# NVIDIA/AMGX

Measured on AMD Instinct MI355X. Metric: amg_setup_solve_seconds_poisson256_fgmres_agg, lower is better.
Workload: dtype fp64; 1 GPU; global_batch=16777216, seq_len=256, parallelism=dd1, rows_per_gpu=16777216, converged=True

## Files before the change

amgx_amd/amg/coloring.py:

```python

from __future__ import annotations

from typing import Callable, Dict

import numpy as np
import torch

from .. import ops

COLORING_REGISTRY: Dict[str, Callable] = {}


def register_coloring(name: str):
    def deco(fn):
        COLORING_REGISTRY[name] = fn
        return fn
    return deco


def _host_adj(A, level: int = 1):
    import scipy.sparse as sp
    ro = A.row_offsets.cpu().numpy().astype(np.int64)
    ci = A.col_indices.cpu().numpy().astype(np.int64)
    n = A.n_rows
    keep = ci < n
    rows = np.repeat(np.arange(n), np.diff(ro))[keep]
    cols = ci[keep]
    g = sp.csr_matrix((np.ones(rows.size, dtype=np.int8), (rows, cols)),
                      shape=(n, n))
    g = g + g.T
    if level >= 2:
        g = g @ g
    g = g.tocsr()
    g.setdiag(0)
    g.eliminate_zeros()
    return g.indptr, g.indices


def _square_graph_matrix(A):
    from ..matrix import CSRMatrix
    n = A.n_rows
    dev = A.row_offsets.device
    ci = A.col_indices
    keep = ci < n
    if bool(keep.all()):
        ro, cols = A.row_offsets, A.col_indices
    else:
        deg = A.row_offsets.to(torch.int64)
        rows = torch.repeat_interleave(
            torch.arange(n, dtype=torch.int64, device=dev),
            deg[1:] - deg[:-1])
        kept = torch.bincount(rows[keep], minlength=n)
        ro = torch.zeros(n + 1, dtype=torch.int64, device=dev)
        torch.cumsum(kept, 0, out=ro[1:])
        ro = ro.to(torch.int32)
        cols = ci[keep].contiguous()
    P = CSRMatrix(ro, cols,
                  torch.ones(int(cols.numel()), dtype=torch.float64,
                             device=dev), n_cols=n)
    return ops.spgemm(P, P)


def _greedy(indptr, indices, order):
    n = indptr.size - 1
    colors = np.full(n, -1, dtype=np.int32)
    for i in order:
        nb = indices[indptr[i]:indptr[i + 1]]
        used = set(int(colors[j]) for j in nb if colors[j] >= 0)
        c = 0
        while c in used:
            c += 1
        colors[i] = c
    return colors, (int(colors.max()) + 1 if n else 0)


def _hash(i: np.ndarray, salt: int) -> np.ndarray:
    s = np.uint64((salt * 0x9E3779B97F4A7C15) % (1 << 64))
    x = (i.astype(np.uint64) + s) * np.uint64(0xBF58476D1CE4E5B9)
    return (x ^ (x >> np.uint64(31))).astype(np.uint64)


@register_coloring("MIN_MAX")
def _min_max(A, scope, level):
    frac = scope.get("max_uncolored_percentage") if scope is not None \
        else 0.0
    if level <= 1:
        return ops.color_matrix(A, max_uncolored_frac=float(frac or 0))
    return ops.color_matrix(_square_graph_matrix(A),
                            max_uncolored_frac=float(frac or 0))


@register_coloring("PARALLEL_GREEDY")
def _parallel_greedy(A, scope, level):
    if A.row_offsets.is_cuda:
        return ops.color_matrix(A if level <= 1 else _square_graph_matrix(A),
                                seed=7)
    indptr, indices = _host_adj(A, level)
    n = indptr.size - 1
    colors = np.full(n, -1, dtype=np.int32)
    w = _hash(np.arange(n), 7)
    guard = 0
    while (colors < 0).any():
        newly = []
        for i in np.nonzero(colors < 0)[0]:
            nb = indices[indptr[i]:indptr[i + 1]]
            un_nb = nb[colors[nb] < 0]
            un_nb = un_nb[un_nb != i]
            if un_nb.size and not (w[i] > w[un_nb]).all():
                continue
            used = set(int(colors[j]) for j in nb if colors[j] >= 0)
            c = 0
            while c in used:
                c += 1
            newly.append((i, c))
        for i, c in newly:
            colors[i] = c
        guard += 1
        if guard > n + 2:
            raise RuntimeError("PARALLEL_GREEDY coloring did not converge")
    return colors, int(colors.max()) + 1 if n else 0


@register_coloring("SERIAL_GREEDY_BFS")
def _serial_greedy_bfs(A, scope, level):
    import collections
    indptr, indices = _host_adj(A, level)
    n = indptr.size - 1
    order = []
    seen = np.zeros(n, dtype=bool)
    for s in range(n):
        if seen[s]:
            continue
        q = collections.deque([s])
        seen[s] = True
        while q:
            i = q.popleft()
            order.append(i)
            for j in indices[indptr[i]:indptr[i + 1]]:
                if not seen[j]:
                    seen[j] = True
                    q.append(j)
    return _greedy(indptr, indices, np.asarray(order, dtype=np.int64))


@register_coloring("GREEDY_RECOLOR")
def _greedy_recolor(A, scope, level):
    colors, num = COLORING_REGISTRY["MIN_MAX"](A, scope, level)
    if not torch.is_tensor(colors):
        colors = torch.from_numpy(np.ascontiguousarray(colors))
    colors = colors.to(A.row_offsets.device, torch.int64)
    n = A.n_rows
    if n == 0 or num <= 1:
        return colors.to(torch.int32), max(num, 1 if n else 0)
    dev = colors.device
    if level >= 2:
        if dev.type == "cuda":
            A2 = _square_graph_matrix(A)
            ro64 = A2.row_offsets.to(torch.int64)
            ci = A2.col_indices.to(torch.int64)
        else:
            indptr, indices = _host_adj(A, level)
            ro64 = torch.from_numpy(indptr.astype(np.int64))
            ci = torch.from_numpy(indices.astype(np.int64))
    else:
        ro64 = A.row_offsets.to(torch.int64)
        ci = A.col_indices.to(torch.int64)
    rows = torch.repeat_interleave(
        torch.arange(n, dtype=torch.int64, device=dev), ro64[1:] - ro64[:-1])
    keep = (ci < n) & (ci != rows)
    er, ec = rows[keep], ci[keep]
    for c in range(num - 1, 0, -1):
        in_class = colors == c
        if not bool(in_class.any()):
            continue
        sel = in_class[er]
        sr, sc = er[sel], ec[sel]
        local = torch.full((n,), -1, dtype=torch.int64, device=dev)
        cls_rows = torch.nonzero(in_class, as_tuple=True)[0]
        local[cls_rows] = torch.arange(cls_rows.numel(), dtype=torch.int64,
                                       device=dev)
        used = torch.zeros(cls_rows.numel(), c + 1, dtype=torch.bool,
                           device=dev)
        nb_col = torch.clamp(colors[sc], max=c)
        used[local[sr], nb_col] = True
        cand = torch.arange(c + 1, dtype=torch.int64, device=dev) \
            .expand(cls_rows.numel(), c + 1)
        new_c = torch.where(used, torch.full_like(cand, c), cand) \
            .min(dim=1).values
        colors[cls_rows] = torch.minimum(new_c, colors[cls_rows])
    return colors.to(torch.int32), int(colors.max()) + 1


@register_coloring("MULTI_HASH")
def _multi_hash(A, scope, level):
    if A.row_offsets.is_cuda:
        max_hash = int(scope.get("max_num_hash")) if scope is not None else 7
        return ops.color_matrix(A if level <= 1 else _square_graph_matrix(A),
                                seed=11, multihash_rounds=max_hash)
    indptr, indices = _host_adj(A, level)
    n = indptr.size - 1
    max_hash = int(scope.get("max_num_hash")) if scope is not None else 7
    colors = np.full(n, -1, dtype=np.int32)
    for salt in range(max_hash):
        w = _hash(np.arange(n), salt + 11)
        un = colors < 0
        un_rows = np.nonzero(un)[0]
        if un_rows.size == 0:
            break
        newc = []
        for i in un_rows:
            nb = indices[indptr[i]:indptr[i + 1]]
            nb = nb[un[nb]]
            nbw = w[nb[nb != i]]
            if nbw.size == 0 or w[i] > nbw.max():
                newc.append(i)
        colors[np.asarray(newc, dtype=np.int64)] = salt
    if (colors < 0).any():
        for i in np.nonzero(colors < 0)[0]:
            nb = indices[indptr[i]:indptr[i + 1]]
            used = set(int(colors[j]) for j in nb if colors[j] >= 0)
            c = 0
            while c in used:
                c += 1
            colors[i] = max(c, 0)
    return colors, int(colors.max()) + 1 if n else 0


@register_coloring("ROUND_ROBIN")
def _round_robin(A, scope, level):
    n = A.n_rows
    if A.row_offsets.is_cuda and n > 20000:
        num = int(scope.get("num_colors") or 0) if scope is not None else 0
        if num <= 0:
            ro = A.row_offsets.to(torch.int64)
            num = max(int((ro[1:] - ro[:-1]).max()) + 1, 1)
        colors = (torch.arange(n, dtype=torch.int64,
                               device=A.row_offsets.device)
                  % num).to(torch.int32)
        return colors, num
    indptr, indices = _host_adj(A, level)
    n = indptr.size - 1
    colors = np.full(n, -1, dtype=np.int32)
    k = 1
    for i in range(n):
        nb = indices[indptr[i]:indptr[i + 1]]
        used = set(int(colors[j]) for j in nb if colors[j] >= 0)
        start = i % max(k, 1)
        c = start
        while c in used:
            c += 1
        colors[i] = c
        k = max(k, c + 1)
    return colors, int(colors.max()) + 1 if n else 0


@register_coloring("UNIFORM")
def _uniform(A, scope, level):
    n = A.n_rows
    ro = A.row_offsets.to(torch.int64)
    k = int((ro[1:] - ro[:-1]).max()) + 1 if n else 1
    k = max(k, 1)
    colors = (torch.arange(n, dtype=torch.int64,
                           device=A.row_offsets.device) % k).to(torch.int32)
    return colors, k if n else 0


@register_coloring("MIN_MAX_2RING")
def _min_max_2ring(A, scope, level):
    return ops.color_matrix(_square_graph_matrix(A))


@register_coloring("GREEDY_MIN_MAX_2RING")
def _greedy_min_max_2ring(A, scope, level):
    if A.row_offsets.is_cuda:
        return ops.color_matrix(_square_graph_matrix(A), seed=3)
    indptr, indices = _host_adj(A, 2)
    return _greedy(indptr, indices, np.arange(indptr.size - 1))


@register_coloring("LOCALLY_DOWNWIND")
def _locally_downwind(A, scope, level):
    indptr, indices = _host_adj(A, level)
    ro = A.row_offsets.cpu().numpy().astype(np.int64)
    ci = A.col_indices.cpu().numpy().astype(np.int64)
    v = A.values.cpu().numpy().reshape(A.nnz, -1)[:, 0]
    n = A.n_rows
    rows = np.repeat(np.arange(n), np.diff(ro))
    off = (rows != ci) & (ci < n)
    outflow = np.zeros(n)
    np.add.at(outflow, rows[off], -v[off])
    order = np.argsort(-outflow, kind="stable")
    return _greedy(indptr, indices, order)


class MatrixColoring:
    def __init__(self, colors: torch.Tensor, num_colors: int):
        self.colors = colors
        self.num_colors = num_colors
        counts = torch.bincount(colors.to(torch.int64), minlength=num_colors)
        order = torch.argsort(colors.to(torch.int64), stable=True)
        self.rows_sorted = order.to(torch.int32).contiguous()
        b = [0]
        for c in counts.cpu().tolist():
            b.append(b[-1] + int(c))
        self.bounds = b
        self.bounds_dev = torch.tensor(b, dtype=torch.int32,
                                       device=colors.device)

    @classmethod
    def create(cls, A, scope=None) -> "MatrixColoring":
        scheme = (scope.get("matrix_coloring_scheme")
                  if scope is not None else "MIN_MAX") or "MIN_MAX"
        level = int(scope.get("coloring_level")) if scope is not None else 1
        fn = COLORING_REGISTRY.get(scheme)
        if fn is None:
            raise KeyError(f"unknown coloring scheme {scheme!r}; known: "
                           f"{sorted(COLORING_REGISTRY)}")
        colors, num = fn(A, scope, max(level, 1))
        if isinstance(colors, np.ndarray):
            colors = torch.from_numpy(colors)
        return cls(colors.to(A.row_offsets.device), num)

    def rows_of(self, c: int) -> torch.Tensor:
        return self.rows_sorted[self.bounds[c]:self.bounds[c + 1]]

    def validate(self, A, level: int = 1) -> bool:
        indptr, indices = _host_adj(A, level)
        col = self.colors.cpu().numpy()
        rows = np.repeat(np.arange(indptr.size - 1), np.diff(indptr))
        return not bool((col[rows] == col[indices]).any())
```

amgx_amd/amg/level.py:

```python

from __future__ import annotations

from typing import Optional

import numpy as np
import torch

from .. import ops
from ..matrix import CSRMatrix


class AMGLevel:

    def __init__(self, A: CSRMatrix, scope, index: int):
        self.A = A
        self.scope = scope
        self.index = index
        self.next: Optional[AMGLevel] = None
        self.smoother = None
        mgr = getattr(A, "manager", None)
        n = mgr.ext_size if mgr is not None else A.n_rows * A.block_dim
        self.r = torch.zeros(n, dtype=A.dtype, device=A.device)
        self.bc = None
        self.xc = None

    def create_coarse_vertices(self) -> int:
        raise NotImplementedError

    def create_coarse_matrix(self) -> CSRMatrix:
        raise NotImplementedError

    def restrict_residual(self, r, bc):
        raise NotImplementedError

    def prolongate_and_apply(self, xc, x):
        raise NotImplementedError

    def rebuild_coarse_values(self):
        return None

    def alloc_coarse_vectors(self, Ac: CSRMatrix):
        mgr = getattr(Ac, "manager", None)
        nc = mgr.ext_size if mgr is not None else Ac.n_rows * Ac.block_dim
        self.bc = torch.zeros(nc, dtype=Ac.dtype, device=Ac.device)
        self.xc = torch.zeros(nc, dtype=Ac.dtype, device=Ac.device)


class AggregationLevel(AMGLevel):

    def __init__(self, A, scope, index):
        super().__init__(A, scope, index)
        self.aggregates = None
        self.num_aggregates = 0
        self._scale = None
        self._scale_counter = 0

    def create_coarse_vertices(self) -> int:
        from .aggregation import AGG_SELECTOR_REGISTRY
        selector = self.scope.get("selector") or "SIZE_2"
        mgr = getattr(self.A, "manager", None)
        fn = AGG_SELECTOR_REGISTRY.get(selector)
        if fn is None:
            raise KeyError(f"unknown aggregation selector {selector!r}; "
                           f"known: {sorted(AGG_SELECTOR_REGISTRY)}")
        if mgr is not None:
            agg, num = fn(self._local_square_view(), self.scope)
        else:
            agg, num = fn(self.A, self.scope)
        self.aggregates = agg.to(self.A.row_offsets.device)
        self.num_aggregates = num
        self._build_r_structure()
        return num

    def _local_square_view(self) -> CSRMatrix:
        A = self.A
        n = A.n_rows
        ro = A.row_offsets.to(torch.int64)
        keep = A.col_indices.to(torch.int64) < n
        rows = torch.repeat_interleave(
            torch.arange(n, dtype=torch.int64, device=keep.device),
            ro[1:] - ro[:-1])
        counts = torch.bincount(rows[keep], minlength=n)
        ro2 = torch.zeros(n + 1, dtype=torch.int64, device=keep.device)
        torch.cumsum(counts, 0, out=ro2[1:])
        return CSRMatrix(ro2.to(torch.int32),
                         A.col_indices[keep].contiguous(),
                         A.values[keep].contiguous(),
                         n_cols=n, block_dim=A.block_dim)

    def _build_r_structure(self):
        agg = self.aggregates.to(torch.int64)
        order = torch.argsort(agg, stable=True).to(torch.int32)
        counts = torch.bincount(agg, minlength=self.num_aggregates)
        off = torch.zeros(self.num_aggregates + 1, dtype=torch.int64,
                          device=agg.device)
        torch.cumsum(counts, 0, out=off[1:])
        self.r_structure = (off.to(torch.int32).contiguous(),
                            order.contiguous())

    def create_coarse_matrix(self) -> CSRMatrix:
        mgr = getattr(self.A, "manager", None)
        gen = self.scope.get("coarseAgenerator")
        if mgr is None:
            Ac = ops.galerkin_aggregation(self.A, self.aggregates,
                                          self.num_aggregates, generator=gen)
            Ac = self._color_renumber(Ac)
            geom = self.A._cache.get("geometry")
            if geom is not None:
                g = np.asarray(geom, dtype=np.float64)
                agg = self.aggregates.cpu().numpy().astype(np.int64)
                sums = np.zeros((self.num_aggregates, g.shape[1]))
                cnts = np.zeros(self.num_aggregates)
                np.add.at(sums, agg, g)
                np.add.at(cnts, agg, 1.0)
                Ac._cache["geometry"] = sums / np.maximum(cnts, 1.0)[:, None]
            return Ac
        return self._create_coarse_matrix_distributed(mgr)

    def _create_coarse_matrix_distributed(self, mgr) -> CSRMatrix:
        import torch.distributed as tdist
        from ..distributed.manager import DistributedManager
        A = self.A
        nc_local = self.num_aggregates
        counts = [None] * mgr.world
        tdist.all_gather_object(counts, nc_local)
        coarse_start = int(sum(counts[:mgr.rank]))
        n_global_c = int(sum(counts))
        aggv = torch.zeros((A.n_cols,), dtype=torch.float64, device=A.device)
        aggv[:mgr.n_local] = self.aggregates.to(torch.float64) + coarse_start
        mgr.exchange_halo(aggv, block_override=1)
        agg_col = aggv.round().to(torch.int32)
        Ac_local = ops.galerkin_aggregation(
            A, self.aggregates, nc_local, agg_col, n_global_c,
            generator=self.scope.get("coarseAgenerator"))
        Ac = DistributedManager.upload_global_csr(
            Ac_local.row_offsets, Ac_local.col_indices, Ac_local.values,
            nc_local, coarse_start, n_global_c,
            device=A.device, block_dim=A.block_dim, dtype=A.dtype)
        iperm = Ac.manager.row_iperm.to(self.aggregates.device)
        self.aggregates = iperm[self.aggregates.long()].to(torch.int32)
        self._build_r_structure()
        return Ac

    def _color_renumber(self, Ac):
        import os

        import torch

        from .coloring import MatrixColoring
        if not os.environ.get("AMGX_AMD_COARSE_RENUMBER"):
            return Ac
        if (not Ac.values.is_cuda or Ac.block_dim != 1
                or getattr(self.A, "manager", None) is not None
                or Ac.n_rows < 512):
            return Ac
        col = MatrixColoring.create(Ac, self.scope)
        perm = col.rows_sorted.to(torch.int64)
        iperm = torch.empty_like(perm)
        iperm[perm] = torch.arange(Ac.n_rows, dtype=torch.int64,
                                   device=perm.device)
        self.aggregates = iperm[self.aggregates.to(torch.int64)] \
            .to(torch.int32)
        self._build_r_structure()
        Ac2 = ops.galerkin_aggregation(self.A, self.aggregates,
                                       self.num_aggregates,
                                       generator=self.scope.get(
                                           "coarseAgenerator"))
        self._coarse_coloring = MatrixColoring(
            col.colors[perm].contiguous(), col.num_colors)
        Ac2.coloring = self._coarse_coloring
        return Ac2

    def rebuild_coarse_values(self):
        if self.aggregates is None \
                or getattr(self.A, "manager", None) is not None:
            return None
        Ac = ops.galerkin_aggregation(self.A, self.aggregates,
                                      self.num_aggregates,
                                      generator=self.scope.get(
                                          "coarseAgenerator"))
        coloring = getattr(self, "_coarse_coloring", None)
        if coloring is not None and Ac.values.is_cuda:
            Ac.coloring = coloring
        return Ac

    def restrict_residual(self, r, bc):
        ops.restrict_agg(r, self.aggregates, self.num_aggregates,
                         self.A.block_dim,
                         structure=getattr(self, "r_structure", None), out=bc)

    def prolongate_and_apply(self, xc, x):
        es = int(self.scope.get("error_scaling") or 0)
        if es in (2, 3):
            self._prolongate_scaled(xc, x, es)
            return
        ops.prolongate_agg(x, xc, self.aggregates, self.A.block_dim)

    def _prolongate_scaled(self, xc, x, mode: int):
        import math

        if self.A.values.is_complex():
            raise NotImplementedError(
                "error_scaling 2 / 3 is not available in the complex modes")
        if self._scale_counter > 0 and self._scale is not None:
            ef = torch.zeros_like(x)
            ops.prolongate_agg(ef, xc, self.aggregates, self.A.block_dim)
            ops.axpy(x, ef, self._scale)
            self._scale_counter -= 1
            return
        ef = torch.zeros_like(x)
        ops.prolongate_agg(ef, xc, self.aggregates, self.A.block_dim)
        steps = int(self.scope.get("scaling_smoother_steps") or 2)
        if self.smoother is not None and steps > 0:
            self.smoother.sweep(self.r, ef, steps)
        Aef = torch.zeros_like(ef)
        ops.spmv(self.A, ef, Aef)
        mgr = getattr(self.A, "manager", None)

        def gdot(u, v):
            if mgr is not None:
                d = ops.dot(u.reshape(-1)[:mgr.owned_size],
                            v.reshape(-1)[:mgr.owned_size])
                return float(mgr.global_sum(d))
            return float(ops.dot(u, v))

        if mode == 2:
            num, den = gdot(self.r, Aef), gdot(Aef, Aef)
        else:
            num, den = gdot(self.r, ef), gdot(ef, Aef)
        if den == 0.0:
            alpha = 1.0
        else:
            alpha = num / den
            if abs(alpha) < 0.3:
                alpha = math.copysign(0.3, alpha)
            elif abs(alpha) > 10.0:
                alpha = math.copysign(10.0, alpha)
        ops.axpy(x, ef, alpha)
        self._scale = alpha
        self._scale_counter = int(self.scope.get("reuse_scale") or 0)


class ClassicalLevel(AMGLevel):

    default_selector = "PMIS"
    default_interp = "D1"

    def __init__(self, A, scope, index):
        if A.block_dim != 1:
            raise ValueError(
                "CLASSICAL AMG supports scalar (1x1) matrices only, got "
                f"block_dim={A.block_dim}; use algorithm=AGGREGATION for "
                "block systems")
        super().__init__(A, scope, index)
        self.P = None
        self.R = None
        self.cf_map = None
        self.num_coarse = 0

    def create_coarse_vertices(self) -> int:
        mgr = getattr(self.A, "manager", None)
        if mgr is not None:
            from .classical_dist import (aggressive_thin_dist, pmis_dist,
                                         strength_dist)
            theta = float(self.scope.get("strength_threshold"))
            mrs = float(self.scope.get("max_row_sum"))
            self._strong_out, strong_union = strength_dist(
                self.A, mgr, theta, mrs)
            cf, nc = pmis_dist(self.A, mgr, strong_union)
            self._aggressive = self.index < int(
                self.scope.get("aggressive_levels") or 0)
            if self._aggressive:
                cf, nc = aggressive_thin_dist(self.A, mgr, strong_union, cf)
            self.cf_map = cf
            self.num_coarse = nc
            self.A._cache["cf_map"] = self.cf_map
            return nc
        from .classical import SELECTOR_REGISTRY, STRENGTH_REGISTRY
        strength = self.scope.get("strength") or "AHAT"
        S = STRENGTH_REGISTRY[strength](self.A, self.scope)
        sel = self.scope.get("selector") if self.scope.has("selector") \
            else self.default_selector
        if sel in (None, "SIZE_2", "SIZE_4", "SIZE_8"):
            sel = self.default_selector
        if self.index < int(self.scope.get("aggressive_levels") or 0):
            agg_sel = self.scope.get("aggressive_selector")
            sel = ("AGGRESSIVE_" + sel) if agg_sel in (None, "DEFAULT") \
                else agg_sel
            self._aggressive = True
        else:
            self._aggressive = False
        cf, nc = SELECTOR_REGISTRY[sel](self.A, S, self.scope)
        dev = self.A.row_offsets.device
        S, cf = S.to(dev), cf.to(dev)
        self.S = S
        self.cf_map = cf
        self.num_coarse = nc
        self.A._cache["cf_map"] = cf
        return nc

    def create_coarse_matrix(self) -> CSRMatrix:
        mgr = getattr(self.A, "manager", None)
        if mgr is not None:
            return self._create_coarse_matrix_distributed(mgr)
        from .classical import INTERP_REGISTRY
        interp = self.scope.get("interpolator") \
            if self.scope.has("interpolator") else self.default_interp
        if getattr(self, "_aggressive", False):
            interp = self.scope.get("aggressive_interpolator") or "MULTIPASS"
        self.P = INTERP_REGISTRY[interp](self.A, self.S, self.cf_map,
                                         self.num_coarse, self.scope)
        if self.P.row_offsets.device != self.A.row_offsets.device:
            self.P = self.P.to(self.A.row_offsets.device)
        tf = float(self.scope.get("interp_truncation_factor"))
        me = int(self.scope.get("interp_max_elements"))
        if tf > 0.0 or me >= 0:
            self.P = ops.truncate_rows(self.P, tf, me)
        self.R = ops.transpose(self.P)
        Ac = ops.galerkin_rap(self.R, self.A, self.P)
        return Ac

    def rebuild_coarse_values(self):
        if self.cf_map is None \
                or getattr(self.A, "manager", None) is not None:
            return None
        from .classical import STRENGTH_REGISTRY
        strength = self.scope.get("strength") or "AHAT"
        self.S = STRENGTH_REGISTRY[strength](self.A, self.scope) \
            .to(self.A.row_offsets.device)
        self.A._cache["cf_map"] = self.cf_map
        return self.create_coarse_matrix()

    def _create_coarse_matrix_distributed(self, mgr) -> CSRMatrix:
        from .classical_dist import (ClassicalDistOperators,
                                     coarse_numbering, rap_dist)
        from ..distributed.manager import DistributedManager
        A = self.A
        cf_ext, coarse_offs = coarse_numbering(mgr, self.cf_map,
                                               self.num_coarse)
        interp = self.scope.get("interpolator") \
            if self.scope.has("interpolator") else self.default_interp
        if getattr(self, "_aggressive", False):
            interp = self.scope.get("aggressive_interpolator") or "MULTIPASS"
        if interp == "D2":
            from .classical_dist import interp_d2_dist
            P_m = interp_d2_dist(A, mgr, self._strong_out, cf_ext,
                                 coarse_offs,
                                 float(self.scope.get("strength_threshold")))
        elif interp in (None, "D1"):
            S_dev = self._strong_out
            if A.row_offsets.is_cuda:
                S_dev = S_dev.to(torch.uint8)
            P_m = ops._backend(A).interp_d1(A, S_dev, cf_ext,
                                            int(coarse_offs[-1]))
        elif interp == "MULTIPASS":
            from .classical_dist import interp_multipass_dist
            P_m = interp_multipass_dist(A, mgr, self._strong_out, cf_ext,
                                        coarse_offs)
        elif interp == "EM":
            from .classical_dist import interp_em_dist
            P_m = interp_em_dist(A, mgr, self._strong_out, cf_ext,
                                 coarse_offs)
        else:
            raise NotImplementedError(
                f"distributed interpolator {interp!r}: D1/D2/MULTIPASS/EM"
                " are wired")
        tf = float(self.scope.get("interp_truncation_factor"))
        me = int(self.scope.get("interp_max_elements"))
        if tf > 0.0 or me >= 0:
            P_m = ops.truncate_rows(P_m, tf, me)
        rap = rap_dist(A, mgr, P_m, coarse_offs)
        Ac = DistributedManager.upload_global_csr(
            rap.row_offsets, rap.col_indices, rap.values, self.num_coarse,
            int(coarse_offs[mgr.rank]), int(coarse_offs[-1]),
            device=A.row_offsets.device, block_dim=1, dtype=A.dtype)
        self._dist_ops = ClassicalDistOperators(A, mgr, P_m, Ac,
                                                coarse_offs)
        return Ac

    def restrict_residual(self, r, bc):
        if getattr(self, "_dist_ops", None) is not None:
            self._dist_ops.restrict(r, bc)
            return
        ops.spmv(self.R, r, bc)

    def prolongate_and_apply(self, xc, x):
        if getattr(self, "_dist_ops", None) is not None:
            self._dist_ops.prolongate_add(xc, x)
            return
        tmp = torch.zeros_like(x)
        ops.spmv(self.P, xc, tmp)
        ops.axpy(x, tmp, 1.0)


class EnergyminLevel(ClassicalLevel):

    @property
    def default_selector(self):
        return self.scope.get("energymin_selector") or "CR"

    @property
    def default_interp(self):
        return self.scope.get("energymin_interpolator") or "EM"


def create_level(algorithm: str, A, scope, index) -> AMGLevel:
    if A.values.is_complex() and algorithm != "AGGREGATION":
        raise NotImplementedError(
            f"algorithm={algorithm} (classical / energymin AMG) is not "
            "available in the complex modes")
    if algorithm == "AGGREGATION":
        return AggregationLevel(A, scope, index)
    if algorithm == "CLASSICAL":
        return ClassicalLevel(A, scope, index)
    if algorithm == "ENERGYMIN":
        return EnergyminLevel(A, scope, index)
    raise KeyError(f"unknown AMG algorithm {algorithm!r}")
```

amgx_amd/csrc/bindings.cpp:

```cpp

#include <torch/extension.h>
#include <ATen/cuda/CUDAContext.h>
#include <pybind11/complex.h>

#include <algorithm>
#include <array>
#include <climits>
#include <complex>
#include <vector>

#include "core_api.h"

namespace {

using torch::Tensor;

hipStream_t cur_stream() {
    return (hipStream_t)at::cuda::getCurrentCUDAStream().stream();
}

inline void check_dev(const Tensor& t) {
    TORCH_CHECK(t.is_cuda(), "amgx_amd._core requires device tensors");
}

// ... 330 lines not shown
    int n = (int)(ro.numel() - 1);
    check_scalar_if_complex(va, b, "gs_smooth_rows");
    DISPATCH(AMGX_VALUE_PAIRS, "gs_smooth_rows", (va, x), [&] {
        amgx_hip::gs_smooth_rows<scalar_a, scalar_v>(
            iptr(ro), iptr(ci), dptr<scalar_a>(va), dptr<scalar_a>(dinv),
            dptr<scalar_v>(bvec), dptr<scalar_v>(x), iptr(rows),
            (int)rows.numel(), (scalar_v)omega, n, (int)b, cur_stream());
    });
}

void gs_sweep(Tensor ro, Tensor ci, Tensor va, int64_t b, Tensor dinv,
              Tensor bvec, Tensor x, Tensor rows_sorted,
              std::vector<int64_t> bounds, double omega, bool symmetric) {
    check_block_dim(b, "gs_sweep");
    int n = (int)(ro.numel() - 1);
    check_scalar_if_complex(va, b, "gs_sweep");
    DISPATCH(AMGX_VALUE_PAIRS, "gs_sweep", (va, x), [&] {
        auto run = [&](int, int64_t s, int64_t e) {
            amgx_hip::gs_smooth_rows<scalar_a, scalar_v>(
                iptr(ro), iptr(ci), dptr<scalar_a>(va), dptr<scalar_a>(dinv),
                dptr<scalar_v>(bvec), dptr<scalar_v>(x), iptr(rows_sorted) + s,
                (int)(e - s), (scalar_v)omega, n, (int)b, cur_stream());
        };
        for_each_color(bounds, true, run);
        if (symmetric) for_each_color(bounds, false, run);
    });
}

void gs_sweep_sorted(Tensor ro_s, Tensor ci_s, Tensor va_s, Tensor dinv_s,
                     Tensor bvec, Tensor x, Tensor rows_sorted,
                     std::vector<int64_t> bounds, Tensor bounds_dev,
                     double omega, bool symmetric) {
    int nc = (int)bounds.size() - 1;
    int64_t n = (int64_t)ro_s.numel() - 1;
    if (n <= amgx_hip::SMALL_LEVEL_ROWS) {
        DISPATCH(AMGX_VALUE_PAIRS, "gs_sweep_small", (va_s, x), [&] {
            amgx_hip::gs_sweep_small<scalar_a, scalar_v>(
                iptr(ro_s), iptr(ci_s), dptr<scalar_a>(va_s),
                dptr<scalar_a>(dinv_s), dptr<scalar_v>(bvec),
                dptr<scalar_v>(x), iptr(rows_sorted), iptr(bounds_dev), nc,
                (scalar_v)omega, symmetric, cur_stream());
        });
        return;
    }
    DISPATCH(AMGX_VALUE_PAIRS, "gs_sweep_sorted", (va_s, x), [&] {
        auto run = [&](int, int64_t s, int64_t e) {
            amgx_hip::gs_rows_sorted<scalar_a, scalar_v>(
                iptr(ro_s) + s, iptr(ci_s), dptr<scalar_a>(va_s),
                dptr<scalar_a>(dinv_s) + s, dptr<scalar_v>(bvec),
                dptr<scalar_v>(x), iptr(rows_sorted) + s, (int)(e - s),
                (scalar_v)omega, cur_stream());
        };
        for_each_color(bounds, true, run);
        if (symmetric) for_each_color(bounds, false, run);
    });
}

Tensor dilu_setup(Tensor ro, Tensor ci, Tensor va, int64_t b, Tensor didx,
                  Tensor tidx, Tensor colors, Tensor rows_sorted,
                  std::vector<int64_t> bounds) {
    check_block_dim(b, "dilu_setup");
    int n = (int)(ro.numel() - 1);
    check_scalar_if_complex(va, b, "dilu_setup");
    auto einv = b == 1 ? torch::zeros({n}, va.options())
                       : torch::zeros({n, b, b}, va.options());
    DISPATCH(AMGX_VALUE_TYPES, "dilu_setup", (va), [&] {
        for_each_color(bounds, true, [&](int c, int64_t s, int64_t e) {
            amgx_hip::dilu_setup_color<scalar_t>(
                iptr(ro), iptr(ci), dptr<scalar_t>(va), iptr(didx), iptr(tidx),
                iptr(colors), iptr(rows_sorted) + s, (int)(e - s), c,
                dptr<scalar_t>(einv), (int)b, cur_stream());
        });
    });
    return einv;
}

std::vector<Tensor> slab_split(Tensor ro_s, Tensor ci_s, Tensor rows_sorted,
                               Tensor colors, bool upper) {
    check_dev(ro_s);
    int64_t n = (int64_t)ro_s.numel() - 1;
    TORCH_CHECK(rows_sorted.numel() == n && colors.numel() == n,
                "slab_split: rows_sorted / colors do not have n rows");
    hipStream_t st = cur_stream();
    auto ro_x = torch::empty({n + 1}, ro_s.options());
    long long nnz = amgx_hip::slab_split_count(
        iptr(ro_s), iptr(ci_s), iptr(rows_sorted), iptr(colors), (int)n,
        upper, iptr(ro_x), st);
    auto ci_x = torch::empty({(int64_t)nnz}, ro_s.options());
    auto map_x = torch::empty({(int64_t)nnz}, ro_s.options());
    amgx_hip::slab_split_fill(iptr(ro_s), iptr(ci_s), iptr(rows_sorted),
                              iptr(colors), (int)n, upper, iptr(ro_x),
                              iptr(ci_x), iptr(map_x), st);
    return {ro_x, ci_x, map_x};
}

void dilu_sorted(Tensor ro_s, Tensor ci_s, Tensor va_s, int64_t b,
                 Tensor einv_s, Tensor rows_sorted,
                 std::vector<int64_t> bounds, Tensor bounds_dev, Tensor rhs,
                 Tensor w, Tensor z, Tensor x, double relax, bool fused,
                 bool any_size) {
    check_block_dim(b, "dilu_sorted");
    TORCH_CHECK(!fused || b == 1 || b == 4,
                "dilu_sorted: no fused-residual kernel for block_dim ", b);
    check_scalar_if_complex(va_s, b, "dilu_sorted");
    int nc = (int)bounds.size() - 1;
    int bb = (int)(b * b);
    int64_t n = (int64_t)ro_s.numel() - 1;
    if (b == 1) {
        TORCH_CHECK(any_size || n <= amgx_hip::DILU_SMALL_ROWS,
                    "dilu_sorted: scalar levels of more than ",
                    amgx_hip::DILU_SMALL_ROWS, " rows run dilu_split");
        TORCH_CHECK(bounds_dev.numel() == nc + 1 && rows_sorted.numel() == n &&
                        w.numel() >= n && z.numel() >= w.numel() &&
                        x.numel() >= n && rhs.numel() >= n &&
                        (!fused || x.numel() >= w.numel()),
                    "dilu_sorted: vectors shorter than the matrix");
        DISPATCH(AMGX_VALUE_PAIRS, "dilu_small_full", (va_s, x), [&] {
            amgx_hip::dilu_small_full<scalar_a, scalar_v>(
                iptr(ro_s), iptr(ci_s), dptr<scalar_a>(va_s),
                dptr<scalar_a>(einv_s), iptr(rows_sorted), iptr(bounds_dev),
                nc, dptr<scalar_v>(rhs), dptr<scalar_v>(w), dptr<scalar_v>(z),
                dptr<scalar_v>(x), (scalar_v)relax, (long long)w.numel(),
                fused, cur_stream());
        });
        return;
    }
    w.zero_();
    z.zero_();
    DISPATCH(AMGX_VALUE_PAIRS, "dilu_sorted", (va_s, x), [&] {
        hipStream_t st = cur_stream();
        const scalar_v* xres = fused ? dptr<scalar_v>(x) : nullptr;
        for_each_color(bounds, true, [&](int, int64_t s, int64_t e) {
            amgx_hip::dilu_fwd_sorted<scalar_a, scalar_v>(
                iptr(ro_s) + s, iptr(ci_s), dptr<scalar_a>(va_s),
                dptr<scalar_a>(einv_s) + s * bb, iptr(rows_sorted) + s,
                (int)(e - s), dptr<scalar_v>(rhs), xres, dptr<scalar_v>(w),
                (int)b, st);
        });
        for_each_color(bounds, false, [&](int, int64_t s, int64_t e) {
            amgx_hip::dilu_bwd_sorted<scalar_a, scalar_v>(
                iptr(ro_s) + s, iptr(ci_s), dptr<scalar_a>(va_s),
                dptr<scalar_a>(einv_s) + s * bb, iptr(rows_sorted) + s,
                (int)(e - s), dptr<scalar_v>(w), dptr<scalar_v>(z), (int)b,
                st);
        });
        amgx_hip::axpy<scalar_v>(dptr<scalar_v>(x), dptr<scalar_v>(z),
                                 (scalar_v)relax, x.numel(), st);
    });
}

constexpr double DILU_LANES_THRESHOLD_FULL = 8.0;
constexpr double DILU_LANES_THRESHOLD_SPLIT = 4.0;
int64_t dilu_lanes(double entries_per_row, bool split) {
    double t = split ? DILU_LANES_THRESHOLD_SPLIT : DILU_LANES_THRESHOLD_FULL;
    return entries_per_row <= t ? 1 : 8;
}

constexpr int64_t DILU_STREAM_MIN_ROWS_FULL = 1 << 14;
constexpr int64_t DILU_STREAM_MIN_ROWS_SPLIT = 1 << 14;
bool dilu_stream(double entries_per_row, int64_t color_rows, bool split) {
    int64_t least = split ? DILU_STREAM_MIN_ROWS_SPLIT
                          : DILU_STREAM_MIN_ROWS_FULL;
    return entries_per_row > 0.0 && color_rows >= least;
}

void dilu_split(Tensor ro_f, Tensor ci_f, Tensor va_f, Tensor ro_u,
                Tensor ci_u, Tensor va_u, Tensor einv_s, Tensor rows_sorted,
                std::vector<int64_t> bounds, Tensor rhs, Tensor w, Tensor x,
                double relax, bool fused, int64_t lanes,
                c10::optional<Tensor> y_opt, int64_t form) {
    int64_t n = (int64_t)ro_u.numel() - 1;
    TORCH_CHECK(ro_f.numel() == n + 1 && rows_sorted.numel() == n &&
                    einv_s.numel() == n,
                "dilu_split: slabs, rows_sorted and Einv disagree on n");
    TORCH_CHECK(form == 0 || form == 1 || form == 2,
                "dilu_split: form must be 0 (routed), 1 (lane forms) or 2 "
                "(stream form)");
    TORCH_CHECK(form != 2 || lanes == 0,
                "dilu_split: the stream form takes no lanes");
    TORCH_CHECK(!bounds.empty() && bounds.front() == 0 && bounds.back() == n,
                "dilu_split: color bounds do not cover the n rows");
    TORCH_CHECK(va_f.numel() == ci_f.numel() && va_u.numel() == ci_u.numel(),
                "dilu_split: scalar slabs hold one value per column index");
    TORCH_CHECK(rhs.numel() >= n && x.numel() >= n && w.numel() >= n &&
                    (!fused || w.numel() >= x.numel()),
                "dilu_split: vectors shorter than the matrix");
    TORCH_CHECK(w.scalar_type() == x.scalar_type() &&
                    rhs.scalar_type() == x.scalar_type() &&
                    va_u.scalar_type() == va_f.scalar_type() &&
                    einv_s.scalar_type() == va_f.scalar_type(),
                "dilu_split: mixed value types");
    TORCH_CHECK(lanes == 0 || lanes == 1 || lanes == 8,
                "dilu_split: lanes must be 0 (routed), 1 or 8");
    Tensor y;
    if (fused) {
        y = y_opt.has_value() ? *y_opt : torch::empty_like(w);
        TORCH_CHECK(y.is_contiguous() && y.device() == x.device() &&
                        y.scalar_type() == x.scalar_type() &&
                        y.numel() >= x.numel(),
                    "dilu_split: y must be a vector like w");
    }
    double rows = (double)std::max<int64_t>(n, 1);
    int lanes_f = lanes ? (int)lanes
                        : (int)dilu_lanes((double)ci_f.numel() / rows, !fused);
    int lanes_u = lanes ? (int)lanes
                        : (int)dilu_lanes((double)ci_u.numel() / rows, true);
    const double epr_f = (double)ci_f.numel() / rows;
    const double epr_u = (double)ci_u.numel() / rows;
    auto pick = [&](int lane_form, double epr, int64_t count, bool split) {
        bool stream = form == 2 || (form == 0 && lanes == 0 &&
                                    dilu_stream(epr, count, split));
        return stream ? amgx_hip::DILU_STREAM : lane_form;
    };
    DISPATCH(AMGX_VALUE_PAIRS, "dilu_split", (va_f, x), [&] {
        hipStream_t st = cur_stream();
        if (fused)
            amgx_hip::dilu_y_init<scalar_v>(dptr<scalar_v>(x),
                                            dptr<scalar_v>(y),
                                            (long long)x.numel(), st);
        for_each_color(bounds, true, [&](int, int64_t s, int64_t e) {
            if (fused)
                amgx_hip::dilu_fwd_full<scalar_a, scalar_v>(
                    iptr(ro_f) + s, iptr(ci_f), dptr<scalar_a>(va_f),
                    dptr<scalar_a>(einv_s) + s, iptr(rows_sorted) + s,
                    (int)(e - s), dptr<scalar_v>(rhs), dptr<scalar_v>(x),
                    dptr<scalar_v>(w), dptr<scalar_v>(y),
                    pick(lanes_f, epr_f, e - s, false), st);
            else
                amgx_hip::dilu_fwd_lower<scalar_a, scalar_v>(
                    iptr(ro_f) + s, iptr(ci_f), dptr<scalar_a>(va_f),
                    dptr<scalar_a>(einv_s) + s, iptr(rows_sorted) + s,
                    (int)(e - s), dptr<scalar_v>(rhs), dptr<scalar_v>(w),
                    pick(lanes_f, epr_f, e - s, true), st);
        });
        for_each_color(bounds, false, [&](int, int64_t s, int64_t e) {
            amgx_hip::dilu_bwd_upper<scalar_a, scalar_v>(
                iptr(ro_u) + s, iptr(ci_u), dptr<scalar_a>(va_u),
                dptr<scalar_a>(einv_s) + s, iptr(rows_sorted) + s,
                (int)(e - s), dptr<scalar_v>(w), dptr<scalar_v>(x),
                (scalar_v)relax, pick(lanes_u, epr_u, e - s, true), st);
        });
    });
}

void dilu_small(Tensor ro_f, Tensor ci_f, Tensor va_f, Tensor ro_u,
                Tensor ci_u, Tensor va_u, Tensor einv_s, Tensor rows_sorted,
                std::vector<int64_t> bounds, Tensor bounds_dev, Tensor rhs,
                Tensor w, Tensor x, double relax, bool fused, int64_t lanes,
                c10::optional<Tensor> y_opt, int64_t sweeps, bool any_size) {
    int64_t n = (int64_t)ro_u.numel() - 1;
    int64_t nc = (int64_t)bounds.size() - 1;
    TORCH_CHECK(any_size || n <= amgx_hip::DILU_SMALL_ROWS,
                "dilu_small: scalar levels of more than ",
                amgx_hip::DILU_SMALL_ROWS, " rows run dilu_split");
    TORCH_CHECK(ro_f.numel() == n + 1 && rows_sorted.numel() == n &&
                    einv_s.numel() == n,
                "dilu_small: slabs, rows_sorted and Einv disagree on n");
    TORCH_CHECK(!bounds.empty() && bounds.front() == 0 && bounds.back() == n &&
                    bounds_dev.numel() == nc + 1 &&
                    bounds_dev.scalar_type() == torch::kInt32,
                "dilu_small: color bounds do not cover the n rows");
    TORCH_CHECK(va_f.numel() == ci_f.numel() && va_u.numel() == ci_u.numel(),
                "dilu_small: scalar slabs hold one value per column index");
    TORCH_CHECK(rhs.numel() >= n && x.numel() >= n && w.numel() >= n &&
                    (!fused || w.numel() >= x.numel()),
                "dilu_small: vectors shorter than the matrix");
    TORCH_CHECK(w.scalar_type() == x.scalar_type() &&
                    rhs.scalar_type() == x.scalar_type() &&
                    va_u.scalar_type() == va_f.scalar_type() &&
                    einv_s.scalar_type() == va_f.scalar_type(),
                "dilu_small: mixed value types");
    TORCH_CHECK(lanes == 0 || lanes == 1 || lanes == 8,
                "dilu_small: lanes must be 0 (routed), 1 or 8");
    TORCH_CHECK(sweeps >= 1 && sweeps <= (1 << 20),
                "dilu_small: sweeps must be at least 1");
    for (Tensor t : {ro_f, ci_f, va_f, ro_u, ci_u, va_u, einv_s, rows_sorted,
                     bounds_dev, rhs, w, x})
        check_dev(t);
    Tensor y;
    if (fused) {
        TORCH_CHECK(y_opt.has_value(), "dilu_small: a fused apply needs y");
        y = *y_opt;
        TORCH_CHECK(y.is_contiguous() && y.device() == x.device() &&
                        y.scalar_type() == x.scalar_type() &&
                        y.numel() >= x.numel(),
                    "dilu_small: y must be a vector like w");
    }
    double rows = (double)std::max<int64_t>(n, 1);
    int lanes_f = lanes ? (int)lanes
                        : (int)dilu_lanes((double)ci_f.numel() / rows, !fused);
    int lanes_u = lanes ? (int)lanes
                        : (int)dilu_lanes((double)ci_u.numel() / rows, true);
    DISPATCH(AMGX_VALUE_PAIRS, "dilu_small", (va_f, x), [&] {
        amgx_hip::dilu_small<scalar_a, scalar_v>(
            iptr(ro_f), iptr(ci_f), dptr<scalar_a>(va_f), iptr(ro_u),
            iptr(ci_u), dptr<scalar_a>(va_u), dptr<scalar_a>(einv_s),
            iptr(rows_sorted), iptr(bounds_dev), (int)nc, dptr<scalar_v>(rhs),
            dptr<scalar_v>(w), fused ? dptr<scalar_v>(y) : nullptr,
            dptr<scalar_v>(x), (scalar_v)relax, (long long)x.numel(), fused,
            lanes_f, lanes_u, (int)sweeps, cur_stream());
    });
}

std::tuple<Tensor, int64_t> color_minmax(Tensor ro, Tensor ci, int64_t n,
                                         int64_t max_rounds, int64_t seed,
                                         int64_t mode1_rounds) {
    auto colors = torch::full({n}, -1,
                              ro.options().dtype(torch::kInt32));
    auto colors_next = torch::empty_like(colors);
    auto counter = torch::zeros({1}, ro.options().dtype(torch::kInt32));
    hipStream_t st = cur_stream();
    int rounds = 0;
    for (; rounds < max_rounds; ++rounds) {
        counter.zero_();
        int mode = rounds < mode1_rounds ? 1 : 0;
        amgx_hip::color_minmax_round(
            iptr(ro), iptr(ci), (int)n, iptr(colors), iptr(colors_next),
            rounds, (int)(seed + rounds * 7919), mode, iptr(counter), st);
        std::swap(colors, colors_next);
        int left = counter.cpu().item<int>();
        if (left == 0) break;
    }
    TORCH_CHECK((colors.min().cpu().item<int>()) >= 0,
                "MIN_MAX coloring did not converge in ", max_rounds,
                " rounds");
    int64_t ncolors = (colors.max().cpu().item<int>()) + 1;
    return {colors, ncolors};
}

Tensor size2_match(Tensor ro, Tensor ci, Tensor va, Tensor tidx, Tensor diag,
                   int64_t n, int64_t max_iters, int64_t seed) {
    auto agg = torch::full({n}, -1, ro.options().dtype(torch::kInt32));
    auto prop = torch::empty({n}, ro.options().dtype(torch::kInt32));
    auto changed = torch::zeros({1}, ro.options().dtype(torch::kInt32));
    hipStream_t st = cur_stream();
    DISPATCH(AMGX_VALUE_TYPES, "size2_match", (va), [&] {
        for (int it = 0; it < max_iters; ++it) {
            amgx_hip::agg_propose<scalar_t>(
                iptr(ro), iptr(ci), dptr<scalar_t>(va), iptr(tidx),
                dptr<scalar_t>(diag), (int)n, iptr(agg), iptr(prop), (int)seed,
                st);
            changed.zero_();
            amgx_hip::agg_match(iptr(prop), (int)n, iptr(agg), iptr(changed),
                                st);
            if (changed.cpu().item<int>() == 0) break;
        }
        auto agg_out = torch::empty_like(agg);
        amgx_hip::agg_merge_singletons<scalar_t>(
            iptr(ro), iptr(ci), dptr<scalar_t>(va), iptr(tidx),
            dptr<scalar_t>(diag), (int)n, iptr(agg), iptr(agg_out), st);
        agg = agg_out;
    });
    return agg;
}

Tensor pairwise_weights(Tensor ro, Tensor ci, Tensor va, Tensor tidx,
                        Tensor diag, int64_t n, int64_t formula) {
    check_dev(va);
    TORCH_CHECK(formula == 0 || formula == 1,
                "pairwise_weights: weight_formula must be 0 or 1");
    TORCH_CHECK_NOT_IMPLEMENTED(formula == 0 || !va.is_complex(),
                                "pairwise_weights: weight_formula 1 is "
                                "signed and unavailable for complex values");
    TORCH_CHECK(tidx.numel() == ci.numel() && va.numel() == ci.numel() &&
                    diag.numel() == n && ro.numel() == n + 1,
                "pairwise_weights: array sizes do not match the structure");
    auto w = torch::empty({ci.numel()}, va.options().dtype(torch::kFloat64));
    DISPATCH(AMGX_VALUE_TYPES, "pairwise_weights", (va), [&] {
        amgx_hip::pairwise_weights<scalar_t>(
            iptr(ro), iptr(ci), dptr<scalar_t>(va), iptr(tidx),
            dptr<scalar_t>(diag), (int)n, (int)formula, dptr<double>(w),
            cur_stream());
    });
    return w;
}

int pairwise_lanes(int64_t nnz, int64_t n) {
    double avg = (double)nnz / (double)std::max<int64_t>(n, 1);
    return avg <= 8.0 ? 1 : 8;
}

Tensor pairwise_propose(Tensor ro, Tensor ci, Tensor w, int64_t n, Tensor agg,
                        Tensor sizes, int64_t cap, int64_t seed,
                        int64_t lanes) {
    check_dev(w);
    TORCH_CHECK(ro.numel() == n + 1 && w.numel() == ci.numel() &&
                    agg.numel() == n && sizes.numel() == n,
                "pairwise_propose: array sizes do not match the structure");
    auto prop = torch::empty({n}, ro.options().dtype(torch::kInt32));
    int icap = cap <= 0 ? INT_MAX : (int)std::min<int64_t>(cap, INT_MAX);
    if (lanes == 0) lanes = pairwise_lanes(ci.numel(), n);
    amgx_hip::pairwise_propose(iptr(ro), iptr(ci), dptr<double>(w), (int)n,
                               iptr(agg), iptr(sizes), icap, (int)seed,
                               (int)lanes, iptr(prop), cur_stream());
    return prop;
}

std::tuple<Tensor, int64_t, Tensor, int64_t> pairwise_match(
    Tensor ro, Tensor ci, Tensor w, int64_t n, Tensor sizes_in, int64_t cap,
    int64_t merge_singletons, int64_t max_iters, double max_unassigned,
    int64_t seed, int64_t lanes) {
    check_dev(w);
    TORCH_CHECK(ro.numel() == n + 1 && w.numel() == ci.numel() &&
                    sizes_in.numel() == n,
                "pairwise_match: array sizes do not match the structure");
    TORCH_CHECK(merge_singletons >= 0 && merge_singletons <= 2,
                "pairwise_match: merge_singletons must be 0, 1 or 2");
    auto iopt = ro.options().dtype(torch::kInt32);
    auto agg = torch::full({n}, -1, iopt);
    auto sizes = sizes_in.clone();
    if (n == 0) return {agg, 0, sizes, 0};
    auto prop = torch::empty({n}, iopt);
    auto counter = torch::zeros({1}, iopt);
    hipStream_t st = cur_stream();
    const int* rp = iptr(ro);
    const int* cp = iptr(ci);
    const double* wp = dptr<double>(w);
    int icap = cap <= 0 ? INT_MAX : (int)std::min<int64_t>(cap, INT_MAX);
    if (lanes == 0) lanes = pairwise_lanes(ci.numel(), n);
    auto unaggregated = [&] {
        counter.zero_();
        amgx_hip::pairwise_count_unaggregated(iptr(agg), (int)n,
                                              iptr(counter), st);
        return (int64_t)counter.cpu().item<int>();
    };

    int64_t un = n, rounds = 0;
    while (rounds < max_iters && un > 0 &&
           !((double)un < max_unassigned * (double)n)) {
        amgx_hip::pairwise_propose(rp, cp, wp, (int)n, iptr(agg), iptr(sizes),
                                   icap, (int)seed, (int)lanes, iptr(prop),
                                   st);
        amgx_hip::pairwise_match(iptr(prop), (int)n, iptr(agg), iptr(sizes),
                                 st);
        ++rounds;
        int64_t left = unaggregated();
        if (left == un) break;
        un = left;
    }

    if (merge_singletons == 1 && un > 0) {
        auto agg_next = torch::empty_like(agg);
        while (un > 0) {
            amgx_hip::pairwise_join_sweep(rp, cp, wp, (int)n, iptr(agg),
                                          (int)seed, iptr(agg_next), st);
            std::swap(agg, agg_next);
            int64_t left = unaggregated();
            if (left == un) break;
            un = left;
        }
    } else if (merge_singletons == 2 && un > 0) {
        auto bid_root = torch::empty({n}, iopt);
        auto bid_w = torch::zeros({n}, ro.options().dtype(torch::kInt64));
        auto bid_i = torch::full({n}, n, iopt);
        while (un > 0) {
            amgx_hip::pairwise_join_capped(
                rp, cp, wp, (int)n, iptr(agg), iptr(sizes), icap, (int)seed,
                iptr(bid_root),
                reinterpret_cast<unsigned long long*>(dptr<int64_t>(bid_w)),
                iptr(bid_i), st);
            int64_t left = unaggregated();
            if (left == un) break;
            un = left;
        }
    }

    auto ids = torch::empty({n + 1}, iopt);
    size_t tmp_bytes = amgx_hip::pairwise_renumber_tmp_bytes((int)n);
    auto tmp = torch::empty({(int64_t)std::max<size_t>(tmp_bytes, 16)},
                            ro.options().dtype(torch::kUInt8));
    auto agg_out = torch::empty({n}, iopt);
    auto sizes_out = torch::zeros({n}, iopt);
    amgx_hip::pairwise_renumber(iptr(agg), (int)n, iptr(sizes_in), iptr(ids),
                                tmp.data_ptr(), tmp_bytes, iptr(agg_out),
                                iptr(sizes_out), st);
    int64_t num = ids[n].cpu().item<int>();
    return {agg_out, num, sizes_out.narrow(0, 0, num).clone(), rounds};
}

void restrict_agg(Tensor r, Tensor agg, int64_t b, Tensor rc) {
    rc.zero_();
    DISPATCH(AMGX_VALUE_TYPES, "restrict_agg", (r), [&] {
        amgx_hip::restrict_agg<scalar_t>(dptr<scalar_t>(r), iptr(agg),
                                         (int)agg.numel(), (int)b,
                                         dptr<scalar_t>(rc), cur_stream());
    });
}

void restrict_csr(Tensor r, Tensor off, Tensor fids, int64_t b, Tensor rc) {
    DISPATCH(AMGX_VALUE_TYPES, "restrict_csr", (r), [&] {
        amgx_hip::restrict_csr<scalar_t>(
            iptr(off), iptr(fids), dptr<scalar_t>(r), (int)(off.numel() - 1),
            (int)b, dptr<scalar_t>(rc), cur_stream());
    });
}

void prolongate_agg(Tensor x, Tensor xc, Tensor agg, int64_t b) {
    DISPATCH(AMGX_VALUE_TYPES, "prolongate_agg", (x), [&] {
        amgx_hip::prolongate_agg<scalar_t>(
            dptr<scalar_t>(x), dptr<scalar_t>(xc), iptr(agg), (int)agg.numel(),
            (int)b, cur_stream());
    });
}

void dense_gemv(Tensor Ainv, Tensor b, Tensor x) {
    DISPATCH(AMGX_VALUE_PAIRS, "dense_gemv", (Ainv, b), [&] {
        amgx_hip::dense_gemv<scalar_a, scalar_v>(
            dptr<scalar_a>(Ainv), dptr<scalar_v>(b), dptr<scalar_v>(x),
            (int)b.numel(), cur_stream());
    });
}

void gather(Tensor src, Tensor idx, int64_t b, Tensor dst) {
    DISPATCH(AMGX_VALUE_TYPES, "gather", (src), [&] {
        amgx_hip::gather<scalar_t>(dptr<scalar_t>(src), iptr(idx),
                                   (int)idx.numel(), (int)b,
                                   dptr<scalar_t>(dst), cur_stream());
    });
}

std::tuple<Tensor, Tensor, Tensor> galerkin_agg(Tensor ro, Tensor ci,
                                                Tensor va, Tensor agg,
                                                Tensor agg_col, int64_t nc,
                                                int64_t ncmod,
                                                int64_t block_dim) {
    int n = (int)(ro.numel() - 1);
    long long nnz = ci.numel();
    int bb = (int)(block_dim * block_dim);
    check_scalar_if_complex(va, block_dim, "galerkin_agg");
    auto ro_c = torch::empty({nc + 1}, ro.options());
    auto ci_c = torch::empty({nnz}, ro.options());
    auto va_c = block_dim == 1
                    ? torch::empty({nnz}, va.options())
                    : torch::empty({nnz, block_dim, block_dim}, va.options());
    long long nnz_c = 0;
    DISPATCH(AMGX_VALUE_TYPES, "galerkin_agg", (va), [&] {
        nnz_c = amgx_hip::galerkin_agg<scalar_t>(
            iptr(ro), iptr(ci), dptr<scalar_t>(va), n, nnz, iptr(agg),
            iptr(agg_col), (int)nc, (long long)ncmod, iptr(ro_c), iptr(ci_c),
            dptr<scalar_t>(va_c), bb, cur_stream());
    });
    return {ro_c, ci_c.narrow(0, 0, nnz_c), va_c.narrow(0, 0, nnz_c)};
}

std::tuple<Tensor, Tensor, Tensor> spgemm(Tensor roA, Tensor ciA, Tensor vaA,
                                          Tensor roB, Tensor ciB, Tensor vaB,
                                          int64_t n_cols_B,
                                          int64_t capacity) {
    int m = (int)(roA.numel() - 1);
    int k = (int)(roB.numel() - 1);
    auto ro_c = torch::empty({m + 1}, roA.options());
    auto ci_c = torch::empty({capacity}, roA.options());
    auto va_c = torch::empty({capacity}, vaA.options());
    long long nnz_c = 0;
    DISPATCH(AMGX_VALUE_TYPES, "spgemm", (vaA), [&] {
        nnz_c = amgx_hip::spgemm_esc<scalar_t>(
            iptr(roA), iptr(ciA), dptr<scalar_t>(vaA), m, ciA.numel(),
            iptr(roB), iptr(ciB), dptr<scalar_t>(vaB), k, (int)n_cols_B,
            iptr(ro_c), iptr(ci_c), dptr<scalar_t>(va_c), cur_stream());
    });
    return {ro_c, ci_c.narrow(0, 0, nnz_c), va_c.narrow(0, 0, nnz_c)};
}

std::tuple<Tensor, Tensor, Tensor> transpose(Tensor ro, Tensor ci, Tensor va,
                                             int64_t n_cols) {
    int m = (int)(ro.numel() - 1);
    long long nnz = ci.numel();
    auto ro_t = torch::empty({n_cols + 1}, ro.options());
    auto ci_t = torch::empty({nnz}, ro.options());
    auto va_t = torch::empty({nnz}, va.options());
    DISPATCH(AMGX_REAL_TYPES, "transpose", (va), [&] {
        amgx_hip::transpose_csr<scalar_t>(
            iptr(ro), iptr(ci), dptr<scalar_t>(va), m, (int)n_cols, nnz,
            iptr(ro_t), iptr(ci_t), dptr<scalar_t>(va_t), cur_stream());
    });
    return {ro_t, ci_t, va_t};
}

Tensor strength_ahat(Tensor ro, Tensor ci, Tensor va, Tensor didx,
                     double theta, double max_row_sum) {
    int n = (int)(ro.numel() - 1);
    auto strong = torch::empty({ci.numel()}, ro.options().dtype(torch::kUInt8));
    DISPATCH(AMGX_REAL_TYPES, "strength_ahat", (va), [&] {
        amgx_hip::strength_ahat<scalar_t>(
            iptr(ro), iptr(ci), dptr<scalar_t>(va), iptr(didx), n, theta,
            max_row_sum, dptr<unsigned char>(strong), cur_stream());
    });
    return strong;
}

Tensor pmis_select(Tensor ro, Tensor ci, Tensor tidx, Tensor strong,
                   int64_t max_rounds) {
    int n = (int)(ro.numel() - 1);
    auto w = torch::empty({n}, ro.options().dtype(torch::kFloat32));
    auto state = torch::zeros({n}, ro.options().dtype(torch::kChar));
    auto state_mid = torch::zeros_like(state);
    auto state_out = torch::zeros_like(state);
    auto counter = torch::zeros({1}, ro.options().dtype(torch::kInt32));
    hipStream_t st = cur_stream();
    amgx_hip::pmis_lambda(iptr(ro), iptr(ci), iptr(tidx),
                          dptr<unsigned char>(strong), n, dptr<float>(w), st);
    amgx_hip::pmis_mark_isolated(iptr(ro), iptr(ci), iptr(tidx),
                                 dptr<unsigned char>(strong), n,
                                 dptr<signed char>(state), st);
    for (int64_t round = 0;; ++round) {
        if (round >= max_rounds) {
            TORCH_CHECK(!state.eq(0).any().item<bool>(),
                        "PMIS failed to converge in ", max_rounds, " rounds");
            break;
        }
        counter.zero_();
        amgx_hip::pmis_one_round(
            iptr(ro), iptr(ci), iptr(tidx), dptr<unsigned char>(strong), n,
            dptr<float>(w), dptr<signed char>(state),
            dptr<signed char>(state_mid), dptr<signed char>(state_out),
            iptr(counter), st);
        std::swap(state, state_out);
        if (counter.cpu().item<int>() == 0) break;
    }
    return state;
}

std::tuple<Tensor, Tensor, Tensor> interp_d1(Tensor ro, Tensor ci, Tensor va,
                                             Tensor strong, Tensor cf,
                                             Tensor didx, Tensor p_ro,
                                             int64_t p_nnz) {
    int n = (int)(ro.numel() - 1);
    auto p_ci = torch::empty({p_nnz}, ro.options());
    auto p_va = torch::empty({p_nnz}, va.options());
    DISPATCH(AMGX_REAL_TYPES, "interp_d1", (va), [&] {
        amgx_hip::interp_d1<scalar_t>(
            iptr(ro), iptr(ci), dptr<scalar_t>(va),
            dptr<unsigned char>(strong), iptr(cf), iptr(didx), iptr(p_ro), n,
            (int)cf.numel(), iptr(p_ci), dptr<scalar_t>(p_va), cur_stream());
    });
    return {p_ro, p_ci, p_va};
}

std::tuple<Tensor, Tensor, Tensor> truncate_rows(Tensor ro, Tensor ci,
                                                 Tensor va, double factor,
                                                 int64_t max_elem) {
    int n = (int)(ro.numel() - 1);
    auto counts = torch::empty({n}, ro.options());
    DISPATCH(AMGX_REAL_TYPES, "truncate_count", (va), [&] {
        amgx_hip::truncate_rows_gpu<scalar_t>(
            iptr(ro), iptr(ci), dptr<scalar_t>(va), n, factor, (int)max_elem,
            nullptr, nullptr, nullptr, iptr(counts), cur_stream());
    });
    auto ro_out = torch::zeros({n + 1}, ro.options());
    ro_out.slice(0, 1, n + 1).copy_(
        torch::cumsum(counts.to(torch::kLong), 0).to(torch::kInt));
    int64_t nnz_out = n > 0 ? ro_out[n].item<int64_t>() : 0;
    auto ci_out = torch::empty({nnz_out}, ro.options());
    auto va_out = torch::empty({nnz_out}, va.options());
    DISPATCH(AMGX_REAL_TYPES, "truncate_fill", (va), [&] {
        amgx_hip::truncate_fill_gpu<scalar_t>(
            iptr(ro), iptr(ci), dptr<scalar_t>(va), n, factor, (int)max_elem,
            iptr(ro_out), iptr(ci_out), dptr<scalar_t>(va_out), cur_stream());
    });
    return {ro_out, ci_out, va_out};
}

Tensor interp_d1_count(Tensor ro, Tensor ci, Tensor strong, Tensor cf) {
    int n = (int)(ro.numel() - 1);
    auto counts = torch::empty({n}, ro.options());
    amgx_hip::interp_d1_count(iptr(ro), iptr(ci), dptr<unsigned char>(strong),
                              iptr(cf), n, (int)cf.numel(), iptr(counts),
                              cur_stream());
    return counts;
}

Tensor ilu0_setup(Tensor ro, Tensor ci, Tensor va, Tensor didx, Tensor pos,
                  Tensor rows_sorted, std::vector<int64_t> bounds) {
    int n = (int)(ro.numel() - 1);
    auto lu = va.clone();
    DISPATCH(AMGX_REAL_TYPES, "ilu0_setup", (va), [&] {
        for_each_color(bounds, true, [&](int, int64_t s, int64_t e) {
            amgx_hip::ilu0_factor_color_launch<scalar_t>(
                iptr(ro), iptr(ci), iptr(pos), iptr(didx),
                iptr(rows_sorted) + s, (int)(e - s), dptr<scalar_t>(lu), n,
                cur_stream());
        });
    });
    return lu;
}

std::vector<Tensor> ilu0_setup_block(Tensor ro, Tensor ci, Tensor va,
                                     int64_t b, Tensor didx, Tensor pos,
                                     Tensor rows_sorted,
                                     std::vector<int64_t> bounds) {
    check_block_dim(b, "ilu0_setup_block");
    int n = (int)(ro.numel() - 1);
    auto lu = va.clone().reshape({-1});
    auto dinv = torch::zeros({(int64_t)n * b * b}, va.options());
    DISPATCH(AMGX_REAL_TYPES, "ilu0_setup_block", (va), [&] {
        hipStream_t st = cur_stream();
        for_each_color(bounds, true, [&](int, int64_t s, int64_t e) {
            amgx_hip::ilu0_factor_color_block_launch<scalar_t>(
                iptr(ro), iptr(ci), iptr(pos), iptr(didx),
                iptr(rows_sorted) + s, (int)(e - s), dptr<scalar_t>(lu),
                dptr<scalar_t>(dinv), n, (int)b, st);
            amgx_hip::ilu0_invert_diag_block_launch<scalar_t>(
                iptr(didx), iptr(rows_sorted) + s, (int)(e - s),
                dptr<scalar_t>(lu), dptr<scalar_t>(dinv), (int)b, st);
        });
    });
    return {lu, dinv};
}

void ilu0_apply_block(Tensor ro, Tensor ci, Tensor lu, Tensor dinv,
                      int64_t b, Tensor pos, Tensor rows_sorted,
                      std::vector<int64_t> bounds, Tensor r, Tensor y,
                      Tensor z, Tensor x, double relax) {
    check_block_dim(b, "ilu0_apply_block");
    int n = (int)(ro.numel() - 1);
    y.zero_();
    z.zero_();
    DISPATCH(AMGX_REAL_PAIRS, "ilu0_apply_block", (lu, x), [&] {
        hipStream_t st = cur_stream();
        for_each_color(bounds, true, [&](int, int64_t s, int64_t e) {
            amgx_hip::ilu0_fwd_block_launch<scalar_a, scalar_v>(
                iptr(ro), iptr(ci), iptr(pos), dptr<scalar_a>(lu),
                iptr(rows_sorted) + s, (int)(e - s), dptr<scalar_v>(r),
                dptr<scalar_v>(y), n, (int)b, st);
        });
        for_each_color(bounds, false, [&](int, int64_t s, int64_t e) {
            amgx_hip::ilu0_bwd_block_launch<scalar_a, scalar_v>(
                iptr(ro), iptr(ci), iptr(pos), dptr<scalar_a>(lu),
                dptr<scalar_a>(dinv), iptr(rows_sorted) + s, (int)(e - s),
                dptr<scalar_v>(y), dptr<scalar_v>(z), n, (int)b, st);
        });
        amgx_hip::axpy<scalar_v>(dptr<scalar_v>(x), dptr<scalar_v>(z),
                                 (scalar_v)relax, x.numel(), st);
    });
}

void ilu0_apply_sorted(Tensor ro_s, Tensor ci_s, Tensor lu_s, Tensor diag_s,
                       Tensor pos, Tensor rows_sorted,
                       std::vector<int64_t> bounds, Tensor r, Tensor y,
                       Tensor z, Tensor x, double relax) {
    int n = (int)(ro_s.numel() - 1);
    y.zero_();
    z.zero_();
    DISPATCH(AMGX_REAL_PAIRS, "ilu0_apply_sorted", (lu_s, x), [&] {
        hipStream_t st = cur_stream();
        for_each_color(bounds, true, [&](int, int64_t s, int64_t e) {
            amgx_hip::ilu0_fwd_sorted<scalar_a, scalar_v>(
                iptr(ro_s) + s, iptr(ci_s), dptr<scalar_a>(lu_s), iptr(pos),
                iptr(rows_sorted) + s, (int)(e - s), dptr<scalar_v>(r),
                dptr<scalar_v>(y), n, st);
        });
        for_each_color(bounds, false, [&](int, int64_t s, int64_t e) {
            amgx_hip::ilu0_bwd_sorted<scalar_a, scalar_v>(
                iptr(ro_s) + s, iptr(ci_s), dptr<scalar_a>(lu_s),
                dptr<scalar_a>(diag_s) + s, iptr(pos), iptr(rows_sorted) + s,
                (int)(e - s), dptr<scalar_v>(y), dptr<scalar_v>(z), n, st);
        });
        amgx_hip::axpy<scalar_v>(dptr<scalar_v>(x), dptr<scalar_v>(z),
                                 (scalar_v)relax, x.numel(), st);
    });
}

}

PYBIND11_MODULE(TORCH_EXTENSION_NAME, m) {
    m.attr("SMALL_LEVEL_ROWS") = amgx_hip::SMALL_LEVEL_ROWS;
    m.attr("SPGEMM_HASH_TOP_CAP") = pybind11::dict(
        pybind11::arg("float64") = amgx_hip::spgemm_hash_top_cap<double>(),
        pybind11::arg("float32") = amgx_hip::spgemm_hash_top_cap<float>(),
        pybind11::arg("complex128") =
            amgx_hip::spgemm_hash_top_cap<cplx<double>>(),
        pybind11::arg("complex64") =
            amgx_hip::spgemm_hash_top_cap<cplx<float>>());
    m.def("csrmv", &csrmv);
    m.def("reduce_op", &reduce_op);
    m.def("axpy", &axpy);
    m.def("axpy_dalpha", &axpy_dalpha);
    m.def("mfma4_probe", &mfma4_probe);
    m.def("spgemm_hash", &spgemm_hash);
    m.attr("ILU1_TOP_CAP") = amgx_hip::ILU1_TOP_CAP;
    m.def("ilu1_pattern", &ilu1_pattern);
    m.def("ilu1_embed", &ilu1_embed);
    m.def("bsrmv_generic", &bsrmv_generic);
    m.def("scal_drsqrt", &scal_drsqrt);
    m.def("axpby", &axpby);
    m.def("scal", &scal);
    m.def("diag_index", &diag_index);
    m.def("extract_diag", &extract_diag);
    m.def("trans_index", &trans_index);
    m.def("jacobi_dinv", &jacobi_dinv);
    m.def("jacobi_smooth", &jacobi_smooth);
    m.def("gs_smooth_rows", &gs_smooth_rows);
    m.def("gs_sweep", &gs_sweep);
    m.def("gs_sweep_sorted", &gs_sweep_sorted);
    m.def("dilu_setup", &dilu_setup);
    m.attr("DILU_SMALL_ROWS") = amgx_hip::DILU_SMALL_ROWS;
    {
        using pybind11::arg;
        m.def("dilu_sorted", &dilu_sorted, arg("ro_s"), arg("ci_s"),
              arg("va_s"), arg("b"), arg("einv_s"), arg("rows_sorted"),
              arg("bounds"), arg("bounds_dev"), arg("rhs"), arg("w"),
              arg("z"), arg("x"), arg("relax"), arg("fused"),
              arg("any_size") = false);
        m.def("dilu_small", &dilu_small, arg("ro_f"), arg("ci_f"),
              arg("va_f"), arg("ro_u"), arg("ci_u"), arg("va_u"),
              arg("einv_s"), arg("rows_sorted"), arg("bounds"),
              arg("bounds_dev"), arg("rhs"), arg("w"), arg("x"), arg("relax"),
              arg("fused"), arg("lanes") = 0, arg("y") = pybind11::none(),
              arg("sweeps") = 1, arg("any_size") = false);
    }
    {
        using pybind11::arg;
        m.def("dilu_split", &dilu_split, arg("ro_f"), arg("ci_f"),
              arg("va_f"), arg("ro_u"), arg("ci_u"), arg("va_u"),
              arg("einv_s"), arg("rows_sorted"), arg("bounds"), arg("rhs"),
              arg("w"), arg("x"), arg("relax"), arg("fused"),
              arg("lanes") = 0, arg("y") = pybind11::none(),
              arg("form") = 0);
    }
    m.def("dilu_lanes", &dilu_lanes, pybind11::arg("entries_per_row"),
          pybind11::arg("split") = false);
    m.def("dilu_stream", &dilu_stream, pybind11::arg("entries_per_row"),
          pybind11::arg("color_rows"), pybind11::arg("split") = false);
    m.def("dilu_stream_window", &amgx_hip::dilu_stream_window_of,
          pybind11::arg("pair_bytes") = 16);
    m.attr("DILU_STREAM_ROWS") = amgx_hip::DILU_STREAM_ROWS;
    m.attr("DILU_STREAM_WINDOW") = amgx_hip::DILU_STREAM_WINDOW;
    m.attr("DILU_STREAM_MIN_ROWS_FULL") = DILU_STREAM_MIN_ROWS_FULL;
    m.attr("DILU_STREAM_MIN_ROWS_SPLIT") = DILU_STREAM_MIN_ROWS_SPLIT;
    m.def("slab_split", &slab_split);
    m.def("color_minmax", &color_minmax);
    m.def("size2_match", &size2_match);
    m.def("pairwise_weights", &pairwise_weights);
    m.def("pairwise_propose", &pairwise_propose);
    m.def("pairwise_match", &pairwise_match);
    m.def("restrict_agg", &restrict_agg);
    m.def("restrict_csr", &restrict_csr);
    m.def("prolongate_agg", &prolongate_agg);
    m.def("dense_gemv", &dense_gemv);
    m.def("gather", &gather);
    m.def("galerkin_agg", &galerkin_agg);
    m.def("spgemm", &spgemm);
    m.def("transpose", &transpose);
    m.def("strength_ahat", &strength_ahat);
    m.def("pmis_select", &pmis_select);
    m.def("interp_d1", &interp_d1);
    m.def("interp_d1_count", &interp_d1_count);
    m.def("truncate_rows", &truncate_rows);
    m.def("ilu0_setup", &ilu0_setup);
    m.def("ilu0_setup_block", &ilu0_setup_block);
    m.def("ilu0_apply_sorted", &ilu0_apply_sorted);
    m.def("ilu0_apply_block", &ilu0_apply_block);
}
```

amgx_amd/csrc/core_api.h:

```cpp
#pragma once

#include <hip/hip_runtime.h>

#include <cstdint>

#include "cplx.h"

#define AMGX_REAL_TYPES(X) X(double) X(float)
#define AMGX_VALUE_TYPES(X) AMGX_REAL_TYPES(X) X(cplx<double>) X(cplx<float>)
#define AMGX_REAL_PAIRS(X) X(double, double) X(float, float) X(float, double)
#define AMGX_VALUE_PAIRS(X)                                                   \
    AMGX_REAL_PAIRS(X)                                                        \
    X(cplx<double>, cplx<double>)                                             \
    X(cplx<float>, cplx<float>)                                               \
    X(cplx<float>, cplx<double>)

#define AMGX_INSTANTIATE(F, ...) template decltype(F<__VA_ARGS__>) F<__VA_ARGS__>;

namespace amgx_hip {

constexpr int MAX_BLOCK_DIM = 16;


template <typename TA, typename TV>
void csrmv(const int* ro, const int* ci, const TA* va, const TV* x, TV* y,
           const TV* bvec, TV alpha, TV beta, TV gamma, int r0, int r1,
           double avg_deg, hipStream_t s);

template <typename TA, typename TV>
void bsrmv(const int* ro, const int* ci, const TA* va, int b, const TV* x,
           TV* y, const TV* bvec, TV alpha, TV beta, TV gamma, int r0, int r1,
           hipStream_t s);

template <typename TA, typename TV>
void bsrmv_generic(const int* ro, const int* ci, const TA* va, int b,
                   const TV* x, TV* y, const TV* bvec, TV alpha, TV beta,
                   TV gamma, int r0, int r1, hipStream_t s);

template <typename T>
void reduce(const T* x, const T* y, long long n, int op, void* ws, void* out,
            hipStream_t s);

template <typename T>
void axpy(T* y, const T* x, T a, long long n, hipStream_t s);
template <typename T>
void axpy_dalpha(T* y, const T* x, const T* alpha, T scale, long long n,
                 hipStream_t s);
template <typename T>
void scal_drsqrt(T* x, const T* s2, long long n, hipStream_t s);
template <typename T>
void axpby(T* y, const T* x, T a, T b, long long n, hipStream_t s);
template <typename T>
void scal(T* x, T a, long long n, hipStream_t s);

void diag_index(const int* ro, const int* ci, int n, int* out, hipStream_t s);
template <typename T>
void extract_diag(const T* va, const int* didx, int n, int b, T* out,
                  hipStream_t s);
void trans_index(const int* ro, const int* ci, int n, int* out, hipStream_t s);

template <typename T>
void jacobi_dinv(const int* ro, const T* va, const int* didx, int n, int b,
                 bool l1, T* dinv, hipStream_t s);
template <typename TA, typename TV>
void jacobi_smooth(const int* ro, const int* ci, const TA* va, const TA* dinv,
                   const TV* bvec, const TV* xi, TV* xo, TV omega, int n,
                   int b, hipStream_t s);
template <typename TA, typename TV>
void gs_smooth_rows(const int* ro, const int* ci, const TA* va,
                    const TA* dinv, const TV* bvec, TV* x, const int* rows,
                    int count, TV omega, int n, int b, hipStream_t s);

constexpr int SMALL_LEVEL_ROWS = 1 << 14;

template <typename TA, typename TV>
void gs_sweep_small(const int* ro_s, const int* ci_s, const TA* va_s,
                    const TA* dinv_s, const TV* bvec, TV* x, const int* rows,
                    const int* bounds, int ncolors, TV omega, bool symmetric,
                    hipStream_t s);
template <typename TA, typename TV>
void gs_rows_sorted(const int* ro_s, const int* ci_s, const TA* va_s,
                    const TA* dinv_s, const TV* bvec, TV* x, const int* rows,
                    int count, TV omega, hipStream_t s);

constexpr int DILU_SMALL_ROWS = 1 << 10;
template <typename TA, typename TV>
void dilu_small(const int* ro_f, const int* ci_f, const TA* va_f,
                const int* ro_u, const int* ci_u, const TA* va_u,
                const TA* einv_s, const int* rows, const int* bounds,
                int ncolors, const TV* rhs, TV* w, TV* y, TV* x, TV relax,
                long long vec_n, bool fused, int lanes_f, int lanes_u,
                int sweeps, hipStream_t s);
template <typename TA, typename TV>
void dilu_small_full(const int* ro_s, const int* ci_s, const TA* va_s,
                     const TA* einv_s, const int* rows, const int* bounds,
                     int ncolors, const TV* rhs, TV* w, TV* z, TV* x,
                     TV relax, long long vec_n, bool fused, hipStream_t s);
template <typename TA, typename TV>
void dilu_fwd_sorted(const int* ro_s, const int* ci_s, const TA* va_s,
                     const TA* einv_s, const int* rows, int count,
                     const TV* rhs, const TV* xres ,
                     TV* w, int b, hipStream_t s);
template <typename TA, typename TV>
void dilu_bwd_sorted(const int* ro_s, const int* ci_s, const TA* va_s,
                     const TA* einv_s, const int* rows, int count,
                     const TV* wv, TV* z, int b, hipStream_t s);
constexpr int DILU_STREAM = 64;
constexpr int DILU_STREAM_ROWS = 64;
constexpr int DILU_STREAM_WINDOW_BYTES = 8192;
constexpr int DILU_STREAM_WINDOW = 512;
constexpr int dilu_stream_window_of(int pair_bytes) {
    int w = DILU_STREAM_WINDOW_BYTES / pair_bytes;
    w -= w % 64;
    return w < DILU_STREAM_WINDOW ? w : DILU_STREAM_WINDOW;
}
template <typename TV>
void dilu_y_init(const TV* x, TV* y, long long n, hipStream_t s);
template <typename TA, typename TV>
void dilu_fwd_full(const int* ro_s, const int* ci_s, const TA* va_s,
                   const TA* einv_s, const int* rows, int count,
                   const TV* rhs, const TV* x, TV* w, TV* y, int lanes,
                   hipStream_t s);
template <typename TA, typename TV>
void dilu_fwd_lower(const int* ro_l, const int* ci_l, const TA* va_l,
                    const TA* einv_s, const int* rows, int count,
                    const TV* rhs, TV* w, int lanes, hipStream_t s);
template <typename TA, typename TV>
void dilu_bwd_upper(const int* ro_u, const int* ci_u, const TA* va_u,
                    const TA* einv_s, const int* rows, int count, TV* w,
                    TV* x, TV relax, int lanes, hipStream_t s);
template <typename T>
void dilu_setup_color(const int* ro, const int* ci, const T* va,
                      const int* didx, const int* tidx, const int* colors,
                      const int* rows, int count, int color, T* einv, int b,
                      hipStream_t s);

template <typename T>
void restrict_agg(const T* r, const int* agg, int n, int b, T* rc,
                  hipStream_t s);
template <typename T>
void restrict_csr(const int* off, const int* fids, const T* r, int nc, int b,
                  T* rc, hipStream_t s);
template <typename T>
void prolongate_agg(T* x, const T* xc, const int* agg, int n, int b,
                    hipStream_t s);

template <typename TA, typename TV>
void dense_gemv(const TA* Ainv, const TV* b, TV* x, int n, hipStream_t s);

template <typename T>
void gather(const T* src, const int* idx, int count, int b, T* dst,
            hipStream_t s);

void mfma4_probe(const double* a, const double* b, double* c, hipStream_t s);
template <typename TA, typename TV>
void bsrmv_b4(const int* ro, const int* ci, const TA* va, const TV* x, TV* y,
              const TV* bvec, double alpha, double beta, double gamma,
              int row_begin, int row_end, hipStream_t s);
template <typename TA, typename TV>
void bsrmv_bn(const int* ro, const int* ci, const TA* va, int b, const TV* x,
              TV* y, const TV* bvec, double alpha, double beta, double gamma,
              int row_begin, int row_end, hipStream_t s);
template <typename TA, typename TV>
void dilu_fwd_b4_sorted(const int* ro_s, const int* ci_s, const TA* va_s,
                        const TA* einv_s, const int* rows, int count,
                        const TV* r, const TV* xres ,
                        TV* w, hipStream_t s);
template <typename TA, typename TV>
void dilu_bwd_b4_sorted(const int* ro_s, const int* ci_s, const TA* va_s,
                        const TA* einv_s, const int* rows, int count,
                        const TV* w, TV* z, hipStream_t s);
template <typename TA>
void dilu_setup_b4(const int* ro, const int* ci, const TA* va,
                   const int* didx, const int* tidx, const int* colors,
                   const int* rows, int count, int color, TA* einv,
                   hipStream_t s);

void color_minmax_round(const int* ro, const int* ci, int n,
                        const int* colors_prev, int* colors_next, int iter,
                        int seed, int mode, int* n_uncolored, hipStream_t s);

template <typename T>
void agg_propose(const int* ro, const int* ci, const T* va, const int* tidx,
                 const T* diag, int n, const int* agg, int* prop, int seed,
                 hipStream_t s);
void agg_match(const int* prop, int n, int* agg, int* changed, hipStream_t s);
template <typename T>
void agg_merge_singletons(const int* ro, const int* ci, const T* va,
                          const int* tidx, const T* diag, int n,
                          const int* agg_in, int* agg_out, hipStream_t s);

template <typename T>
void pairwise_weights(const int* ro, const int* ci, const T* va,
                      const int* tidx, const T* diag, int n, int formula,
                      double* w, hipStream_t s);
void pairwise_propose(const int* ro, const int* ci, const double* w, int n,
                      const int* agg, const int* sizes, int cap, int seed,
                      int lanes, int* prop, hipStream_t s);
void pairwise_match(const int* prop, int n, int* agg, int* sizes,
                    hipStream_t s);
void pairwise_count_unaggregated(const int* agg, int n, int* count,
                                 hipStream_t s);
void pairwise_join_sweep(const int* ro, const int* ci, const double* w, int n,
                         const int* agg_in, int seed, int* agg_out,
                         hipStream_t s);
void pairwise_join_capped(const int* ro, const int* ci, const double* w, int n,
                          int* agg, int* sizes, int cap, int seed,
                          int* bid_root, unsigned long long* bid_w, int* bid_i,
                          hipStream_t s);
size_t pairwise_renumber_tmp_bytes(int n);
void pairwise_renumber(int* agg, int n, const int* sizes_in, int* ids,
                       void* tmp, size_t tmp_bytes, int* agg_out,
                       int* sizes_out, hipStream_t s);

long long slab_split_count(const int* ro_s, const int* ci_s, const int* rows,
                           const int* colors, int n, bool upper, int* ro_x,
                           hipStream_t s);
void slab_split_fill(const int* ro_s, const int* ci_s, const int* rows,
                     const int* colors, int n, bool upper, const int* ro_x,
                     int* ci_x, int* map_x, hipStream_t s);

template <typename T>
long long galerkin_agg(const int* ro, const int* ci, const T* va, int n,
                       long long nnz, const int* agg, const int* agg_col,
                       int nc, long long ncmod, int* ro_c, int* ci_c, T* va_c,
                       int bb, hipStream_t s);

template <typename T>
long long spgemm_esc(const int* roA, const int* ciA, const T* vaA, int m,
                     long long nnzA, const int* roB, const int* ciB,
                     const T* vaB, int k, int n, int* ro_c, int* ci_c, T* va_c,
                     hipStream_t s);

template <typename T>
void transpose_csr(const int* ro, const int* ci, const T* va, int m, int n,
                   long long nnz, int* ro_t, int* ci_t, T* va_t,
                   hipStream_t s);

template <typename T>
constexpr int spgemm_hash_top_cap() { return sizeof(T) > 8 ? 4096 : 8192; }
template <typename T>
long long spgemm_hash(const int* roA, const int* ciA, const T* vaA, int m,
                      const int* roB, const int* ciB, const T* vaB,
                      const int* aggcol, int mode, int cap0, int* roC_out,
                      int* ciC_cap_buf, T* vaC_cap_buf, long long cap_nnz,
                      int** big_rows_out, int* n_big_out, hipStream_t s);
void free_device_buf(void* p, hipStream_t s);

constexpr int ILU1_TOP_CAP = 8192;
struct Ilu1Tiers {
    int* mid_rows = nullptr;
    int n_mid = 0;
    int* big_rows = nullptr;
    int n_big = 0;
};
long long ilu1_pattern_count(const int* ro, const int* ci, const int* colors,
                             int n, int* roC_out, Ilu1Tiers* tiers,
                             hipStream_t s);
void ilu1_pattern_fill(const int* ro, const int* ci, const int* colors, int n,
                       const int* roC, int* ciC, const Ilu1Tiers& tiers,
                       hipStream_t s);
void ilu1_tiers_free(Ilu1Tiers* tiers, hipStream_t s);
template <typename T>
void ilu1_embed(const int* roA, const int* ciA, const T* vaA, int n,
                long long nnzA, int bb, const int* roL, const int* ciL,
                T* vaL, int* a_to_lu, hipStream_t s);

template <typename T>
void strength_ahat(const int* ro, const int* ci, const T* va, const int* didx,
                   int n, double theta, double max_row_sum,
                   unsigned char* strong, hipStream_t s);
void pmis_lambda(const int* ro, const int* ci, const int* tidx,
                 const unsigned char* strong, int n, float* w, hipStream_t s);
void pmis_mark_isolated(const int* ro, const int* ci, const int* tidx,
                        const unsigned char* strong, int n, signed char* state,
                        hipStream_t s);
void pmis_one_round(const int* ro, const int* ci, const int* tidx,
                    const unsigned char* strong, int n, const float* w,
                    const signed char* state, signed char* state_mid,
                    signed char* state_out, int* n_undecided, hipStream_t s);
void interp_d1_count(const int* ro, const int* ci, const unsigned char* strong,
                     const int* cf, int n, int ncols, int* counts,
                     hipStream_t s);
template <typename T>
void interp_d1(const int* ro, const int* ci, const T* va,
               const unsigned char* strong, const int* cf, const int* didx,
               const int* p_ro, int n, int ncols, int* p_ci, T* p_va,
               hipStream_t s);

template <typename T>
void ilu0_factor_color_launch(const int* ro, const int* ci, const int* pos,
                              const int* didx, const int* rows, int count,
                              T* lu, int n, hipStream_t s);
template <typename TA, typename TV>
void ilu0_fwd_sorted(const int* ro_s, const int* ci_s, const TA* lu_s,
                     const int* pos, const int* rows, int count, const TV* r,
                     TV* y, int n, hipStream_t s);
template <typename TA, typename TV>
void ilu0_bwd_sorted(const int* ro_s, const int* ci_s, const TA* lu_s,
                     const TA* diag_s, const int* pos, const int* rows,
                     int count, const TV* y, TV* z, int n, hipStream_t s);
template <typename T>
void ilu0_factor_color_block_launch(const int* ro, const int* ci,
                                    const int* pos, const int* didx,
                                    const int* rows, int count, T* lu,
                                    const T* dinv, int n, int b,
                                    hipStream_t s);
template <typename T>
void ilu0_invert_diag_block_launch(const int* didx, const int* rows,
                                   int count, const T* lu, T* dinv, int b,
                                   hipStream_t s);
template <typename TA, typename TV>
void ilu0_fwd_block_launch(const int* ro, const int* ci, const int* pos,
                           const TA* lu, const int* rows, int count,
                           const TV* r, TV* y, int n, int b, hipStream_t s);
template <typename TA, typename TV>
void ilu0_bwd_block_launch(const int* ro, const int* ci, const int* pos,
                           const TA* lu, const TA* dinv, const int* rows,
                           int count, const TV* y, TV* z, int n, int b,
                           hipStream_t s);

template <typename T>
void truncate_rows_gpu(const int* ro, const int* ci, const T* va, int n,
                       double factor, int max_elem, const int* ro_out,
                       int* ci_out, T* va_out, int* counts, hipStream_t s);
template <typename T>
void truncate_fill_gpu(const int* ro, const int* ci, const T* va, int n,
                       double factor, int max_elem, const int* ro_out,
                       int* ci_out, T* va_out, hipStream_t s);
}
```

amgx_amd/csrc/kernels_setup.hip:

```cpp

#include <cstring>

#include <rocprim/rocprim.hpp>

#include <stdexcept>
#include <string>

#include "common.h"
#include "core_api.h"

namespace amgx_hip {

__device__ __forceinline__ unsigned int hash_u32(unsigned int a,
                                                 unsigned int seed) {
    a ^= seed;
    a = (a ^ 61u) ^ (a >> 16);
    a *= 9u;
    a ^= a >> 4;
    a *= 0x27d4eb2du;
    a ^= a >> 15;
    return a;
}

__global__ __launch_bounds__(AMGX_BLOCK) void color_round_kernel(const int* __restrict__ ro,
                                   const int* __restrict__ ci, int n,
                                   const int* __restrict__ colors_prev,
                                   int* __restrict__ colors_next, int iter,
                                   int seed, int mode,
                                   int* __restrict__ n_uncolored) {
    int i = blockIdx.x * blockDim.x + threadIdx.x;
    if (i >= n) return;
    if (colors_prev[i] >= 0) { colors_next[i] = colors_prev[i]; return; }
    unsigned long long mine =
        ((unsigned long long)hash_u32((unsigned)i, (unsigned)seed) << 32) |
        (unsigned)i;
    bool is_max = true;
    unsigned long long used = 0ull;
    int big_used_max = -1;
    for (int k = ro[i]; k < ro[i + 1]; ++k) {
        int j = ci[k];
        if (j == i || j >= n) continue;
        int cj = colors_prev[j];
        if (cj >= 0) {
            if (cj < 64) used |= (1ull << cj);
            else big_used_max = max(big_used_max, cj);
            continue;
        }
        unsigned long long h =
            ((unsigned long long)hash_u32((unsigned)j, (unsigned)seed) << 32) |
            (unsigned)j;
        if (h > mine) { is_max = false; break; }
    }
    int out = -1;
    if (is_max) {
        if (mode == 1) {
            out = iter;
        } else {
            int c = (int)(__builtin_ffsll((long long)~used) - 1);
            if (c < 0 || c >= 64) c = big_used_max + 1;
            out = c;
        }
    } else {
        atomicAdd(n_uncolored, 1);
    }
    colors_next[i] = out;
}

void color_minmax_round(const int* ro, const int* ci, int n,
                        const int* colors_prev, int* colors_next, int iter,
                        int seed, int mode, int* n_uncolored, hipStream_t s) {
    hipLaunchKernelGGL(color_round_kernel, dim3(grid_1d(n)), dim3(AMGX_BLOCK),
                       0, s, ro, ci, n, colors_prev, colors_next, iter, seed,
                       mode, n_uncolored);
}

template <typename T>
__device__ __forceinline__ double edge_weight(const T* va, const int* tidx,
                                              const T* diag, int k, int i,
                                              int j) {
    double aij = absd(va[k]);
    double aji = tidx[k] >= 0 ? absd(va[tidx[k]]) : 0.0;
    double di = absd(diag[i]);
    double dj = absd(diag[j]);
    double scale = rsqrt((di > 0 ? di : 1.0) * (dj > 0 ? dj : 1.0));
    return (aij + aji) * scale;
}

template <typename T>
__global__ __launch_bounds__(AMGX_BLOCK) void agg_propose_kernel(const int* __restrict__ ro,
                                   const int* __restrict__ ci,
                                   const T* __restrict__ va,
                                   const int* __restrict__ tidx,
                                   const T* __restrict__ diag, int n,
                                   const int* __restrict__ agg,
                                   int* __restrict__ prop, int seed) {
    int i = blockIdx.x * blockDim.x + threadIdx.x;
    if (i >= n) return;
    if (agg[i] >= 0) { prop[i] = -1; return; }
    int best = -1;
    double bw = 0.0;
    unsigned int bt = 0;
    for (int k = ro[i]; k < ro[i + 1]; ++k) {
        int j = ci[k];
        if (j == i || j >= n || agg[j] >= 0) continue;
        double w = edge_weight(va, tidx, diag, k, i, j);
        unsigned int tj = hash_u32((unsigned)j, (unsigned)seed);
        if (w > bw ||
            (w == bw && best >= 0 &&
             (tj > bt || (tj == bt && j > best)))) {
            bw = w; best = j; bt = tj;
        }
    }
    prop[i] = best;
}

__global__ __launch_bounds__(AMGX_BLOCK) void agg_match_kernel(const int* __restrict__ prop, int n,
                                 int* __restrict__ agg,
                                 int* __restrict__ changed) {
    int i = blockIdx.x * blockDim.x + threadIdx.x;
    if (i >= n) return;
    int j = prop[i];
    if (j >= 0 && prop[j] == i && i < j) {
        agg[i] = i;
        agg[j] = i;
        atomicAdd(changed, 1);
    }
}

template <typename T>
__global__ __launch_bounds__(AMGX_BLOCK) void agg_singleton_kernel(const int* __restrict__ ro,
                                     const int* __restrict__ ci,
                                     const T* __restrict__ va,
                                     const int* __restrict__ tidx,
                                     const T* __restrict__ diag, int n,
                                     const int* __restrict__ agg_in,
                                     int* __restrict__ agg_out) {
    int i = blockIdx.x * blockDim.x + threadIdx.x;
    if (i >= n) return;
    if (agg_in[i] >= 0) { agg_out[i] = agg_in[i]; return; }
    int best = -1;
    double bw = -1.0;
    for (int k = ro[i]; k < ro[i + 1]; ++k) {
        int j = ci[k];
        if (j == i || j >= n || agg_in[j] < 0) continue;
        double w = edge_weight(va, tidx, diag, k, i, j);
        if (w > bw || (w == bw && best >= 0 && agg_in[j] > agg_in[best])) {
            bw = w;
            best = j;
        }
    }
    agg_out[i] = best >= 0 ? agg_in[best] : i;
}

template <typename T>
void agg_propose(const int* ro, const int* ci, const T* va, const int* tidx,
                 const T* diag, int n, const int* agg, int* prop, int seed,
                 hipStream_t s) {
    hipLaunchKernelGGL((agg_propose_kernel<T>), dim3(grid_1d(n)),
                       dim3(AMGX_BLOCK), 0, s, ro, ci, va, tidx, diag, n, agg,
                       prop, seed);
}

void agg_match(const int* prop, int n, int* agg, int* changed, hipStream_t s) {
    hipLaunchKernelGGL(agg_match_kernel, dim3(grid_1d(n)), dim3(AMGX_BLOCK),
                       0, s, prop, n, agg, changed);
}

template <typename T>
void agg_merge_singletons(const int* ro, const int* ci, const T* va,
                          const int* tidx, const T* diag, int n,
                          const int* agg_in, int* agg_out, hipStream_t s) {
    hipLaunchKernelGGL((agg_singleton_kernel<T>), dim3(grid_1d(n)),
                       dim3(AMGX_BLOCK), 0, s, ro, ci, va, tidx, diag, n,
                       agg_in, agg_out);
}


template <typename T>
__device__ __forceinline__ double pairwise_weight(const T* __restrict__ va,
                                                  const int* __restrict__ tidx,
                                                  const T* __restrict__ diag,
                                                  int k, int i, int j, int n,
                                                  int formula) {
#pragma clang fp contract(off)
    if (j == i || j >= n) return 0.0;
    int t = tidx[k];
    if (t < 0) return 0.0;
    if (formula == 0) {
        double di = absd(diag[i]), dj = absd(diag[j]);
        double m = di > dj ? di : dj;
        if (!(m > 0.0)) return 0.0;
        return 0.5 * (absd(va[k]) + absd(va[t])) / m;
    }
    if constexpr (is_cplx<T>::value) {
        return 0.0;
    } else {
        double di = (double)diag[i], dj = (double)diag[j];
        if (di == 0.0 || dj == 0.0) return 0.0;
        return -0.5 * ((double)va[k] / di + (double)va[t] / dj);
    }
}

template <typename T>
__global__ __launch_bounds__(AMGX_BLOCK) void pairwise_weights_kernel(
    const int* __restrict__ ro, const int* __restrict__ ci,
    const T* __restrict__ va, const int* __restrict__ tidx,
    const T* __restrict__ diag, int n, int formula, double* __restrict__ w) {
    int i = blockIdx.x * blockDim.x + threadIdx.x;
    if (i >= n) return;
    for (int k = ro[i]; k < ro[i + 1]; ++k)
        w[k] = pairwise_weight(va, tidx, diag, k, i, ci[k], n, formula);
}

__device__ __forceinline__ unsigned int pair_hash(int i, int j,
                                                  unsigned int seed) {
    unsigned int lo = (unsigned)min(i, j), hi = (unsigned)max(i, j);
    return hash_u32(hash_u32(lo, seed) ^ hi, seed);
}

struct PairCand {
    double w;
    unsigned int h;
    int j;
};

__device__ __forceinline__ bool cand_better(int i, const PairCand& a,
                                            const PairCand& b) {
    if (a.j < 0) return false;
    if (b.j < 0) return true;
    if (a.w != b.w) return a.w > b.w;
    if (a.h != b.h) return a.h > b.h;
    int alo = min(i, a.j), blo = min(i, b.j);
    if (alo != blo) return alo > blo;
    return max(i, a.j) > max(i, b.j);
}

__device__ __forceinline__ PairCand match_cand(
    const int* __restrict__ ci, const double* __restrict__ w,
    const int* __restrict__ agg, const int* __restrict__ sizes, int k, int i,
    int n, int si, int cap, unsigned int seed) {
    PairCand c{0.0, 0u, -1};
    int j = ci[k];
    if (j == i || j >= n) return c;
    double wk = w[k];
    if (!(wk > 0.0) || agg[j] >= 0) return c;
    if ((long long)si + sizes[j] > (long long)cap) return c;
    c.w = wk;
    c.h = pair_hash(i, j, seed);
    c.j = j;
    return c;
}

__global__ __launch_bounds__(AMGX_BLOCK) void pairwise_propose_kernel(
    const int* __restrict__ ro, const int* __restrict__ ci,
    const double* __restrict__ w, int n, const int* __restrict__ agg,
    const int* __restrict__ sizes, int cap, unsigned int seed,
    int* __restrict__ prop) {
    int i = blockIdx.x * blockDim.x + threadIdx.x;
    if (i >= n) return;
    if (agg[i] >= 0) { prop[i] = -1; return; }
    int si = sizes[i];
    PairCand best{0.0, 0u, -1};
    for (int k = ro[i]; k < ro[i + 1]; ++k) {
        PairCand c = match_cand(ci, w, agg, sizes, k, i, n, si, cap, seed);
        if (cand_better(i, c, best)) best = c;
    }
    prop[i] = best.j >= 0 ? best.j : i;
}

template <int L>
__global__ __launch_bounds__(AMGX_BLOCK) void pairwise_propose_vec_kernel(
    const int* __restrict__ ro, const int* __restrict__ ci,
    const double* __restrict__ w, int n, const int* __restrict__ agg,
    const int* __restrict__ sizes, int cap, unsigned int seed,
    int* __restrict__ prop) {
    const int lane = threadIdx.x & (L - 1);
    long long t = (long long)blockIdx.x * blockDim.x + threadIdx.x;
    if (t / L >= n) return;
    int i = (int)(t / L);
    if (agg[i] >= 0) {
        if (lane == 0) prop[i] = -1;
        return;
    }
    int si = sizes[i];
    PairCand best{0.0, 0u, -1};
    for (int k = ro[i] + lane; k < ro[i + 1]; k += L) {
        PairCand c = match_cand(ci, w, agg, sizes, k, i, n, si, cap, seed);
        if (cand_better(i, c, best)) best = c;
    }
#pragma unroll
    for (int off = L / 2; off > 0; off >>= 1) {
        PairCand o;
        o.w = __shfl_down(best.w, off, L);
        o.h = __shfl_down(best.h, off, L);
        o.j = __shfl_down(best.j, off, L);
        if (cand_better(i, o, best)) best = o;
    }
    if (lane == 0) prop[i] = best.j >= 0 ? best.j : i;
}

__global__ __launch_bounds__(AMGX_BLOCK) void pairwise_match_kernel(
    const int* __restrict__ prop, int n, int* __restrict__ agg,
    int* __restrict__ sizes) {
    int i = blockIdx.x * blockDim.x + threadIdx.x;
    if (i >= n) return;
    int j = prop[i];
    if (j > i && prop[j] == i) {
        agg[i] = i;
        agg[j] = i;
        sizes[i] += sizes[j];
    }
}

__global__ __launch_bounds__(AMGX_BLOCK) void pairwise_count_kernel(
    const int* __restrict__ agg, int n, int* __restrict__ count) {
    int i = blockIdx.x * blockDim.x + threadIdx.x;
    int c = block_reduce_sum<int>((i < n && agg[i] < 0) ? 1 : 0);
    if (threadIdx.x == 0 && c > 0) atomicAdd(count, c);
}

__device__ __forceinline__ PairCand join_cand(
    const int* __restrict__ ci, const double* __restrict__ w,
    const int* __restrict__ agg, const int* __restrict__ sizes, int k, int i,
    int n, int si, int cap, unsigned int seed) {
    PairCand c{0.0, 0u, -1};
    int j = ci[k];
    if (j == i || j >= n) return c;
    double wk = w[k];
    if (!(wk > 0.0)) return c;
    int r = agg[j];
    if (r < 0) return c;
    if (sizes && (long long)si + sizes[r] > (long long)cap) return c;
    c.w = wk;
    c.h = pair_hash(i, j, seed);
    c.j = j;
    return c;
}

__global__ __launch_bounds__(AMGX_BLOCK) void pairwise_join_sweep_kernel(
    const int* __restrict__ ro, const int* __restrict__ ci,
    const double* __restrict__ w, int n, const int* __restrict__ agg_in,
    unsigned int seed, int* __restrict__ agg_out) {
    int i = blockIdx.x * blockDim.x + threadIdx.x;
    if (i >= n) return;
    int a = agg_in[i];
    if (a < 0) {
        PairCand best{0.0, 0u, -1};
        for (int k = ro[i]; k < ro[i + 1]; ++k) {
            PairCand c = join_cand(ci, w, agg_in, nullptr, k, i, n, 0, 0, seed);
            if (cand_better(i, c, best)) best = c;
        }
        if (best.j >= 0) a = agg_in[best.j];
    }
    agg_out[i] = a;
}

__global__ __launch_bounds__(AMGX_BLOCK) void pairwise_bid_kernel(
    const int* __restrict__ ro, const int* __restrict__ ci,
    const double* __restrict__ w, int n, const int* __restrict__ agg,
    const int* __restrict__ sizes, int cap, unsigned int seed,
    int* __restrict__ bid_root, unsigned long long* __restrict__ bid_w) {
    int i = blockIdx.x * blockDim.x + threadIdx.x;
    if (i >= n) return;
    int r = -1;
    if (agg[i] < 0) {
        PairCand best{0.0, 0u, -1};
        int si = sizes[i];
        for (int k = ro[i]; k < ro[i + 1]; ++k) {
            PairCand c = join_cand(ci, w, agg, sizes, k, i, n, si, cap, seed);
            if (cand_better(i, c, best)) best = c;
        }
        if (best.j >= 0) {
            r = agg[best.j];
            unsigned long long bits =
                (unsigned long long)__double_as_longlong(best.w);
            bid_w[i] = bits;
            atomicMax(&bid_w[r], bits);
        }
    }
    bid_root[i] = r;
}

__global__ __launch_bounds__(AMGX_BLOCK) void pairwise_bid_tie_kernel(
    int n, const int* __restrict__ bid_root,
    const unsigned long long* __restrict__ bid_w, int* __restrict__ bid_i) {
    int i = blockIdx.x * blockDim.x + threadIdx.x;
    if (i >= n) return;
    int r = bid_root[i];
    if (r >= 0 && bid_w[i] == bid_w[r]) atomicMin(&bid_i[r], i);
}

__global__ __launch_bounds__(AMGX_BLOCK) void pairwise_accept_kernel(
    int n, int* __restrict__ agg, int* __restrict__ sizes,
    unsigned long long* __restrict__ bid_w, int* __restrict__ bid_i) {
    int r = blockIdx.x * blockDim.x + threadIdx.x;
    if (r >= n) return;
    if (agg[r] != r) return;
    int i = bid_i[r];
    if (i < n) {
        agg[i] = r;
        sizes[r] += sizes[i];
        bid_i[r] = n;
    }
    bid_w[r] = 0ull;
}

__global__ __launch_bounds__(AMGX_BLOCK) void pairwise_root_flag_kernel(
    int* __restrict__ agg, int n, int* __restrict__ ids) {
    int i = blockIdx.x * blockDim.x + threadIdx.x;
    if (i > n) return;
    int f = 0;
    if (i < n) {
        if (agg[i] < 0) agg[i] = i;
        f = agg[i] == i ? 1 : 0;
    }
    ids[i] = f;
}

__global__ __launch_bounds__(AMGX_BLOCK) void pairwise_renumber_kernel(
    const int* __restrict__ agg, int n, const int* __restrict__ ids,
    const int* __restrict__ sizes_in, int* __restrict__ agg_out,
    int* __restrict__ sizes_out) {
    int i = blockIdx.x * blockDim.x + threadIdx.x;
    if (i >= n) return;
    int id = ids[agg[i]];
    agg_out[i] = id;
    atomicAdd(&sizes_out[id], sizes_in[i]);
}

template <typename T>
void pairwise_weights(const int* ro, const int* ci, const T* va,
                      const int* tidx, const T* diag, int n, int formula,
                      double* w, hipStream_t s) {
    if (n <= 0) return;
    hipLaunchKernelGGL((pairwise_weights_kernel<T>), dim3(grid_1d(n)),
                       dim3(AMGX_BLOCK), 0, s, ro, ci, va, tidx, diag, n,
                       formula, w);
}

void pairwise_propose(const int* ro, const int* ci, const double* w, int n,
                      const int* agg, const int* sizes, int cap, int seed,
                      int lanes, int* prop, hipStream_t s) {
    if (n <= 0) return;
    if (lanes == 8) {
        hipLaunchKernelGGL((pairwise_propose_vec_kernel<8>),
                           dim3(grid_1d((long long)n * 8)), dim3(AMGX_BLOCK),
                           0, s, ro, ci, w, n, agg, sizes, cap,
                           (unsigned)seed, prop);
    } else if (lanes == 1) {
        hipLaunchKernelGGL(pairwise_propose_kernel, dim3(grid_1d(n)),
                           dim3(AMGX_BLOCK), 0, s, ro, ci, w, n, agg, sizes,
                           cap, (unsigned)seed, prop);
    } else {
        throw std::runtime_error("pairwise_propose: lanes must be 1 or 8");
    }
}

void pairwise_match(const int* prop, int n, int* agg, int* sizes,
                    hipStream_t s) {
    if (n <= 0) return;
    hipLaunchKernelGGL(pairwise_match_kernel, dim3(grid_1d(n)),
                       dim3(AMGX_BLOCK), 0, s, prop, n, agg, sizes);
}
// ... 199 lines not shown
            HIP_CHECK(hipMemsetAsync(ro_c, 0, (nc + 1) * sizeof(int), s));
        hipLaunchKernelGGL(keys_to_csr, dim3(grid_1d(h_runs, AMGX_BLOCK, 4096)),
                           dim3(AMGX_BLOCK), 0, s, ukeys, (long long)h_runs,
                           nc_ll, (long long)nc, ro_c, ci_c);
        dev_free(tmp, s); dev_free(tmpb, s); dev_free(vals, s);
        dev_free(nruns, s); dev_free(keys, s); dev_free(rows, s);
        return (long long)h_runs;
    }
    int* perm = (int*)dev_alloc(nnz * sizeof(int) * 2, s);
    int* perm_alt = perm + nnz;
    hipLaunchKernelGGL(make_agg_keys_perm, dim3(grid_1d(nnz, AMGX_BLOCK, 4096)),
                       dim3(AMGX_BLOCK), 0, s, rows, ci, agg, agg_col, nnz,
                       nc_ll, keys, perm);
    size_t tmp_bytes = 0;
    rocprim::radix_sort_pairs(nullptr, tmp_bytes, keys, keys_alt, perm,
                              perm_alt, nnz, 0, 64, s);
    void* tmp = dev_alloc(tmp_bytes, s);
    rocprim::radix_sort_pairs(tmp, tmp_bytes, keys, keys_alt, perm, perm_alt,
                              nnz, 0, 64, s);
    int* run_starts = (int*)dev_alloc((nnz + 1) * sizeof(int), s);
    unsigned int* nruns = (unsigned int*)dev_alloc(sizeof(unsigned int), s);
    HIP_CHECK(hipMemsetAsync(nruns, 0, sizeof(unsigned int), s));
    hipLaunchKernelGGL(find_run_starts, dim3(grid_1d(nnz, AMGX_BLOCK, 4096)),
                       dim3(AMGX_BLOCK), 0, s, keys_alt, nnz, run_starts,
                       nruns);
    unsigned int h_runs = 0;
    HIP_CHECK(hipMemcpyAsync(&h_runs, nruns, sizeof(unsigned int),
                             hipMemcpyDeviceToHost, s));
    HIP_CHECK(hipStreamSynchronize(s));
    if (h_runs == 0) {
        HIP_CHECK(hipMemsetAsync(ro_c, 0, (nc + 1) * sizeof(int), s));
        dev_free(run_starts, s); dev_free(nruns, s); dev_free(perm, s);
        dev_free(tmp, s); dev_free(keys, s); dev_free(rows, s);
        return 0;
    }
    size_t tmp3 = 0;
    int* rs_alt = (int*)dev_alloc(h_runs * sizeof(int), s);
    rocprim::radix_sort_keys(nullptr, tmp3, run_starts, rs_alt, h_runs, 0, 32, s);
    void* tmpc = dev_alloc(tmp3, s);
    rocprim::radix_sort_keys(tmpc, tmp3, run_starts, rs_alt, h_runs, 0, 32, s);
    K* ukeys = keys;
    hipLaunchKernelGGL(gather_keys, dim3(grid_1d(h_runs, AMGX_BLOCK, 4096)),
                       dim3(AMGX_BLOCK), 0, s, keys_alt, rs_alt,
                       (long long)h_runs, ukeys);
    hipLaunchKernelGGL(keys_to_csr, dim3(grid_1d(h_runs, AMGX_BLOCK, 4096)),
                       dim3(AMGX_BLOCK), 0, s, ukeys, (long long)h_runs, nc_ll,
                       (long long)nc, ro_c, ci_c);
    hipLaunchKernelGGL((sum_blocks_by_run<T>),
                       dim3(grid_1d((long long)h_runs * bb, AMGX_BLOCK, 4096)),
                       dim3(AMGX_BLOCK), 0, s, rs_alt, perm_alt, va, h_runs,
                       nnz, bb, va_c);
    dev_free(tmp, s); dev_free(tmpc, s); dev_free(rs_alt, s);
    dev_free(run_starts, s); dev_free(nruns, s); dev_free(perm, s);
    dev_free(keys, s); dev_free(rows, s);
    return (long long)h_runs;
}

__global__ __launch_bounds__(AMGX_BLOCK) void expand_degree(const int* __restrict__ ciA,
                              const int* __restrict__ roB, long long nnzA,
                              unsigned long long* __restrict__ deg) {
    long long stride = (long long)gridDim.x * blockDim.x;
    for (long long k = (long long)blockIdx.x * blockDim.x + threadIdx.x;
         k < nnzA; k += stride) {
        int c = ciA[k];
        deg[k] = (unsigned long long)(roB[c + 1] - roB[c]);
    }
}

template <typename T>
__global__ __launch_bounds__(AMGX_BLOCK) void expand_fill(const int* __restrict__ rowsA,
                            const int* __restrict__ ciA,
                            const T* __restrict__ vaA,
                            const int* __restrict__ roB,
                            const int* __restrict__ ciB,
                            const T* __restrict__ vaB, long long nnzA,
                            const unsigned long long* __restrict__ off,
                            long long ncolsB,
                            unsigned long long* __restrict__ keys,
                            T* __restrict__ vals) {
    long long stride = (long long)gridDim.x * blockDim.x;
    for (long long k = (long long)blockIdx.x * blockDim.x + threadIdx.x;
         k < nnzA; k += stride) {
        int i = rowsA[k];
        int c = ciA[k];
        T av = vaA[k];
        unsigned long long o = off[k];
        for (int t = roB[c]; t < roB[c + 1]; ++t) {
            keys[o] = (unsigned long long)i * ncolsB + ciB[t];
            vals[o] = av * vaB[t];
            ++o;
        }
    }
}

template <typename T>
long long spgemm_esc(const int* roA, const int* ciA, const T* vaA, int m,
                     long long nnzA, const int* roB, const int* ciB,
                     const T* vaB, int k, int n, int* ro_c, int* ci_c, T* va_c,
                     hipStream_t s) {
    using K = unsigned long long;
    K* deg = (K*)dev_alloc((nnzA + 1) * sizeof(K), s);
    hipLaunchKernelGGL(expand_degree, dim3(grid_1d(nnzA, AMGX_BLOCK, 4096)),
                       dim3(AMGX_BLOCK), 0, s, ciA, roB, nnzA, deg);
    size_t tmp_bytes = 0;
    rocprim::exclusive_scan(nullptr, tmp_bytes, deg, deg, (K)0, nnzA + 1,
                            rocprim::plus<K>(), s);
    void* tmp = dev_alloc(tmp_bytes, s);
    rocprim::exclusive_scan(tmp, tmp_bytes, deg, deg, (K)0, nnzA + 1,
                            rocprim::plus<K>(), s);
    K total = 0;
    HIP_CHECK(hipMemcpyAsync(&total, deg + nnzA, sizeof(K),
                             hipMemcpyDeviceToHost, s));
    HIP_CHECK(hipStreamSynchronize(s));
    dev_free(tmp, s);
    if (total == 0) {
        HIP_CHECK(hipMemsetAsync(ro_c, 0, (m + 1) * sizeof(int), s));
        dev_free(deg, s);
        return 0;
    }
    int* rowsA = (int*)dev_alloc(nnzA * sizeof(int), s);
    hipLaunchKernelGGL(fill_row_ids, dim3(grid_1d(m)), dim3(AMGX_BLOCK), 0, s,
                       roA, m, rowsA);
    K* keys = (K*)dev_alloc(total * sizeof(K) * 2, s);
    K* keys_alt = keys + total;
    T* vals = (T*)dev_alloc(total * sizeof(T) * 2, s);
    T* vals_alt = vals + total;
    hipLaunchKernelGGL((expand_fill<T>), dim3(grid_1d(nnzA, AMGX_BLOCK, 4096)),
                       dim3(AMGX_BLOCK), 0, s, rowsA, ciA, vaA, roB, ciB, vaB,
                       nnzA, deg, (long long)n, keys, vals);
    size_t tmp2 = 0;
    rocprim::radix_sort_pairs(nullptr, tmp2, keys, keys_alt, vals, vals_alt,
                              total, 0, 64, s);
    void* tmpb = dev_alloc(tmp2, s);
    rocprim::radix_sort_pairs(tmpb, tmp2, keys, keys_alt, vals, vals_alt,
                              total, 0, 64, s);
    unsigned int* nruns = (unsigned int*)dev_alloc(sizeof(unsigned int), s);
    size_t tmp3 = 0;
    rocprim::reduce_by_key(nullptr, tmp3, keys_alt, vals_alt, total, keys,
                           va_c, nruns, rocprim::plus<T>(),
                           rocprim::equal_to<K>(), s);
    void* tmpc = dev_alloc(tmp3, s);
    rocprim::reduce_by_key(tmpc, tmp3, keys_alt, vals_alt, total, keys, va_c,
                           nruns, rocprim::plus<T>(), rocprim::equal_to<K>(),
                           s);
    unsigned int h_runs = 0;
    HIP_CHECK(hipMemcpyAsync(&h_runs, nruns, sizeof(unsigned int),
                             hipMemcpyDeviceToHost, s));
    HIP_CHECK(hipStreamSynchronize(s));
    if (h_runs == 0)
        HIP_CHECK(hipMemsetAsync(ro_c, 0, (m + 1) * sizeof(int), s));
    hipLaunchKernelGGL(keys_to_csr, dim3(grid_1d(h_runs, AMGX_BLOCK, 4096)),
                       dim3(AMGX_BLOCK), 0, s, keys, (long long)h_runs,
                       (long long)n, (long long)m, ro_c, ci_c);
    dev_free(tmpb, s); dev_free(tmpc, s); dev_free(nruns, s);
    dev_free(vals, s); dev_free(keys, s); dev_free(rowsA, s); dev_free(deg, s);
    return (long long)h_runs;
}

template <typename T>
__global__ __launch_bounds__(AMGX_BLOCK) void gather_vals_rows(const int* __restrict__ perm,
                                 const T* __restrict__ va,
                                 const int* __restrict__ rows, long long nnz,
                                 T* __restrict__ va_t, int* __restrict__ ci_t) {
    long long stride = (long long)gridDim.x * blockDim.x;
    for (long long t = (long long)blockIdx.x * blockDim.x + threadIdx.x;
         t < nnz; t += stride) {
        int p = perm[t];
        va_t[t] = va[p];
        ci_t[t] = rows[p];
    }
}

__global__ __launch_bounds__(AMGX_BLOCK) void cols_to_ro(const int* __restrict__ cols_sorted, long long nnz,
                           int n, int* __restrict__ ro_t) {
    long long stride = (long long)gridDim.x * blockDim.x;
    for (long long t = (long long)blockIdx.x * blockDim.x + threadIdx.x;
         t < nnz; t += stride) {
        int c = cols_sorted[t];
        int cprev = (t == 0) ? -1 : cols_sorted[t - 1];
        if (c != cprev)
            for (int q = cprev + 1; q <= c; ++q) ro_t[q] = (int)t;
        if (t == nnz - 1)
            for (int q = c + 1; q <= n; ++q) ro_t[q] = (int)nnz;
    }
}

__global__ __launch_bounds__(AMGX_BLOCK) void iota_kernel(int* p, long long n) {
    long long stride = (long long)gridDim.x * blockDim.x;
    for (long long t = (long long)blockIdx.x * blockDim.x + threadIdx.x; t < n;
         t += stride)
        p[t] = (int)t;
}

template <typename T>
void transpose_csr(const int* ro, const int* ci, const T* va, int m, int n,
                   long long nnz, int* ro_t, int* ci_t, T* va_t,
                   hipStream_t s) {
    if (nnz == 0) {
        HIP_CHECK(hipMemsetAsync(ro_t, 0, (n + 1) * sizeof(int), s));
        return;
    }
    int* rows = (int*)dev_alloc(nnz * sizeof(int), s);
    hipLaunchKernelGGL(fill_row_ids, dim3(grid_1d(m)), dim3(AMGX_BLOCK), 0, s,
                       ro, m, rows);
    int* cols = (int*)dev_alloc(nnz * sizeof(int) * 2, s);
    int* cols_alt = cols + nnz;
    int* perm = (int*)dev_alloc(nnz * sizeof(int) * 2, s);
    int* perm_alt = perm + nnz;
    HIP_CHECK(hipMemcpyAsync(cols, ci, nnz * sizeof(int),
                             hipMemcpyDeviceToDevice, s));
    hipLaunchKernelGGL(iota_kernel, dim3(grid_1d(nnz, AMGX_BLOCK, 4096)),
                       dim3(AMGX_BLOCK), 0, s, perm, nnz);
    size_t tmp_bytes = 0;
    rocprim::radix_sort_pairs(nullptr, tmp_bytes, cols, cols_alt, perm,
                              perm_alt, nnz, 0, 32, s);
    void* tmp = dev_alloc(tmp_bytes, s);
    rocprim::radix_sort_pairs(tmp, tmp_bytes, cols, cols_alt, perm, perm_alt,
                              nnz, 0, 32, s);
    hipLaunchKernelGGL((gather_vals_rows<T>),
                       dim3(grid_1d(nnz, AMGX_BLOCK, 4096)), dim3(AMGX_BLOCK),
                       0, s, perm_alt, va, rows, nnz, va_t, ci_t);
    hipLaunchKernelGGL(cols_to_ro, dim3(grid_1d(nnz, AMGX_BLOCK, 4096)),
                       dim3(AMGX_BLOCK), 0, s, cols_alt, nnz, n, ro_t);
    dev_free(tmp, s); dev_free(perm, s); dev_free(cols, s); dev_free(rows, s);
}

template <bool UPPER>
__device__ __forceinline__ bool slab_split_keep(int j, int n, int c,
                                                const int* __restrict__ colors) {
    if (j >= n) return false;
    return UPPER ? colors[j] > c : colors[j] < c;
}

template <bool UPPER>
__global__ __launch_bounds__(AMGX_BLOCK) void slab_split_count_kernel(
    const int* __restrict__ ro_s, const int* __restrict__ ci_s,
    const int* __restrict__ rows, const int* __restrict__ colors, int n,
    int* __restrict__ counts) {
    int t = blockIdx.x * blockDim.x + threadIdx.x;
    if (t > n) return;
    int cnt = 0;
    if (t < n) {
        int c = colors[rows[t]];
        for (int k = ro_s[t]; k < ro_s[t + 1]; ++k)
            cnt += slab_split_keep<UPPER>(ci_s[k], n, c, colors) ? 1 : 0;
    }
    counts[t] = cnt;
}

template <bool UPPER>
__global__ __launch_bounds__(AMGX_BLOCK) void slab_split_fill_kernel(
    const int* __restrict__ ro_s, const int* __restrict__ ci_s,
    const int* __restrict__ rows, const int* __restrict__ colors, int n,
    const int* __restrict__ ro_x, int* __restrict__ ci_x,
    int* __restrict__ map_x) {
    int t = blockIdx.x * blockDim.x + threadIdx.x;
    if (t >= n) return;
    int c = colors[rows[t]];
    int o = ro_x[t];
    for (int k = ro_s[t]; k < ro_s[t + 1]; ++k) {
        int j = ci_s[k];
        if (slab_split_keep<UPPER>(j, n, c, colors)) {
            ci_x[o] = j;
            map_x[o] = k;
            ++o;
        }
    }
}

long long slab_split_count(const int* ro_s, const int* ci_s, const int* rows,
                           const int* colors, int n, bool upper, int* ro_x,
                           hipStream_t s) {
    auto kern = upper ? slab_split_count_kernel<true>
                      : slab_split_count_kernel<false>;
    hipLaunchKernelGGL(kern, dim3(grid_1d((long long)n + 1)),
                       dim3(AMGX_BLOCK), 0, s, ro_s, ci_s, rows, colors, n,
                       ro_x);
    size_t tmp_bytes = 0;
    rocprim::exclusive_scan(nullptr, tmp_bytes, ro_x, ro_x, 0, (size_t)n + 1,
                            rocprim::plus<int>(), s);
    void* tmp = dev_alloc(tmp_bytes, s);
    rocprim::exclusive_scan(tmp, tmp_bytes, ro_x, ro_x, 0, (size_t)n + 1,
                            rocprim::plus<int>(), s);
    int total = 0;
    HIP_CHECK(hipMemcpyAsync(&total, ro_x + n, sizeof(int),
                             hipMemcpyDeviceToHost, s));
    HIP_CHECK(hipStreamSynchronize(s));
    dev_free(tmp, s);
    return (long long)total;
}

void slab_split_fill(const int* ro_s, const int* ci_s, const int* rows,
                     const int* colors, int n, bool upper, const int* ro_x,
                     int* ci_x, int* map_x, hipStream_t s) {
    if (n <= 0) return;
    auto kern = upper ? slab_split_fill_kernel<true>
                      : slab_split_fill_kernel<false>;
    hipLaunchKernelGGL(kern, dim3(grid_1d(n)), dim3(AMGX_BLOCK), 0, s, ro_s,
                       ci_s, rows, colors, n, ro_x, ci_x, map_x);
}

#define INSTANTIATE_SETUP(T)                                                   \
    AMGX_INSTANTIATE(agg_propose, T)                                           \
    AMGX_INSTANTIATE(agg_merge_singletons, T)                                  \
    AMGX_INSTANTIATE(pairwise_weights, T)                                      \
    AMGX_INSTANTIATE(galerkin_agg, T)                                         \
    AMGX_INSTANTIATE(spgemm_esc, T)
#define INSTANTIATE_SETUP_REAL(T) AMGX_INSTANTIATE(transpose_csr, T)

AMGX_VALUE_TYPES(INSTANTIATE_SETUP)
AMGX_REAL_TYPES(INSTANTIATE_SETUP_REAL)

}
```

amgx_amd/ops/__init__.py:

```python

from __future__ import annotations

import torch


def _backend(obj):
    is_cuda = obj.is_cuda if isinstance(obj, torch.Tensor) else obj.is_cuda
    if is_cuda:
        from . import gpu
        return gpu
    from . import cpu
    return cpu


def compute_diag_index(A):
    return _backend(A).compute_diag_index(A)


def extract_diagonal(A):
    return _backend(A).extract_diagonal(A)


def _mgr(A):
    m = getattr(A, "manager", None)
    return m if (m is not None and m.neighbors) else None


def spmv(A, x, y=None, alpha=1.0, beta=0.0, row_begin=0, row_end=-1):
    B = _backend(A)
    mgr = _mgr(A)
    if mgr is None:
        return B.spmv(A, x, y, alpha, beta, row_begin, row_end)
    assert row_begin == 0 and row_end < 0, "windowed distributed spmv: internal"
    if y is None:
        y = _new_dist_vec(A, x)
    reqs = mgr.exchange_halo(x, async_start=True) or []
    B.spmv(A, x, y, alpha, beta, 0, mgr.boundary_start)
    for rq in reqs:
        rq.wait()
    B.spmv(A, x, y, alpha, beta, mgr.boundary_start, A.n_rows)
    return y


def _new_dist_vec(A, like):
    import torch
    return torch.zeros(A.manager.ext_size, dtype=like.dtype,
                       device=like.device)


def residual(A, x, b, r=None):
    B = _backend(A)
    mgr = _mgr(A)
    if mgr is None:
        return B.residual(A, x, b, r)
    if r is None:
        r = _new_dist_vec(A, b)
    reqs = mgr.exchange_halo(x, async_start=True) or []
    B.residual(A, x, b, r, 0, mgr.boundary_start)
    for rq in reqs:
        rq.wait()
    B.residual(A, x, b, r, mgr.boundary_start, A.n_rows)
    return r


def dot(x, y):
    return _backend(x).dot(x, y)


def nrm2(x):
    return _backend(x).nrm2(x)


def nrm1(x):
    return _backend(x).nrm1(x)


def nrmmax(x):
    return _backend(x).nrmmax(x)


def axpy(y, x, alpha):
    return _backend(x).axpy(y, x, alpha)


def axpby(y, x, alpha, beta):
    return _backend(x).axpby(y, x, alpha, beta)


def scal(x, alpha):
    return _backend(x).scal(x, alpha)


def jacobi_dinv(A, l1: bool = False):
    return _backend(A).jacobi_dinv(A, l1)


def jacobi_smooth(A, dinv, b, x_in, x_out, omega: float):
    mgr = _mgr(A)
    if mgr is not None:
        mgr.exchange_halo(x_in)
    return _backend(A).jacobi_smooth(A, dinv, b, x_in, x_out, omega)


def gs_smooth_color(A, dinv, b, x, color_rows, omega: float):
    return _backend(A).gs_smooth_color(A, dinv, b, x, color_rows, omega)


def gs_sweep(A, dinv, b, x, coloring, omega: float, symmetric: bool = False):
    mgr = _mgr(A)
    if mgr is not None:
        mgr.exchange_halo(x)
    return _backend(A).gs_sweep(A, dinv, b, x, coloring, omega, symmetric)


def color_matrix(A, max_uncolored_frac: float = 0.0, seed: int = 0,
                 multihash_rounds: int = 0):
    B = _backend(A)
    if multihash_rounds:
        return B.color_matrix(A, max_uncolored_frac, seed,
                              multihash_rounds=multihash_rounds)
    return B.color_matrix(A, max_uncolored_frac, seed)


def size2_matching(A, max_iterations: int = 15, deterministic: bool = True,
                   seed: int = 0):
    return _backend(A).size2_matching(A, max_iterations, deterministic, seed)


def pairwise_weights(A, formula: int = 0):
    return _backend(A).pairwise_weights(A, formula)


def pairwise_matching(row_offsets, col_indices, w, n, sizes, cap,
                      merge_singletons, max_iterations, max_unassigned, seed):
    return _backend(w).pairwise_matching(
        row_offsets, col_indices, w, n, sizes, cap, merge_singletons,
        max_iterations, max_unassigned, seed)


def galerkin_aggregation(A, aggregates, num_aggregates, agg_col=None,
                         ncols_mod=None, generator=None):
    return _backend(A).galerkin_aggregation(A, aggregates, num_aggregates,
                                            agg_col, ncols_mod, generator)


def restrict_agg(r, aggregates, num_aggregates, block_dim: int = 1,
                 structure=None, out=None):
    return _backend(r).restrict_agg(r, aggregates, num_aggregates, block_dim,
                                    structure, out)


def prolongate_agg(x, xc, aggregates, block_dim: int = 1):
    return _backend(x).prolongate_agg(x, xc, aggregates, block_dim)


def spgemm(A, B):
    return _backend(A).spgemm(A, B)


def transpose(A):
    return _backend(A).transpose(A)


def galerkin_rap(R, A, P):
    return _backend(A).galerkin_rap(R, A, P)


def truncate_rows(P, trunc_factor: float = 0.0, max_elements: int = -1):
    return _backend(P).truncate_rows(P, trunc_factor, max_elements)


def dilu_setup(A, coloring):
    return _backend(A).dilu_setup(A, coloring)


def dilu_solve(A, Einv, coloring, r, relaxation, x):
    return _backend(A).dilu_solve(A, Einv, coloring, r, relaxation, x)


def ilu1_pattern(A, coloring):
    return _backend(A).ilu1_pattern(A, coloring)


def dense_solve(Ainv, b, x):
    return _backend(b).dense_solve(Ainv, b, x)
```

amgx_amd/ops/cpu.py:

```python

from __future__ import annotations

import numpy as np
import scipy.sparse as sp
import torch


def _np(x: torch.Tensor) -> np.ndarray:
    return x.detach().numpy()


def _real_only(A, feature: str):
    if A.values.is_complex():
        raise NotImplementedError(
            f"{feature} is not available in the complex modes")


def _work_dtype(A):
    return np.complex128 if A.values.is_complex() else np.float64


def _csr(A) -> sp.csr_matrix:
    m = A.to_scipy()
    if not sp.issparse(m):
# ... 166 lines not shown
        rb = r.reshape(-1)[:n_owned].reshape(-1, bd, 1).to(dinv.dtype)
        upd = torch.bmm(dinv, rb).reshape(-1).to(x_in.dtype)
    xo = x_out.reshape(-1)
    xo[:n_owned] = x_in.reshape(-1)[:n_owned] + omega * upd
    xo[n_owned:] = x_in.reshape(-1)[n_owned:]
    return x_out


def gs_sweep(A, dinv, b, x, coloring, omega, symmetric=False):
    for c in range(coloring.num_colors):
        gs_smooth_color(A, dinv, b, x, coloring.rows_of(c), omega)
    if symmetric:
        for c in range(coloring.num_colors - 1, -1, -1):
            gs_smooth_color(A, dinv, b, x, coloring.rows_of(c), omega)
    return x


def gs_smooth_color(A, dinv, b, x, color_rows, omega: float):
    m = _csr(A) if A.block_dim == 1 else A.to_scipy()
    rows = _np(color_rows).astype(np.int64)
    bd = A.block_dim
    if bd == 1:
        sub = m[rows, :] @ _np(x).reshape(-1)
        upd = omega * _np(dinv)[rows] * (_np(b).reshape(-1)[rows] - sub)
        _np(x).reshape(-1)[rows] += upd
    else:
        xv = _np(x).reshape(-1)
        rowsb = (rows[:, None] * bd + np.arange(bd)[None, :]).reshape(-1)
        sub = (m @ xv)[rowsb]
        res = (_np(b).reshape(-1)[rowsb] - sub).reshape(-1, bd, 1)
        upd = np.matmul(_np(dinv)[rows].astype(res.dtype), res).reshape(-1)
        xv[rowsb] += omega * upd
    return x


def color_matrix(A, max_uncolored_frac: float = 0.0, seed: int = 0):
    ro = _np(A.row_offsets).astype(np.int64)
    ci = _np(A.col_indices).astype(np.int64)
    n = A.n_rows
    rows = np.repeat(np.arange(n), np.diff(ro))
    keep = (rows != ci) & (ci < n)
    er, ec = rows[keep], ci[keep]
    x = (np.arange(n, dtype=np.uint64)
         + np.uint64((seed * 0x9E3779B97F4A7C15) % (1 << 64)))
    x = x * np.uint64(0xBF58476D1CE4E5B9)
    w = x ^ (x >> np.uint64(31))
    colors = np.full(n, -1, dtype=np.int32)
    isolated = np.ones(n, dtype=bool)
    isolated[er] = False
    colors[isolated] = 0
    guard = 0
    while (colors < 0).any():
        guard += 1
        if guard > n + 2:
            raise RuntimeError("coloring did not converge")
        un = colors < 0
        act = un[er] & un[ec]
        beaten = np.zeros(n, dtype=bool)
        np.logical_or.at(beaten, er[act], w[ec[act]] > w[er[act]])
        cand = un & ~beaten
        nb_colored = colors[ec] >= 0
        used = np.zeros(n, dtype=np.uint64)
        sel = nb_colored & cand[er]
        np.bitwise_or.at(used, er[sel],
                         np.uint64(1) << colors[ec[sel]].astype(np.uint64))
        free = (~used).astype(np.uint64)
        low = (free & (~free + np.uint64(1)))
        c_new = np.zeros(n, dtype=np.int32)
        nz = low > 0
        c_new[nz] = (np.log2(low[nz].astype(np.float64))).astype(np.int32)
        big = cand & ~nz
        if big.any():
            mx = np.zeros(n, dtype=np.int32)
            np.maximum.at(mx, er[sel], colors[ec[sel]])
            c_new[big] = mx[big] + 1
        colors[cand] = c_new[cand]
    num = int(colors.max()) + 1 if n else 0
    return torch.from_numpy(colors), num


def _strength_weights(A):
    m = _csr(A) if A.block_dim == 1 else _block_norm_csr(A)
    if m.shape[1] != m.shape[0]:
        m = m[:, :m.shape[0]]
    ad = np.abs(m.diagonal())
    ad = np.where(ad > 0, ad, 1.0)
    absm = abs(m.tocsr())
    w = 0.5 * (absm + absm.T).tocsr()
    dinv = 1.0 / np.sqrt(ad)
    w = sp.diags(dinv) @ w @ sp.diags(dinv)
    w = w.tocsr()
    w.setdiag(0.0)
    w.eliminate_zeros()
    return w


def _block_norm_csr(A) -> sp.csr_matrix:
    _real_only(A, "a block matrix (Frobenius block norms)")
    vals = _np(A.values)
    norms = np.sqrt((vals.astype(np.float64) ** 2).sum(axis=(1, 2)))
    return sp.csr_matrix((norms, _np(A.col_indices).astype(np.int64),
                          _np(A.row_offsets).astype(np.int64)),
                         shape=(A.n_rows, A.n_cols))


def size2_matching(A, max_iterations: int = 15, deterministic: bool = True,
                   seed: int = 0):
    w = _strength_weights(A).tocoo()
    n = A.n_rows
    er = w.row.astype(np.int64)
    ec = w.col.astype(np.int64)
    ew = w.data.astype(np.float64)
    keep = er != ec
    er, ec, ew = er[keep], ec[keep], ew[keep]
    agg = np.full(n, -1, dtype=np.int64)
    rng = np.random.RandomState(seed)
    tie = rng.rand(n)
    next_id = 0
    for _ in range(max_iterations):
        if not (agg < 0).any():
            break
        un = agg < 0
        act = un[er] & un[ec]
        if not act.any():
            break
        ar, ac, aw = er[act], ec[act], ew[act]
        order = np.lexsort((tie[ac], aw, ar))
        prop = np.full(n, -1, dtype=np.int64)
        prop[ar[order]] = ac[order]
        cand = np.nonzero(prop >= 0)[0]
        mutual = cand[(prop[prop[cand]] == cand) & (cand < prop[cand])]
        if mutual.size == 0:
            break
        ids = next_id + np.arange(mutual.size)
        agg[mutual] = ids
        agg[prop[mutual]] = ids
        next_id += int(mutual.size)
    left = agg < 0
    if left.any():
        sel = left[er] & (agg[ec] >= 0)
        if sel.any():
            sr, sc, sw = er[sel], ec[sel], ew[sel]
            order = np.lexsort((np.arange(sr.size), sw, sr))
            join = np.full(n, -1, dtype=np.int64)
            join[sr[order]] = sc[order]
            can_join = left & (join >= 0)
            agg[can_join] = agg[join[can_join]]
        singles = np.nonzero(agg < 0)[0]
        agg[singles] = next_id + np.arange(singles.size)
        next_id += int(singles.size)
    return torch.from_numpy(agg.astype(np.int32)), int(next_id)


_U32 = 0xFFFFFFFF


def _hash_u32(a: int, seed: int) -> int:
    a = (a ^ seed) & _U32
    a = ((a ^ 61) ^ (a >> 16)) & _U32
    a = (a * 9) & _U32
    a ^= a >> 4
    a = (a * 0x27D4EB2D) & _U32
    a ^= a >> 15
    return a


def _pair_hash(i: int, j: int, seed: int) -> int:
    lo, hi = min(i, j), max(i, j)
    return _hash_u32(_hash_u32(lo, seed) ^ hi, seed)


def _absd(v) -> float:
    if isinstance(v, complex):
        return float(np.sqrt(np.float64(v.real) * np.float64(v.real)
                             + np.float64(v.imag) * np.float64(v.imag)))
    return abs(v)


def pairwise_weights(A, formula: int = 0) -> torch.Tensor:
    if formula not in (0, 1):
        raise ValueError("weight_formula must be 0 or 1")
    if A.values.is_complex() and A.block_dim > 1:
        raise NotImplementedError(
            "aggregation of a block matrix is not available in the complex "
            "modes")
    if formula == 1 and (A.values.is_complex() or A.block_dim > 1):
        raise NotImplementedError(
            "weight_formula 1 is signed: scalar real matrices only")
    n = A.n_rows
    ro = _np(A.row_offsets).astype(np.int64)
    ci = _np(A.col_indices).astype(np.int64)
    vals = _np(A.values)
    if A.block_dim > 1:
        vals = np.sqrt((vals.astype(np.float64) ** 2).sum(axis=(1, 2)))
    va = [complex(v) if np.iscomplexobj(vals) else float(v) for v in vals]
    pos = [{int(ci[k]): k for k in range(ro[i], ro[i + 1])} for i in range(n)]
    diag = [va[pos[i][i]] if i in pos[i] else 0.0 for i in range(n)]
    w = np.zeros(ci.size, dtype=np.float64)
    for i in range(n):
        for k in range(ro[i], ro[i + 1]):
            j = int(ci[k])
            if j == i or j >= n or i not in pos[j]:
                continue
            t = pos[j][i]
            if formula == 0:
                m = max(_absd(diag[i]), _absd(diag[j]))
                if m > 0.0:
                    w[k] = 0.5 * (_absd(va[k]) + _absd(va[t])) / m
            elif diag[i] != 0.0 and diag[j] != 0.0:
                w[k] = -0.5 * (va[k] / diag[i] + va[t] / diag[j])
    return torch.from_numpy(w)


def pairwise_matching(row_offsets, col_indices, w, n, sizes, cap,
                      merge_singletons, max_iterations, max_unassigned, seed):
    if merge_singletons not in (0, 1, 2):
        raise ValueError("merge_singletons must be 0, 1 or 2")
    ro = [int(v) for v in _np(row_offsets)]
    ci = [int(v) for v in _np(col_indices)]
    w = [float(v) for v in _np(w)]
    cur = [int(v) for v in _np(sizes)]
    seed = int(seed) & 0x7FFFFFFF
    cap =int(cap) if cap and cap > 0 else None
    agg = [-1] * n

    def edges(i):
        for k in range(ro[i], ro[i + 1]):
            if ci[k] != i and ci[k] < n and w[k] > 0.0:
                yield k, ci[k]

    def key(i, k):
        j = ci[k]
        return (w[k], _pair_hash(i, j, seed), min(i, j), max(i, j))

    def largest(i, ok):
        best = None
        for k, j in edges(i):
            if ok(j) and (best is None or key(i, k) > key(i, best)):
                best = k
        return best

    def fits(i, r):
        return cap is None or cur[i] + cur[r] <= cap

    un, rounds = n, 0
    while (rounds < max_iterations and un > 0
           and not un < max_unassigned * n):
        prop = [-1] * n
        for i in range(n):
            if agg[i] < 0:
                k = largest(i, lambda j: agg[j] < 0 and fits(i, j))
                prop[i] = ci[k] if k is not None else i
        pairs = 0
        for i in range(n):
            j = prop[i]
            if j > i and prop[j] == i:
                agg[i] = agg[j] = i
                cur[i] += cur[j]
                pairs += 1
        rounds += 1
        if pairs == 0:
            break
        un -= 2 * pairs

    if merge_singletons == 1:
        while True:
            new = list(agg)
            for i in range(n):
                if agg[i] < 0:
                    k = largest(i, lambda j: agg[j] >= 0)
                    if k is not None:
                        new[i] = agg[ci[k]]
                        cur[new[i]] += cur[i]
            if new == agg:
                break
            agg = new
    elif merge_singletons == 2:
        while True:
            bids = {}
            for i in range(n):
                if agg[i] < 0:
                    k = largest(i, lambda j: agg[j] >= 0 and fits(i, agg[j]))
                    if k is not None:
                        bids.setdefault(agg[ci[k]], []).append((w[k], i))
            if not bids:
                break
            for r, lst in bids.items():
                wmax = max(wk for wk, _ in lst)
                i = min(i for wk, i in lst if wk == wmax)
                agg[i] = r
                cur[r] += cur[i]
    for i in range(n):
        if agg[i] < 0:
            agg[i] = i

    roots = [i for i in range(n) if agg[i] == i]
    ids = {r: t for t, r in enumerate(roots)}
    out = np.array([ids[a] for a in agg], dtype=np.int32).reshape(n)
    szs = np.array([cur[r] for r in roots], dtype=np.int32).reshape(len(roots))
    return (torch.from_numpy(out), len(roots), torch.from_numpy(szs), rounds)


def galerkin_aggregation(A, aggregates, num_aggregates, agg_col=None,
                         ncols_mod=None, generator=None):
    from ..matrix import CSRMatrix
    agg = _np(aggregates).astype(np.int64)
    n = A.n_rows
    bd = A.block_dim
    if agg_col is not None:
        aggc = _np(agg_col).astype(np.int64)
        ro = _np(A.row_offsets).astype(np.int64)
        ci = _np(A.col_indices).astype(np.int64)
        vals = _np(A.values)
        rows = np.repeat(np.arange(n), np.diff(ro))
        I, J = agg[rows], aggc[ci]
        key = I * int(ncols_mod) + J
        order = np.argsort(key, kind="stable")
        key_s = key[order]
        uniq, start = np.unique(key_s, return_index=True)
        if bd == 1:
            sums = np.add.reduceat(vals[order], start)
        else:
            sums = np.add.reduceat(vals[order], start, axis=0)
        ro_c = np.zeros(num_aggregates + 1, dtype=np.int64)
        np.add.at(ro_c, (uniq // int(ncols_mod)) + 1, 1)
        ro_c = np.cumsum(ro_c)
        ci_c = (uniq % int(ncols_mod)).astype(np.int32)
        if bd == 1:
            out = CSRMatrix(torch.from_numpy(ro_c.astype(np.int32)),
                            torch.from_numpy(ci_c),
                            torch.from_numpy(sums).to(A.dtype),
                            n_cols=int(ncols_mod))
        else:
            out = CSRMatrix(torch.from_numpy(ro_c.astype(np.int32)),
                            torch.from_numpy(ci_c),
                            torch.from_numpy(sums).to(A.dtype),
                            n_cols=int(ncols_mod), block_dim=bd)
        return out
    if bd == 1:
        m = _csr(A)
        P = sp.csr_matrix((np.ones(n), (np.arange(n), agg)),
                          shape=(n, num_aggregates))
        Ac = (P.T @ m @ P).tocsr()
        Ac.sort_indices()
        return CSRMatrix.from_scipy(Ac, dtype=A.dtype)
    ro = _np(A.row_offsets).astype(np.int64)
    ci = _np(A.col_indices).astype(np.int64)
    vals = _np(A.values)
    rows = np.repeat(np.arange(n), np.diff(ro))
    I, J = agg[rows], agg[ci]
    key = I * num_aggregates + J
    order = np.argsort(key, kind="stable")
    key_s = key[order]
    uniq, start = np.unique(key_s, return_index=True)
    out = np.add.reduceat(vals[order], start, axis=0)
    ro_c = np.zeros(num_aggregates + 1, dtype=np.int32)
    np.add.at(ro_c, (uniq // num_aggregates) + 1, 1)
    ro_c = np.cumsum(ro_c).astype(np.int32)
    return type(A).from_bsr(ro_c, (uniq % num_aggregates).astype(np.int32), out,
                            n_cols=num_aggregates, dtype=A.dtype)


def restrict_agg(r, aggregates, num_aggregates, block_dim: int = 1,
                 structure=None, out=None):
    agg = aggregates.to(torch.int64)
    r = r.reshape(-1)[:agg.numel() * block_dim]
    if out is not None and out.dtype == r.dtype:
        rc = out.reshape(-1)[:num_aggregates * block_dim].zero_()
    else:
        rc = torch.zeros(num_aggregates * block_dim, dtype=r.dtype)
    if block_dim == 1:
        rc.index_add_(0, agg, r.reshape(-1))
    else:
        idx = (agg[:, None] * block_dim +
               torch.arange(block_dim, dtype=torch.int64)[None, :]).reshape(-1)
        rc.index_add_(0, idx, r.reshape(-1))
    if out is not None and out.dtype != r.dtype:
        out.reshape(-1)[:rc.numel()].copy_(rc)
    return rc


def prolongate_agg(x, xc, aggregates, block_dim: int = 1):
    agg = aggregates.to(torch.int64)
    xo = x.reshape(-1)[:agg.numel() * block_dim]
    if block_dim == 1:
        xo.add_(xc.reshape(-1)[agg])
    else:
        idx = (agg[:, None] * block_dim +
               torch.arange(block_dim, dtype=torch.int64)[None, :]).reshape(-1)
        xo.add_(xc.reshape(-1)[idx])
    return x


def spgemm(A, B):
    from ..matrix import CSRMatrix
    C = (_csr(A) @ _csr(B)).tocsr()
    C.sum_duplicates()
    C.sort_indices()
    return CSRMatrix.from_scipy(C, dtype=A.dtype)


def transpose(A):
    from ..matrix import CSRMatrix
    return CSRMatrix.from_scipy(_csr(A).T.tocsr(), dtype=A.dtype)


def galerkin_rap(R, A, P):
    from ..matrix import CSRMatrix
    C = (_csr(R) @ _csr(A) @ _csr(P)).tocsr()
    C.sum_duplicates()
    C.sort_indices()
    return CSRMatrix.from_scipy(C, dtype=A.dtype)


def truncate_rows(P, trunc_factor: float = 0.0, max_elements: int = -1):
    from ..matrix import CSRMatrix
    if not (0.0 < trunc_factor < 1.0):
        trunc_factor = 0.0
    if trunc_factor <= 0.0 and max_elements < 0:
        return P
    _real_only(P, "interpolation truncation")
    m = _csr(P).copy()
    n = m.shape[0]
    data, indices, indptr = m.data, m.indices, m.indptr
    new_data, new_idx, new_ptr = [], [], [0]
    for i in range(n):
        s, e = indptr[i], indptr[i + 1]
        d, c = data[s:e], indices[s:e]
        if d.size:
            rs_old = d.sum()
            keep = np.abs(d) >= trunc_factor * np.abs(d).max()
            d2, c2 = d[keep], c[keep]
            if max_elements >= 0 and d2.size > max_elements:
                top = np.argsort(-np.abs(d2), kind="stable")[:max_elements]
                top.sort()
                d2, c2 = d2[top], c2[top]
            rs_new = d2.sum()
            if rs_new != 0 and rs_old != 0:
                d2 = d2 * (rs_old / rs_new)
            new_data.append(d2)
            new_idx.append(c2)
        new_ptr.append(new_ptr[-1] + (len(new_data[-1]) if d.size else 0))
    out = sp.csr_matrix((np.concatenate(new_data) if new_data else np.zeros(0),
                         np.concatenate(new_idx) if new_idx else np.zeros(0, dtype=int),
                         np.asarray(new_ptr)), shape=m.shape)
    return CSRMatrix.from_scipy(out, dtype=P.dtype)


def dilu_setup(A, coloring):
    bd = A.block_dim
    colors = _np(coloring.colors).astype(np.int64)
    if bd == 1:
        m = _csr(A)
        if m.shape[1] != m.shape[0]:
            m = m[:, :m.shape[0]].tocsr()
        wd = _work_dtype(A)
        if A.values.is_complex():
            coo = m.tocoo()
            clash = (coo.row != coo.col) & (colors[coo.row] == colors[coo.col])
            if clash.any():
                raise RuntimeError(
                    "dilu_setup: the coloring is not a valid distance-1 "
                    f"coloring of the matrix ({int(clash.sum())} couplings "
                    "join rows of one color)")
        d = m.diagonal().astype(wd)
        B = m.multiply(m.T).tocsr()
        einv = np.zeros(A.n_rows, dtype=wd)
        done = np.zeros(A.n_rows, dtype=np.float64)
        for c in range(coloring.num_colors):
            rows = np.nonzero(colors == c)[0]
            e = d[rows] - (B[rows, :] @ (einv * done))
            dref = np.where(d[rows] != 0.0, d[rows], 1.0)
            bad = np.abs(e) < 1e-10 * np.abs(dref)
            e = np.where(bad, dref, e)
            einv[rows] = 1.0 / e
            done[rows] = 1.0
        return torch.from_numpy(einv).to(A.dtype)
    _real_only(A, "a block matrix (block DILU)")
    ro = _np(A.row_offsets).astype(np.int64)
    ci = _np(A.col_indices).astype(np.int64)
    vals = _np(A.values).astype(np.float64)
    D = _np(extract_diagonal(A)).astype(np.float64).copy()
    has_diag = _np(A.diag_index()) >= 0
    tau = dilu_pivot_floor(A.dtype)
    AT = transpose_block_index(A)
    einv = np.zeros_like(D)
    with np.errstate(all="ignore"):
        for c in range(coloring.num_colors):
            rows = np.nonzero(colors == c)[0]
            for i in rows:
                E = D[i].copy()
                for k in range(ro[i], ro[i + 1]):
                    j = ci[k]
                    if j != i and j < A.n_rows and colors[j] < c \
                            and AT[k] >= 0:
                        E -= vals[k] @ einv[j] @ vals[AT[k]]
                einv[i] = _dilu_block_inverse(
                    E, D[i] if has_diag[i] else None, tau)
    return torch.from_numpy(einv).to(A.dtype)


def dilu_pivot_floor(dtype) -> float:
    return 1e-5 if dtype in (torch.float32, np.float32) else 1e-10


def _dilu_block_inverse(E, D, tau):
    dmax = float(np.abs(D).max()) if D is not None else 0.0
    emax = float(np.fmax.reduce(np.abs(E).ravel(), initial=0.0))
    inv, pmin = _gauss_jordan_inv(E[None])
    if emax <= 1e10 * (dmax + 1.0) \
            and pmin[0] >= tau * (dmax if dmax > 0.0 else 1.0):
        return inv[0]
    if D is None:
        return np.eye(E.shape[0])
    return _gauss_jordan_inv(D[None])[0][0]


def transpose_block_index(A) -> np.ndarray:
    ro = _np(A.row_offsets).astype(np.int64)
    ci = _np(A.col_indices).astype(np.int64)
    n = A.n_rows
    rows = np.repeat(np.arange(n), np.diff(ro))
    ncols = max(int(A.n_cols), n)
    keys = rows * ncols + ci
    order = np.argsort(keys, kind="stable")
    skeys = keys[order]
    valid = ci < n
    want = np.where(valid, ci * ncols + rows, -1)
    pos = np.searchsorted(skeys, want)
    pos = np.minimum(pos, skeys.size - 1)
    found = valid & (skeys[pos] == want)
    out = np.where(found, order[pos], -1).astype(np.int64)
    return out


def dilu_solve(A, Einv, coloring, r, relaxation, x):
    bd = A.block_dim
    colors = _np(coloring.colors).astype(np.int64)
    m = A.to_scipy()
    if bd != 1:
        _real_only(A, "a block matrix (block DILU)")
    wd = np.complex128 if (A.values.is_complex() or r.is_complex()) \
        else np.float64
    rv = _np(r).reshape(-1).astype(wd)
    w = np.zeros_like(rv)
    ei = _np(Einv).astype(wd)
    nc = coloring.num_colors
    def rowsb(rows):
        return (rows[:, None] * bd + np.arange(bd)[None, :]).reshape(-1)
    mc = m.tocsr()
    for c in range(nc):
        rows = np.nonzero(colors == c)[0]
        rb = rowsb(rows)
        tmp = rv[rb] - (mc[rb, :] @ w)
        if bd == 1:
            w[rb] = ei[rows] * tmp
        else:
            w[rb] = np.matmul(ei[rows], tmp.reshape(-1, bd, 1)).reshape(-1)
    z = w.copy()
    later = np.zeros_like(w)
    for c in range(nc - 1, -1, -1):
        rows = np.nonzero(colors == c)[0]
        rb = rowsb(rows)
        s = mc[rb, :] @ later
        if bd == 1:
            z[rb] = w[rb] - ei[rows] * s
        else:
            z[rb] = w[rb] - np.matmul(ei[rows], s.reshape(-1, bd, 1)).reshape(-1)
        later[rb] = z[rb]
    _np(x).reshape(-1)[:z.size] += relaxation * z
    return x


def dense_solve(Ainv, b, x):
    wd = torch.complex128 if (Ainv.is_complex() or b.is_complex()) \
        else torch.float64
    x.reshape(-1).copy_((Ainv.to(wd) @ b.reshape(-1).to(wd)).to(x.dtype))
    return x


def ilu0_setup(A, coloring):
    _real_only(A, "MULTICOLOR_ILU")
    if A.block_dim != 1:
        return _ilu0_setup_block(A, coloring)
    ro = _np(A.row_offsets).astype(np.int64)
    ci = _np(A.col_indices).astype(np.int64)
    vals = _np(A.values).astype(np.float64).copy()
    colors = _np(coloring.colors).astype(np.int64)
    n = A.n_rows
    order = np.lexsort((np.arange(n), colors))
    pos = np.full(A.n_cols, np.iinfo(np.int64).max, dtype=np.int64)
    pos[order] = np.arange(n)
    lut = {}
    for i in range(n):
        for k in range(ro[i], ro[i + 1]):
            lut[(i, ci[k])] = k
    for i in order:
        row_ks = sorted((pos[ci[k]], k) for k in range(ro[i], ro[i + 1]))
        for pk, kidx in row_ks:
            k = ci[kidx]
            if pk >= pos[i]:
                continue
            ukk = vals[lut[(k, k)]]
            if ukk == 0.0:
                ukk = 1.0
            vals[kidx] /= ukk
            lik = vals[kidx]
# ... 260 lines not shown
```

amgx_amd/ops/gpu.py:

```python

from __future__ import annotations

import math

import torch

try:
    from .. import _core
except ImportError as e:
    raise ImportError(
        "amgx_amd._core (gfx950 HIP extension) is not built. Run "
        "`PYTORCH_ROCM_ARCH=gfx950 python setup.py build_ext --inplace` "
        f"at the repo root. Underlying error: {e}") from e


def _didx(A):
    if A._diag_idx is None:
        A._diag_idx = _core.diag_index(A.row_offsets, A.col_indices, A.n_rows)
    return A._diag_idx


def _tidx(A):
    t = A._cache.get("tidx")
    if t is None:
        t = _core.trans_index(A.row_offsets, A.col_indices, A.n_rows)
        A._cache["tidx"] = t
    return t


def _scratch(A, name, numel, dtype=None):
    dtype = dtype if dtype is not None else A.dtype
    key = ("scratch", name, numel, dtype)
    t = A._cache.get(key)
    if t is None:
        t = torch.empty(numel, dtype=dtype, device=A.device)
        A._cache[key] = t
    return t


MAX_BLOCK_DIM = 16


def _check_block_dim(A, name):
    if not 1 <= A.block_dim <= MAX_BLOCK_DIM:
        raise ValueError(
            f"{name}: block_dim {A.block_dim} is outside the supported range "
            f"1..{MAX_BLOCK_DIM} of the block smoother kernels")


def compute_diag_index(A):
    return _didx(A)


def extract_diagonal(A):
    if A.diag is not None:
        return A.diag
    return _core.extract_diag(A.row_offsets, A.col_indices, A.values,
                              _didx(A), A.n_rows, A.block_dim)


def spmv(A, x, y=None, alpha=1.0, beta=0.0, row_begin=0, row_end=-1):
    assert A.diag is None, \
        "external DIAG matrices must be folded at upload (capi does this)"
    if row_end < 0:
        row_end = A.n_rows
    if y is None:
        y = torch.zeros(A.n_rows * A.block_dim, dtype=x.dtype, device=x.device)
        beta = 0.0
    _core.csrmv(A.row_offsets, A.col_indices, A.values, A.block_dim,
                x.reshape(-1), y.reshape(-1), None, alpha, beta, 0.0,
                row_begin, row_end)
    return y


def residual(A, x, b, r=None, row_begin=0, row_end=-1):
    if r is None:
        r = torch.empty_like(b)
    if row_end < 0:
        row_end = A.n_rows
    _core.csrmv(A.row_offsets, A.col_indices, A.values, A.block_dim,
                x.reshape(-1), r.reshape(-1), b.reshape(-1), -1.0, 0.0, 1.0,
                row_begin, row_end)
    return r


def _coef(v, alpha):
    return complex(alpha) if v.is_complex() else float(alpha)


_RED_DOT, _RED_L1, _RED_LMAX, _RED_ABS2 = range(4)


def dot(x, y):
    r = _core.reduce_op(x.reshape(-1), y.reshape(-1), _RED_DOT).item()
    return complex(r) if x.is_complex() else float(r)


def nrm2(x):
    if x.is_complex():
        return math.sqrt(float(_core.reduce_op(x.reshape(-1), None,
                                               _RED_ABS2).item()))
    return math.sqrt(max(float(_core.reduce_op(x.reshape(-1), x.reshape(-1),
                                               _RED_DOT).item()), 0.0))


def nrm1(x):
    return float(_core.reduce_op(x.reshape(-1), None, _RED_L1).item())


def nrmmax(x):
    return float(_core.reduce_op(x.reshape(-1), None, _RED_LMAX).item())


def dot_async(x, y):
    if x.is_complex():
        raise TypeError("dot_async is real-only (complex modes use dot)")
    return _core.reduce_op(x.reshape(-1), y.reshape(-1), _RED_DOT)


def axpy_dalpha(y, x, alpha, scale=1.0):
    _core.axpy_dalpha(y.reshape(-1), x.reshape(-1), alpha.reshape(-1),
                      float(scale))
    return y


def scal_drsqrt(x, s2):
    _core.scal_drsqrt(x.reshape(-1), s2.reshape(-1))
    return x


def axpy(y, x, alpha):
    _core.axpy(y.reshape(-1), x.reshape(-1), _coef(x, alpha))
    return y


def axpby(y, x, alpha, beta):
    _core.axpby(y.reshape(-1), x.reshape(-1), _coef(x, alpha),
                _coef(x, beta))
    return y


def scal(x, alpha):
    _core.scal(x.reshape(-1), _coef(x, alpha))
    return x


def jacobi_dinv(A, l1: bool = False):
    _check_block_dim(A, "jacobi_dinv")
    if l1 and A.values.is_complex():
        raise NotImplementedError(
            "JACOBI_L1 is not available in the complex modes (dZZI / dCCI / "
            "dZCI): the device l1 diagonal is real-only")
    return _core.jacobi_dinv(A.row_offsets, A.col_indices, A.values, _didx(A),
                             A.n_rows, A.block_dim, bool(l1))


def jacobi_smooth(A, dinv, b, x_in, x_out, omega: float):
    _core.jacobi_smooth(A.row_offsets, A.col_indices, A.values, A.block_dim,
                        dinv, b.reshape(-1), x_in.reshape(-1),
                        x_out.reshape(-1), float(omega))
    return x_out


def gs_smooth_color(A, dinv, b, x, color_rows, omega: float):
    _check_block_dim(A, "gs_smooth_color")
    _core.gs_smooth_rows(A.row_offsets, A.col_indices, A.values, A.block_dim,
                         dinv, b.reshape(-1), x.reshape(-1), color_rows,
                         float(omega))
    return x


def gs_sweep(A, dinv, b, x, coloring, omega: float, symmetric: bool = False):
    _check_block_dim(A, "gs_sweep")
    if A.block_dim == 1:
        st = _slabs(A, coloring)
        va_s = _slab_copy(st, "gs_va", A.values, lambda v: v[st.nzmap])
        dinv_s = _slab_copy(st, "gs_dinv", dinv,
                            lambda d: d.reshape(-1)[st.perm])
        _core.gs_sweep_sorted(st.ro_s, st.ci_s, va_s, dinv_s, b.reshape(-1),
                              x.reshape(-1), coloring.rows_sorted,
                              coloring.bounds, coloring.bounds_dev,
                              float(omega), bool(symmetric))
        return x
    _core.gs_sweep(A.row_offsets, A.col_indices, A.values, A.block_dim, dinv,
                   b.reshape(-1), x.reshape(-1), coloring.rows_sorted,
                   coloring.bounds, float(omega), bool(symmetric))
    return x


def color_matrix(A, max_uncolored_frac: float = 0.0, seed: int = 0,
                 multihash_rounds: int = 0):
    colors, nc = _core.color_minmax(A.row_offsets, A.col_indices, A.n_rows,
                                    4096, int(seed), int(multihash_rounds))
    return colors, int(nc)


class _Slabs:
    __slots__ = ("coloring", "ro_s", "ci_s", "nzmap", "perm", "slot_of_row",
                 "copies", "upper", "lower")


def _slabs(A, coloring):
    st = A._cache.get("slabs")
    if st is None or st.coloring is not coloring:
        st = _Slabs()
        st.coloring = coloring
        st.copies = {}
        st.upper = st.lower = None
        n = A.n_rows
        perm = coloring.rows_sorted.to(torch.int64)
        ro64 = A.row_offsets.to(torch.int64)
        deg = ro64[1:] - ro64[:-1]
        counts = deg[perm]
        total = int(A.nnz)
        st.ro_s = torch.zeros(n + 1, dtype=torch.int32, device=A.device)
        csum = torch.cumsum(counts, 0)
        st.ro_s[1:] = csum.to(torch.int32)
        st.nzmap = (torch.repeat_interleave(ro64[perm], counts)
                    + torch.arange(total, device=A.device, dtype=torch.int64)
                    - torch.repeat_interleave(csum - counts, counts))
        st.ci_s = A.col_indices[st.nzmap].contiguous()
        st.perm = perm
        st.slot_of_row = torch.empty(n, dtype=torch.int32, device=A.device)
        st.slot_of_row[perm] = torch.arange(n, dtype=torch.int32,
                                            device=A.device)
        A._cache["slabs"] = st
    return st


def _slab_copy(st, name, src, gather):
    key = (src.data_ptr(), src._version)
    hit = st.copies.get(name)
    if hit is None or hit[0] != key:
        hit = (key, gather(src))
        st.copies[name] = hit
    return hit[1]


def _slab_part(st, upper):
    part = st.upper if upper else st.lower
    if part is None:
        part = tuple(_core.slab_split(st.ro_s, st.ci_s,
                                      st.coloring.rows_sorted,
                                      st.coloring.colors, bool(upper)))
        if upper:
            st.upper = part
        else:
            st.lower = part
    return part


def _split_path(A):
    return A.block_dim == 1 and A.n_rows > _core.DILU_SMALL_ROWS


class DiluState:
    __slots__ = ("einv", "va_s", "einv_s", "va_u", "va_l")

    def __init__(self, einv, va_s, einv_s, va_u=None):
        self.einv = einv
        self.va_s = va_s
        self.einv_s = einv_s
        self.va_u = va_u
        self.va_l = None

    def cpu(self):
        return self.einv.cpu()


def _check_dilu_coloring(A, coloring):
    n = A.n_rows
    ro = A.row_offsets.to(torch.int64)
    rows = torch.repeat_interleave(
        torch.arange(n, dtype=torch.int64, device=A.device), ro[1:] - ro[:-1])
    cols = A.col_indices.to(torch.int64)
    off = (cols != rows) & (cols < n)
    colors = coloring.colors.to(torch.int64)
    clash = off & (colors[rows] == colors[cols.clamp(max=n - 1)])
    if bool(clash.any()):
        raise RuntimeError(
            "dilu_setup: the coloring is not a valid distance-1 coloring of "
            f"the matrix ({int(clash.sum())} couplings join rows of one "
            "color)")


def dilu_setup(A, coloring):
    _check_block_dim(A, "dilu_setup")
    if A.values.is_complex():
        _check_dilu_coloring(A, coloring)
    einv = _core.dilu_setup(A.row_offsets, A.col_indices, A.values,
                            A.block_dim, _didx(A), _tidx(A), coloring.colors,
                            coloring.rows_sorted, coloring.bounds)
    st = _slabs(A, coloring)
    bb = A.block_dim * A.block_dim
    va_s = A.values.reshape(A.nnz, -1)[st.nzmap].reshape(-1).contiguous()
    einv_s = einv.reshape(A.n_rows, bb)[st.perm].reshape(-1).contiguous() \
        if A.block_dim > 1 else einv[st.perm].contiguous()
    va_u = _gather_part(va_s, _slab_part(st, True)) if A.block_dim == 1 \
        else None
    return DiluState(einv, va_s, einv_s, va_u)


def _gather_part(va_s, part):
    out = torch.empty(part[2].numel(), dtype=va_s.dtype, device=va_s.device)
    _core.gather(va_s, part[2], 1, out)
    return out


DILU_FORMS = ("split", "small", "small_full", "stream")


def _dilu_sorted(A, Einv, coloring, rhs, x, relaxation, fused, lanes=0,
                 sweeps=1, form=None):
    _check_block_dim(A, "dilu_solve / dilu_smooth")
    n = A.n_cols * A.block_dim
    w = _scratch(A, "dilu_w", n, x.dtype)
    st = _slabs(A, coloring)
    forced = form is not None
    if A.block_dim != 1:
        if lanes or forced:
            raise ValueError("lanes and form select among the scalar DILU "
                             "sweeps; a block level does not run them")
        form = "block"
    elif form is None:
        form = "split" if _split_path(A) else "small"
    elif form not in DILU_FORMS:
        raise ValueError(f"form must be one of {DILU_FORMS}")
    if form in ("split", "small", "stream"):
        ro_u, ci_u, _ = _slab_part(st, True)
        y = None
        if fused:
            fwd = (st.ro_s, st.ci_s, Einv.va_s)
            y = _scratch(A, "dilu_y", n, x.dtype)
        else:
            ro_l, ci_l, _ = part = _slab_part(st, False)
            if Einv.va_l is None:
                Einv.va_l = _gather_part(Einv.va_s, part)
            fwd = (ro_l, ci_l, Einv.va_l)
        if form == "small":
            _core.dilu_small(*fwd, ro_u, ci_u, Einv.va_u, Einv.einv_s,
                             coloring.rows_sorted, coloring.bounds,
                             coloring.bounds_dev, rhs.reshape(-1), w,
                             x.reshape(-1), float(relaxation), fused,
                             int(lanes), y, int(sweeps), forced)
            return
        for _ in range(sweeps):
            _core.dilu_split(*fwd, ro_u, ci_u, Einv.va_u, Einv.einv_s,
                             coloring.rows_sorted, coloring.bounds,
                             rhs.reshape(-1), w, x.reshape(-1),
                             float(relaxation), fused, int(lanes), y,
                             2 if form == "stream" else 0)
        return
    if lanes:
        raise ValueError("lanes selects the form of the split-slab sweeps; "
                         "the full-slab apply has one")
    z = _scratch(A, "dilu_z", n, x.dtype)
    for _ in range(sweeps):
        _core.dilu_sorted(st.ro_s, st.ci_s, Einv.va_s, A.block_dim,
                          Einv.einv_s, coloring.rows_sorted, coloring.bounds,
                          coloring.bounds_dev, rhs.reshape(-1), w, z,
                          x.reshape(-1), float(relaxation), fused, forced)


def dilu_smooth(A, Einv, coloring, b, x, relaxation, lanes=0, sweeps=1,
                form=None):
    if A.block_dim not in (1, 4):
        return False
    if getattr(A, "manager", None) is not None:
        return False
    _dilu_sorted(A, Einv, coloring, b, x, relaxation, True, lanes, sweeps,
                 form)
    return True


def dilu_solve(A, Einv, coloring, r, relaxation, x, lanes=0, sweeps=1,
               form=None):
    _dilu_sorted(A, Einv, coloring, r, x, relaxation, False, lanes, sweeps,
                 form)
    return x


def size2_matching(A, max_iterations: int = 15, deterministic: bool = True,
                   seed: int = 0):
    if A.block_dim > 1 and A.values.is_complex():
        raise NotImplementedError(
            "aggregation of a block matrix is not available in the complex "
            "modes (dZZI / dCCI / dZCI)")
    diag = extract_diagonal(A)
    if A.block_dim > 1:
        diag = torch.linalg.vector_norm(diag.reshape(A.n_rows, -1), dim=1)
        va = torch.linalg.vector_norm(
            A.values.reshape(A.nnz, -1).to(torch.float64), dim=1).to(A.dtype)
        roots = _core.size2_match(A.row_offsets, A.col_indices, va, _tidx(A),
                                  diag.to(A.dtype), A.n_rows, max_iterations,
                                  int(seed) + 0x9E3779B1)
    else:
        roots = _core.size2_match(A.row_offsets, A.col_indices, A.values,
                                  _tidx(A), diag, A.n_rows, max_iterations,
                                  int(seed) + 0x9E3779B1)
    uniq, agg = torch.unique(roots, sorted=True, return_inverse=True)
    return agg.to(torch.int32), int(uniq.numel())


def pairwise_weights(A, formula: int = 0):
    if A.block_dim > 1 and A.values.is_complex():
        raise NotImplementedError(
            "aggregation of a block matrix is not available in the complex "
            "modes (dZZI / dCCI / dZCI)")
    if formula == 1 and (A.values.is_complex() or A.block_dim > 1):
        raise NotImplementedError(
            "weight_formula 1 is signed: scalar real matrices only")
    if A.block_dim > 1:
        va = torch.linalg.vector_norm(
            A.values.reshape(A.nnz, -1).to(torch.float64), dim=1)
        didx = _didx(A).long()
        diag = torch.where(didx >= 0, va[didx.clamp(min=0)],
                           torch.zeros((), dtype=va.dtype, device=va.device))
    else:
        va, diag = A.values, extract_diagonal(A)
    return _core.pairwise_weights(A.row_offsets, A.col_indices, va, _tidx(A),
                                  diag.contiguous(), A.n_rows, int(formula))


def pairwise_matching(row_offsets, col_indices, w, n, sizes, cap,
                      merge_singletons, max_iterations, max_unassigned, seed,
                      lanes: int = 0):
    agg, num, szs, rounds = _core.pairwise_match(
        row_offsets, col_indices, w, int(n), sizes, int(cap or 0),
        int(merge_singletons), int(max_iterations), float(max_unassigned),
        int(seed) & 0x7FFFFFFF, int(lanes))
    return agg, int(num), szs, int(rounds)


def galerkin_aggregation(A, aggregates, num_aggregates, agg_col=None,
                         ncols_mod=None, generator=None):
    from ..matrix import CSRMatrix
    if agg_col is None:
        agg_col = aggregates
    if ncols_mod is None:
        ncols_mod = num_aggregates
    if A.block_dim > 1 and A.values.is_complex():
        raise NotImplementedError(
            "the Galerkin product of a block matrix is not available in the "
            "complex modes (dZZI / dCCI / dZCI)")
    if A.block_dim == 1 and generator != "THRUST":
        agg64 = aggregates.to(torch.int64)
        counts = torch.bincount(agg64, minlength=num_aggregates)
        m_ro = torch.zeros(num_aggregates + 1, dtype=torch.int64,
                           device=A.device)
        m_ro[1:] = torch.cumsum(counts, 0)
        fids = torch.argsort(agg64, stable=True).to(torch.int32)
        ro, ci, va, big = _core.spgemm_hash(
            m_ro.to(torch.int32), fids, A.values,
            A.row_offsets, A.col_indices, A.values,
            agg_col, 1, max(A.nnz, 1),
            64 if A.nnz <= 48 * max(num_aggregates, 1) else 512)
        if int(ro[0].item()) != -1:
            if big.numel():
                _sort_unsorted_rows(ro, ci, va, big)
            return CSRMatrix(ro, ci.contiguous(), va.contiguous(),
                             n_cols=int(ncols_mod), block_dim=1)
    ro_c, ci_c, va_c = _core.galerkin_agg(A.row_offsets, A.col_indices,
                                          A.values, aggregates, agg_col,
                                          num_aggregates, int(ncols_mod),
                                          A.block_dim)
    out = CSRMatrix(ro_c, ci_c.contiguous(), va_c.contiguous(),
                    n_cols=int(ncols_mod), block_dim=A.block_dim)
    return out


def restrict_agg(r, aggregates, num_aggregates, block_dim: int = 1,
                 structure=None, out=None):
    nc = num_aggregates * block_dim
    if out is None or out.dtype != r.dtype:
        rc = torch.empty(nc, dtype=r.dtype, device=r.device)
    else:
        rc = out.reshape(-1)[:nc]
    if structure is not None:
        off, fids = structure
        _core.restrict_csr(r.reshape(-1), off, fids, block_dim, rc)
    else:
        _core.restrict_agg(r.reshape(-1), aggregates, block_dim, rc)
    if out is not None and out.dtype != r.dtype:
        out.reshape(-1)[:nc].copy_(rc)
    return rc


def prolongate_agg(x, xc, aggregates, block_dim: int = 1):
    _core.prolongate_agg(x.reshape(-1), xc.reshape(-1), aggregates, block_dim)
    return x


def _expansion_bound(A, B):
    degB = (B.row_offsets[1:] - B.row_offsets[:-1]).to(torch.int64)
    return int(degB[A.col_indices.to(torch.int64)].sum().item())


def _sort_unsorted_rows(ro, ci, va, big_rows):
    ro64 = ro.to(torch.int64)
    for r in big_rows.tolist():
        s, e = int(ro64[r]), int(ro64[r + 1])
        order = torch.argsort(ci[s:e])
        ci[s:e] = ci[s:e][order]
        if va is not None:
            va[s:e] = va[s:e][order]


def spgemm(A, B):
    from ..matrix import CSRMatrix
    cap = max(_expansion_bound(A, B), 1)
    cap0 = 64 if cap <= 48 * max(A.n_rows, 1) else 512
    ro, ci, va, big = _core.spgemm_hash(A.row_offsets, A.col_indices,
                                        A.values, B.row_offsets,
                                        B.col_indices, B.values, None, 0,
                                        cap, cap0)
    if int(ro[0].item()) == -1:
        ro, ci, va = _core.spgemm(A.row_offsets, A.col_indices, A.values,
                                  B.row_offsets, B.col_indices, B.values,
                                  B.n_cols, cap)
        return CSRMatrix(ro, ci.contiguous(), va.contiguous(),
                         n_cols=B.n_cols)
    if big.numel():
        _sort_unsorted_rows(ro, ci, va, big)
    return CSRMatrix(ro, ci.contiguous(), va.contiguous(), n_cols=B.n_cols)


def transpose(A):
    from ..matrix import CSRMatrix
    ro, ci, va = _core.transpose(A.row_offsets, A.col_indices, A.values,
                                 A.n_cols)
    return CSRMatrix(ro, ci, va, n_cols=A.n_rows)


def galerkin_rap(R, A, P):
    AP = spgemm(A, P)
    return spgemm(R, AP)


def truncate_rows(P, trunc_factor: float = 0.0, max_elements: int = -1):
    if not (0.0 < trunc_factor < 1.0):
        trunc_factor = 0.0
    if trunc_factor <= 0.0 and max_elements < 0:
        return P
    from ..matrix import CSRMatrix
    ro, ci, va = _core.truncate_rows(P.row_offsets, P.col_indices,
                                     P.values, float(trunc_factor),
                                     int(max_elements))
    return CSRMatrix(ro, ci.contiguous(), va.contiguous(), n_cols=P.n_cols)


def dense_solve(Ainv, b, x):
    _core.dense_gemv(Ainv, b.reshape(-1), x.reshape(-1))
    return x


def strength_ahat(A, theta=0.25, max_row_sum=1.1):
    return _core.strength_ahat(A.row_offsets, A.col_indices, A.values,
                               _didx(A), float(theta), float(max_row_sum))


def _pmis_graph(A, S):
    n = A.n_rows
    ci, tidx = A.col_indices, _tidx(A)
    sym = A._cache.get("tidx_complete")
    if sym is None:
        sym = not bool(((tidx < 0) & (ci < n)).any().item())
        A._cache["tidx_complete"] = sym
    if sym:
        return A.row_offsets, ci, tidx, S
    one_way = (S != 0) & (tidx < 0) & (ci < n)
    if not bool(one_way.any().item()):
        return A.row_offsets, ci, tidx, S
    dev = A.device
    ro64 = A.row_offsets.to(torch.int64)
    rows = torch.repeat_interleave(
        torch.arange(n, dtype=torch.int64, device=dev), ro64[1:] - ro64[:-1])
    ci64 = ci.to(torch.int64)
    sel = (S != 0) & (ci64 != rows) & (ci64 < n)
    r, c = rows[sel], ci64[sel]
    uk, inv = torch.unique(torch.cat([r * n + c, c * n + r]),
                           return_inverse=True)
    flag = torch.zeros(uk.numel(), dtype=torch.uint8, device=dev)
    flag[inv[:r.numel()]] = 1
    g_ro = torch.zeros(n + 1, dtype=torch.int32, device=dev)
    g_ro[1:] = torch.cumsum(torch.bincount(uk // n, minlength=n),
                            0).to(torch.int32)
    g_ci = (uk % n).to(torch.int32).contiguous()
    return g_ro, g_ci, _core.trans_index(g_ro, g_ci, n), flag


def pmis_select(A, S):
    n = A.n_rows
    guard = 8 * (int(math.log2(n + 2)) + 8)
    state = _core.pmis_select(*_pmis_graph(A, S), guard)
    cmask = state == 1
    cf = torch.full((n,), -1, dtype=torch.int32, device=A.device)
    csum = torch.cumsum(cmask.to(torch.int64), 0)
    cf[cmask] = (csum[cmask] - 1).to(torch.int32)
    return cf, int(cmask.sum().item())


def interp_d1(A, S, cf_map, num_coarse):
    from ..matrix import CSRMatrix
    counts = _core.interp_d1_count(A.row_offsets, A.col_indices, S, cf_map)
    p_ro = torch.zeros(A.n_rows + 1, dtype=torch.int32, device=A.device)
    p_ro[1:] = torch.cumsum(counts.to(torch.int64), 0).to(torch.int32)
    p_nnz = int(p_ro[-1].item())
    p_ro, p_ci, p_va = _core.interp_d1(A.row_offsets, A.col_indices, A.values,
                                       S, cf_map, _didx(A), p_ro, p_nnz)
    return CSRMatrix(p_ro, p_ci, p_va, n_cols=num_coarse)


def ilu0_setup(A, coloring):
    _check_block_dim(A, "ilu0_setup")
    pos = _slabs(A, coloring).slot_of_row
    if A.block_dim != 1:
        lu, dinv = _core.ilu0_setup_block(
            A.row_offsets, A.col_indices, A.values.reshape(-1), A.block_dim,
            _didx(A), pos, coloring.rows_sorted, coloring.bounds)
        return (lu, dinv)
    lu = _core.ilu0_setup(A.row_offsets, A.col_indices, A.values, _didx(A),
                          pos, coloring.rows_sorted, coloring.bounds)
    return lu


def ilu1_pattern(A, coloring):
    from ..matrix import CSRMatrix
    colors = coloring.colors.to(torch.int32).contiguous()
    ro, ci, big = _core.ilu1_pattern(A.row_offsets, A.col_indices, colors,
                                     A.n_rows)
    if int(ro[0].item()) == -1:
        from . import cpu
        return cpu.ilu1_pattern(A.to("cpu"), coloring).to(A.device)
    if big.numel():
        _sort_unsorted_rows(ro, ci, None, big)
    bb = A.block_dim * A.block_dim
    va, _ = _core.ilu1_embed(A.row_offsets, A.col_indices,
                             A.values.reshape(-1), bb, ro, ci)
    if A.block_dim != 1:
        va = va.reshape(-1, A.block_dim, A.block_dim)
    return CSRMatrix(ro, ci, va, n_cols=A.n_cols, block_dim=A.block_dim)


def ilu0_solve(A, factors, coloring, r, x, relaxation=1.0):
    _check_block_dim(A, "ilu0_solve")
    n = A.n_cols * A.block_dim
    y = _scratch(A, "ilu_y", n, r.dtype)
    z = _scratch(A, "ilu_z", n, r.dtype)
    st = _slabs(A, coloring)
    if A.block_dim != 1:
        lu, dinv = factors
        _core.ilu0_apply_block(A.row_offsets, A.col_indices, lu, dinv,
                               A.block_dim, st.slot_of_row,
                               coloring.rows_sorted, coloring.bounds,
                               r.reshape(-1), y, z, x.reshape(-1),
                               float(relaxation))
        return x
    lu_s, diag_s = _slab_copy(
        st, "ilu", factors, lambda f: (
            f.reshape(-1)[st.nzmap],
            f.reshape(-1)[_didx(A).to(torch.int64)][st.perm]))
    _core.ilu0_apply_sorted(st.ro_s, st.ci_s, lu_s, diag_s, st.slot_of_row,
                            coloring.rows_sorted, coloring.bounds,
                            r.reshape(-1), y, z, x.reshape(-1),
                            float(relaxation))
    return x
```

setup.py:

```python

import os

from setuptools import setup

os.environ.setdefault("PYTORCH_ROCM_ARCH", "gfx950")

from torch.utils.cpp_extension import BuildExtension, CUDAExtension

here = os.path.dirname(os.path.abspath(__file__))
csrc = os.path.join(here, "amgx_amd", "csrc")

ext = CUDAExtension(
    name="amgx_amd._core",
    sources=[
        os.path.join(csrc, "bindings.cpp"),
        os.path.join(csrc, "kernels_solve.hip"),
        os.path.join(csrc, "kernels_setup.hip"),
        os.path.join(csrc, "kernels_classical.hip"),
        os.path.join(csrc, "kernels_mfma.hip"),
        os.path.join(csrc, "kernels_spgemm.hip"),
    ],
    extra_compile_args={
        "cxx": ["-O3", "-std=c++17"],
        "nvcc": ["-O3", "-std=c++17"],
    },
)

setup(
    name="amgx_amd",
    version="0.1.0",
    packages=["amgx_amd"],
    ext_modules=[ext],
    cmdclass={"build_ext": BuildExtension.with_options(use_ninja=True)},
)
```

Baseline: 1.216 s.

## Move setup orderings to native rocPRIM kernels and batch convergence checks

Replaces torch argsort/bincount/cumsum chains for color ordering, aggregate CSR structure and slab layout with native rocPRIM radix-sort and offset kernels. Coloring and matching loops now launch several rounds before reading the convergence flag back to the host, which cuts device-to-host syncs. Aggregate renumbering replaces torch.unique, the R structure is reused in the Galerkin product, and value gathers use a native kernel. Batched rounds can run extra idle iterations past convergence on small levels.

Measured after the change: 1.121 s (median of 6 runs). 7.9% less time.

```diff
diff --git a/amgx_amd/amg/coloring.py b/amgx_amd/amg/coloring.py
--- a/amgx_amd/amg/coloring.py
+++ b/amgx_amd/amg/coloring.py
@@ -297,6 +297,12 @@
     def __init__(self, colors: torch.Tensor, num_colors: int):
         self.colors = colors
         self.num_colors = num_colors
+        if colors.is_cuda:
+            from ..ops import gpu
+            self.rows_sorted, self.bounds_dev = gpu.color_order(colors,
+                                                                num_colors)
+            self.bounds = self.bounds_dev.cpu().tolist()
+            return
         counts = torch.bincount(colors.to(torch.int64), minlength=num_colors)
         order = torch.argsort(colors.to(torch.int64), stable=True)
         self.rows_sorted = order.to(torch.int32).contiguous()
diff --git a/amgx_amd/amg/level.py b/amgx_amd/amg/level.py
--- a/amgx_amd/amg/level.py
+++ b/amgx_amd/amg/level.py
@@ -89,6 +89,11 @@
                          n_cols=n, block_dim=A.block_dim)
 
     def _build_r_structure(self):
+        if self.aggregates.is_cuda:
+            from ..ops import gpu
+            self.r_structure = gpu.aggregate_csr(self.aggregates,
+                                                 self.num_aggregates)
+            return
         agg = self.aggregates.to(torch.int64)
         order = torch.argsort(agg, stable=True).to(torch.int32)
         counts = torch.bincount(agg, minlength=self.num_aggregates)
@@ -103,7 +108,9 @@
         gen = self.scope.get("coarseAgenerator")
         if mgr is None:
             Ac = ops.galerkin_aggregation(self.A, self.aggregates,
-                                          self.num_aggregates, generator=gen)
+                                          self.num_aggregates, generator=gen,
+                                          structure=getattr(
+                                              self, "r_structure", None))
             Ac = self._color_renumber(Ac)
             geom = self.A._cache.get("geometry")
             if geom is not None:
@@ -165,7 +172,8 @@
         Ac2 = ops.galerkin_aggregation(self.A, self.aggregates,
                                        self.num_aggregates,
                                        generator=self.scope.get(
-                                           "coarseAgenerator"))
+                                           "coarseAgenerator"),
+                                       structure=self.r_structure)
         self._coarse_coloring = MatrixColoring(
             col.colors[perm].contiguous(), col.num_colors)
         Ac2.coloring = self._coarse_coloring
@@ -178,7 +186,9 @@
         Ac = ops.galerkin_aggregation(self.A, self.aggregates,
                                       self.num_aggregates,
                                       generator=self.scope.get(
-                                          "coarseAgenerator"))
+                                          "coarseAgenerator"),
+                                      structure=getattr(self, "r_structure",
+                                                        None))
         coloring = getattr(self, "_coarse_coloring", None)
         if coloring is not None and Ac.values.is_cuda:
             Ac.coloring = coloring
diff --git a/amgx_amd/csrc/bindings.cpp b/amgx_amd/csrc/bindings.cpp
--- a/amgx_amd/csrc/bindings.cpp
+++ b/amgx_amd/csrc/bindings.cpp
@@ -656,49 +656,91 @@
     });
 }
 
+constexpr int64_t ROUND_SLOTS = 512;
+int64_t round_batch(int64_t n, int64_t batch) {
+    TORCH_CHECK(batch >= 0, "batch must be 0 (by level size) or positive");
+    if (batch > 0) return std::min(batch, ROUND_SLOTS);
+    if (n >= (int64_t(1) << 22)) return 1;
+    if (n >= (int64_t(1) << 20)) return 2;
+    if (n >= (int64_t(1) << 18)) return 4;
+    return 8;
+}
+
+template <typename Round>
+bool run_rounds(int64_t max_rounds, int64_t k, const Tensor& like,
+                Round round) {
+    auto slots = torch::zeros({ROUND_SLOTS},
+                              like.options().dtype(torch::kInt32));
+    int64_t rounds = 0, used = 0;
+    while (rounds < max_rounds) {
+        int64_t kk = std::min(k, max_rounds - rounds);
+        if (used + kk > ROUND_SLOTS) {
+            slots.zero_();
+            used = 0;
+        }
+        for (int64_t r = 0; r < kk; ++r, ++rounds)
+            round(rounds, iptr(slots) + used + r);
+        auto host = slots.narrow(0, used, kk).cpu();
+        const int* h = host.data_ptr<int>();
+        for (int64_t r = 0; r < kk; ++r)
+            if (h[r] == 0) return true;
+        used += kk;
+    }
+    return false;
+}
+
 std::tuple<Tensor, int64_t> color_minmax(Tensor ro, Tensor ci, int64_t n,
                                          int64_t max_rounds, int64_t seed,
-                                         int64_t mode1_rounds) {
+                                         int64_t mode1_rounds, int64_t batch) {
+    check_dev(ro);
+    TORCH_CHECK(ro.numel() == n + 1, "color_minmax: ro does not have n rows");
     auto colors = torch::full({n}, -1,
                               ro.options().dtype(torch::kInt32));
+    if (n == 0) return {colors, 0};
     auto colors_next = torch::empty_like(colors);
-    auto counter = torch::zeros({1}, ro.options().dtype(torch::kInt32));
     hipStream_t st = cur_stream();
-    int rounds = 0;
-    for (; rounds < max_rounds; ++rounds) {
-        counter.zero_();
-        int mode = rounds < mode1_rounds ? 1 : 0;
-        amgx_hip::color_minmax_round(
-            iptr(ro), iptr(ci), (int)n, iptr(colors), iptr(colors_next),
-            rounds, (int)(seed + rounds * 7919), mode, iptr(counter), st);
-        std::swap(colors, colors_next);
-        int left = counter.cpu().item<int>();
-        if (left == 0) break;
-    }
-    TORCH_CHECK((colors.min().cpu().item<int>()) >= 0,
-                "MIN_MAX coloring did not converge in ", max_rounds,
+    bool done = run_rounds(
+        max_rounds, round_batch(n, batch), ro, [&](int64_t r, int* left) {
+            int mode = r < mode1_rounds ? 1 : 0;
+            amgx_hip::color_minmax_round(
+                iptr(ro), iptr(ci), (int)n, iptr(colors), iptr(colors_next),
+                (int)r, (int)(seed + r * 7919), mode, left, st);
+            std::swap(colors, colors_next);
+        });
+    TORCH_CHECK(done, "MIN_MAX coloring did not converge in ", max_rounds,
                 " rounds");
-    int64_t ncolors = (colors.max().cpu().item<int>()) + 1;
+    auto top = torch::zeros({1}, ro.options().dtype(torch::kInt32));
+    amgx_hip::int_max(iptr(colors), (int)n, iptr(top), st);
+    int64_t ncolors = top.cpu().item<int>() + 1;
     return {colors, ncolors};
 }
 
 Tensor size2_match(Tensor ro, Tensor ci, Tensor va, Tensor tidx, Tensor diag,
-                   int64_t n, int64_t max_iters, int64_t seed) {
+                   int64_t n, int64_t max_iters, int64_t seed,
+                   int64_t batch, bool weights) {
     auto agg = torch::full({n}, -1, ro.options().dtype(torch::kInt32));
+    if (n == 0) return agg;
     auto prop = torch::empty({n}, ro.options().dtype(torch::kInt32));
-    auto changed = torch::zeros({1}, ro.options().dtype(torch::kInt32));
     hipStream_t st = cur_stream();
     DISPATCH(AMGX_VALUE_TYPES, "size2_match", (va), [&] {
-        for (int it = 0; it < max_iters; ++it) {
+        Tensor w;
+        const double* wpre = nullptr;
+        if (weights) {
+            w = torch::empty({ci.numel()},
+                             ro.options().dtype(torch::kFloat64));
+            amgx_hip::agg_edge_weights<scalar_t>(
+                iptr(ro), iptr(ci), dptr<scalar_t>(va), iptr(tidx),
+                dptr<scalar_t>(diag), (int)n, dptr<double>(w), st);
+            wpre = dptr<double>(w);
+        }
+        run_rounds(max_iters, round_batch(n, batch), ro,
+                   [&](int64_t, int* changed) {
             amgx_hip::agg_propose<scalar_t>(
                 iptr(ro), iptr(ci), dptr<scalar_t>(va), iptr(tidx),
-                dptr<scalar_t>(diag), (int)n, iptr(agg), iptr(prop), (int)seed,
-                st);
-            changed.zero_();
-            amgx_hip::agg_match(iptr(prop), (int)n, iptr(agg), iptr(changed),
-                                st);
-            if (changed.cpu().item<int>() == 0) break;
-        }
+                dptr<scalar_t>(diag), wpre, (int)n, iptr(agg), iptr(prop),
+                (int)seed, st);
+            amgx_hip::agg_match(iptr(prop), (int)n, iptr(agg), changed, st);
+        });
         auto agg_out = torch::empty_like(agg);
         amgx_hip::agg_merge_singletons<scalar_t>(
             iptr(ro), iptr(ci), dptr<scalar_t>(va), iptr(tidx),
@@ -706,6 +748,55 @@
         agg = agg_out;
     });
     return agg;
+}
+
+std::tuple<Tensor, int64_t> size2_renumber(Tensor roots) {
+    check_dev(roots);
+    int64_t n = roots.numel();
+    auto agg = torch::empty({n}, roots.options());
+    auto ids = torch::empty({n + 1}, roots.options());
+    amgx_hip::root_renumber(iptr(roots), (int)n, iptr(ids), iptr(agg),
+                            cur_stream());
+    int64_t num = ids[n].cpu().item<int>();
+    return {agg, num};
+}
+
+std::tuple<Tensor, Tensor> key_order(Tensor keys, int64_t nkeys) {
+    check_dev(keys);
+    TORCH_CHECK(nkeys >= 0 && nkeys < INT_MAX && keys.numel() < INT_MAX,
+                "key_order: sizes out of the int32 range");
+    int64_t n = keys.numel();
+    auto order = torch::empty({n}, keys.options());
+    auto off = torch::empty({std::max<int64_t>(nkeys, 1) + 1}, keys.options());
+    amgx_hip::key_order(iptr(keys), (int)n, (int)nkeys, iptr(order),
+                        iptr(off), cur_stream());
+    return {order, off.narrow(0, 0, nkeys + 1)};
+}
+
+std::vector<Tensor> slab_structure(Tensor ro, Tensor ci, Tensor rows_sorted,
+                                   int64_t lanes) {
+    check_dev(ro);
+    int64_t n = (int64_t)ro.numel() - 1, nnz = ci.numel();
+    TORCH_CHECK(rows_sorted.numel() == n,
+                "slab_structure: rows_sorted does not have n rows");
+    TORCH_CHECK(lanes == 0 || lanes == 1 || lanes == 8,
+                "slab_structure: lanes must be 0 (routed), 1 or 8");
+    hipStream_t st = cur_stream();
+    auto ro_s = torch::empty({n + 1}, ro.options());
+    auto slot = torch::empty({n}, ro.options());
+    long long total = amgx_hip::slab_offsets(iptr(ro), iptr(rows_sorted),
+                                             (int)n, iptr(ro_s), iptr(slot),
+                                             st);
+    TORCH_CHECK(total == nnz, "slab_structure: rows_sorted is no permutation "
+                "of the rows (", total, " entries of ", nnz, ")");
+    auto nzmap = torch::empty({nnz}, ro.options());
+    auto ci_s = torch::empty({nnz}, ro.options());
+    if (lanes == 0)
+        lanes = dilu_lanes((double)nnz / (double)std::max<int64_t>(n, 1),
+                           false);
+    amgx_hip::slab_fill(iptr(ro), iptr(ci), iptr(rows_sorted), (int)n,
+                        (int)lanes, iptr(ro_s), iptr(nzmap), iptr(ci_s), st);
+    return {ro_s, ci_s, nzmap, slot};
 }
 
 Tensor pairwise_weights(Tensor ro, Tensor ci, Tensor va, Tensor tidx,
@@ -1183,8 +1274,19 @@
     m.attr("DILU_STREAM_MIN_ROWS_FULL") = DILU_STREAM_MIN_ROWS_FULL;
     m.attr("DILU_STREAM_MIN_ROWS_SPLIT") = DILU_STREAM_MIN_ROWS_SPLIT;
     m.def("slab_split", &slab_split);
-    m.def("color_minmax", &color_minmax);
-    m.def("size2_match", &size2_match);
+    {
+        using pybind11::arg;
+        m.def("color_minmax", &color_minmax, arg("ro"), arg("ci"), arg("n"),
+              arg("max_rounds"), arg("seed"), arg("mode1_rounds"),
+              arg("batch") = 0);
+        m.def("size2_match", &size2_match, arg("ro"), arg("ci"), arg("va"),
+              arg("tidx"), arg("diag"), arg("n"), arg("max_iters"),
+              arg("seed"), arg("batch") = 0, arg("weights") = false);
+        m.def("slab_structure", &slab_structure, arg("ro"), arg("ci"),
+              arg("rows_sorted"), arg("lanes") = 0);
+    }
+    m.def("size2_renumber", &size2_renumber);
+    m.def("key_order", &key_order);
     m.def("pairwise_weights", &pairwise_weights);
     m.def("pairwise_propose", &pairwise_propose);
     m.def("pairwise_match", &pairwise_match);
diff --git a/amgx_amd/csrc/core_api.h b/amgx_amd/csrc/core_api.h
--- a/amgx_amd/csrc/core_api.h
+++ b/amgx_amd/csrc/core_api.h
@@ -178,12 +178,17 @@
 
 void color_minmax_round(const int* ro, const int* ci, int n,
                         const int* colors_prev, int* colors_next, int iter,
-                        int seed, int mode, int* n_uncolored, hipStream_t s);
+                        int seed, int mode, int* left, hipStream_t s);
+void int_max(const int* v, int n, int* out, hipStream_t s);
 
 template <typename T>
 void agg_propose(const int* ro, const int* ci, const T* va, const int* tidx,
-                 const T* diag, int n, const int* agg, int* prop, int seed,
-                 hipStream_t s);
+                 const T* diag, const double* wpre, int n, const int* agg,
+                 int* prop, int seed, hipStream_t s);
+template <typename T>
+void agg_edge_weights(const int* ro, const int* ci, const T* va,
+                      const int* tidx, const T* diag, int n, double* w,
+                      hipStream_t s);
 void agg_match(const int* prop, int n, int* agg, int* changed, hipStream_t s);
 template <typename T>
 void agg_merge_singletons(const int* ro, const int* ci, const T* va,
@@ -213,6 +218,16 @@
                        void* tmp, size_t tmp_bytes, int* agg_out,
                        int* sizes_out, hipStream_t s);
 
+void key_order(const int* keys, int n, int nkeys, int* order, int* off,
+               hipStream_t s);
+void root_renumber(const int* roots, int n, int* ids, int* agg,
+                   hipStream_t s);
+long long slab_offsets(const int* ro, const int* rows, int n, int* ro_s,
+                       int* slot_of_row, hipStream_t s);
+void slab_fill(const int* ro, const int* ci, const int* rows, int n,
+               int lanes, const int* ro_s, int* nzmap, int* ci_s,
+               hipStream_t s);
+
 long long slab_split_count(const int* ro_s, const int* ci_s, const int* rows,
                            const int* colors, int n, bool upper, int* ro_x,
                            hipStream_t s);
diff --git a/amgx_amd/csrc/kernels_order.hip b/amgx_amd/csrc/kernels_order.hip
--- /dev/null
+++ b/amgx_amd/csrc/kernels_order.hip
@@ -0,0 +1,165 @@
+
+#include <cstring>
+
+#include <rocprim/rocprim.hpp>
+
+#include <stdexcept>
+#include <string>
+
+#include "common.h"
+#include "core_api.h"
+
+namespace amgx_hip {
+
+namespace {
+
+void* order_alloc(size_t bytes, hipStream_t s) {
+    void* p = nullptr;
+    if (bytes == 0) bytes = 16;
+    HIP_CHECK(hipMallocAsync(&p, bytes, s));
+    return p;
+}
+void order_free(void* p, hipStream_t s) { HIP_CHECK(hipFreeAsync(p, s)); }
+
+void scan_exclusive(int* v, size_t count, hipStream_t s) {
+    size_t tmp_bytes = 0;
+    HIP_CHECK(rocprim::exclusive_scan(nullptr, tmp_bytes, v, v, 0, count,
+                                      rocprim::plus<int>(), s));
+    void* tmp = order_alloc(tmp_bytes, s);
+    HIP_CHECK(rocprim::exclusive_scan(tmp, tmp_bytes, v, v, 0, count,
+                                      rocprim::plus<int>(), s));
+    order_free(tmp, s);
+}
+
+}
+
+__global__ __launch_bounds__(AMGX_BLOCK) void keys_to_offsets_kernel(
+    const int* __restrict__ sorted, int n, int nkeys, int* __restrict__ off) {
+    int t = blockIdx.x * blockDim.x + threadIdx.x;
+    if (t >= n) return;
+    int c = min(max(sorted[t], 0), nkeys - 1);
+    int cprev = t == 0 ? -1 : min(max(sorted[t - 1], 0), nkeys - 1);
+    for (int q = cprev + 1; q <= c; ++q) off[q] = t;
+    if (t == n - 1)
+        for (int q = c + 1; q <= nkeys; ++q) off[q] = n;
+}
+
+__global__ __launch_bounds__(AMGX_BLOCK) void fill_int_kernel(
+    int* __restrict__ p, int count, int v) {
+    int t = blockIdx.x * blockDim.x + threadIdx.x;
+    if (t < count) p[t] = v;
+}
+
+void key_order(const int* keys, int n, int nkeys, int* order, int* off,
+               hipStream_t s) {
+    if (nkeys < 1) nkeys = 1;
+    if (n <= 0) {
+        hipLaunchKernelGGL(fill_int_kernel, dim3(grid_1d(nkeys + 1)),
+                           dim3(AMGX_BLOCK), 0, s, off, nkeys + 1, 0);
+        return;
+    }
+    unsigned bits = 1;
+    while (bits < 31 && (1ll << bits) < (long long)nkeys) ++bits;
+    int* sorted = (int*)order_alloc((size_t)n * sizeof(int), s);
+    rocprim::counting_iterator<int> rows(0);
+    size_t tmp_bytes = 0;
+    HIP_CHECK(rocprim::radix_sort_pairs(nullptr, tmp_bytes, keys, sorted, rows,
+                                        order, (size_t)n, 0u, bits, s));
+    void* tmp = order_alloc(tmp_bytes, s);
+    HIP_CHECK(rocprim::radix_sort_pairs(tmp, tmp_bytes, keys, sorted, rows,
+                                        order, (size_t)n, 0u, bits, s));
+    hipLaunchKernelGGL(keys_to_offsets_kernel, dim3(grid_1d(n)),
+                       dim3(AMGX_BLOCK), 0, s, sorted, n, nkeys, off);
+    order_free(tmp, s);
+    order_free(sorted, s);
+}
+
+__global__ __launch_bounds__(AMGX_BLOCK) void root_flag_kernel(
+    const int* __restrict__ roots, int n, int* __restrict__ ids) {
+    int i = blockIdx.x * blockDim.x + threadIdx.x;
+    if (i > n) return;
+    ids[i] = (i < n && roots[i] == i) ? 1 : 0;
+}
+
+__global__ __launch_bounds__(AMGX_BLOCK) void root_map_kernel(
+    const int* __restrict__ roots, int n, const int* __restrict__ ids,
+    int* __restrict__ agg) {
+    int i = blockIdx.x * blockDim.x + threadIdx.x;
+    if (i >= n) return;
+    int r = roots[i];
+    agg[i] = ids[min(max(r, 0), n - 1)];
+}
+
+void root_renumber(const int* roots, int n, int* ids, int* agg,
+                   hipStream_t s) {
+    hipLaunchKernelGGL(root_flag_kernel, dim3(grid_1d((long long)n + 1)),
+                       dim3(AMGX_BLOCK), 0, s, roots, n, ids);
+    scan_exclusive(ids, (size_t)n + 1, s);
+    if (n <= 0) return;
+    hipLaunchKernelGGL(root_map_kernel, dim3(grid_1d(n)), dim3(AMGX_BLOCK), 0,
+                       s, roots, n, ids, agg);
+}
+
+__global__ __launch_bounds__(AMGX_BLOCK) void slab_lengths_kernel(
+    const int* __restrict__ ro, const int* __restrict__ rows, int n,
+    int* __restrict__ ro_s, int* __restrict__ slot_of_row) {
+    int t = blockIdx.x * blockDim.x + threadIdx.x;
+    if (t > n) return;
+    int len = 0;
+    if (t < n) {
+        int i = rows[t];
+        len = ro[i + 1] - ro[i];
+        slot_of_row[i] = t;
+    }
+    ro_s[t] = len;
+}
+
+template <int LANES>
+__global__ __launch_bounds__(AMGX_BLOCK) void slab_fill_kernel(
+    const int* __restrict__ ro, const int* __restrict__ ci,
+    const int* __restrict__ rows, int n, const int* __restrict__ ro_s,
+    int* __restrict__ nzmap, int* __restrict__ ci_s) {
+    long long g = (long long)blockIdx.x * blockDim.x + threadIdx.x;
+    long long t = g / LANES;
+    int lane = (int)(g % LANES);
+    if (t >= n) return;
+    int src = ro[rows[t]];
+    int dst = ro_s[t];
+    int len = ro_s[t + 1] - dst;
+    for (int e = lane; e < len; e += LANES) {
+        nzmap[dst + e] = src + e;
+        ci_s[dst + e] = ci[src + e];
+    }
+}
+
+long long slab_offsets(const int* ro, const int* rows, int n, int* ro_s,
+                       int* slot_of_row, hipStream_t s) {
+    hipLaunchKernelGGL(slab_lengths_kernel, dim3(grid_1d((long long)n + 1)),
+                       dim3(AMGX_BLOCK), 0, s, ro, rows, n, ro_s,
+                       slot_of_row);
+    scan_exclusive(ro_s, (size_t)n + 1, s);
+    int total = 0;
+    HIP_CHECK(hipMemcpyAsync(&total, ro_s + n, sizeof(int),
+                             hipMemcpyDeviceToHost, s));
+    HIP_CHECK(hipStreamSynchronize(s));
+    return (long long)total;
+}
+
+void slab_fill(const int* ro, const int* ci, const int* rows, int n,
+               int lanes, const int* ro_s, int* nzmap, int* ci_s,
+               hipStream_t s) {
+    if (n <= 0) return;
+    if (lanes == 8) {
+        hipLaunchKernelGGL((slab_fill_kernel<8>),
+                           dim3(grid_1d((long long)n * 8)), dim3(AMGX_BLOCK),
+                           0, s, ro, ci, rows, n, ro_s, nzmap, ci_s);
+    } else if (lanes == 1) {
+        hipLaunchKernelGGL((slab_fill_kernel<1>), dim3(grid_1d(n)),
+                           dim3(AMGX_BLOCK), 0, s, ro, ci, rows, n, ro_s,
+                           nzmap, ci_s);
+    } else {
+        throw std::runtime_error("slab_fill: lanes must be 1 or 8");
+    }
+}
+
+}
diff --git a/amgx_amd/csrc/kernels_setup.hip b/amgx_amd/csrc/kernels_setup.hip
--- a/amgx_amd/csrc/kernels_setup.hip
+++ b/amgx_amd/csrc/kernels_setup.hip
@@ -1,4 +1,5 @@
 
+#include <climits>
 #include <cstring>
 
 #include <rocprim/rocprim.hpp>
@@ -26,52 +27,78 @@
                                    const int* __restrict__ ci, int n,
                                    const int* __restrict__ colors_prev,
                                    int* __restrict__ colors_next, int iter,
-                                   int seed, int mode,
-                                   int* __restrict__ n_uncolored) {
-    int i = blockIdx.x * blockDim.x + threadIdx.x;
-    if (i >= n) return;
-    if (colors_prev[i] >= 0) { colors_next[i] = colors_prev[i]; return; }
-    unsigned long long mine =
-        ((unsigned long long)hash_u32((unsigned)i, (unsigned)seed) << 32) |
-        (unsigned)i;
-    bool is_max = true;
-    unsigned long long used = 0ull;
-    int big_used_max = -1;
-    for (int k = ro[i]; k < ro[i + 1]; ++k) {
-        int j = ci[k];
-        if (j == i || j >= n) continue;
-        int cj = colors_prev[j];
-        if (cj >= 0) {
-            if (cj < 64) used |= (1ull << cj);
-            else big_used_max = max(big_used_max, cj);
-            continue;
+                                   int seed, int mode, int* left) {
+    int i = blockIdx.x * blockDim.x + threadIdx.x;
+    int lost = 0;
+    if (i < n) {
+        int out = colors_prev[i];
+        if (out < 0) {
+            unsigned long long mine =
+                ((unsigned long long)hash_u32((unsigned)i, (unsigned)seed) << 32) |
+                (unsigned)i;
+            bool is_max = true;
+            unsigned long long used = 0ull;
+            int big_used_max = -1;
+            for (int k = ro[i]; k < ro[i + 1]; ++k) {
+                int j = ci[k];
+                if (j == i || j >= n) continue;
+                int cj = colors_prev[j];
+                if (cj >= 0) {
+                    if (cj < 64) used |= (1ull << cj);
+                    else big_used_max = max(big_used_max, cj);
+                    continue;
+                }
+                unsigned long long h =
+                    ((unsigned long long)hash_u32((unsigned)j, (unsigned)seed) << 32) |
+                    (unsigned)j;
+                if (h > mine) { is_max = false; break; }
+            }
+            if (is_max) {
+                if (mode == 1) {
+                    out = iter;
+                } else {
+                    int c = (int)(__builtin_ffsll((long long)~used) - 1);
+                    if (c < 0 || c >= 64) c = max(big_used_max, 63) + 1;
+                    out = c;
+                }
+            } else {
+                lost = 1;
+            }
         }
-        unsigned long long h =
-            ((unsigned long long)hash_u32((unsigned)j, (unsigned)seed) << 32) |
-            (unsigned)j;
-        if (h > mine) { is_max = false; break; }
-    }
-    int out = -1;
-    if (is_max) {
-        if (mode == 1) {
-            out = iter;
-        } else {
-            int c = (int)(__builtin_ffsll((long long)~used) - 1);
-            if (c < 0 || c >= 64) c = big_used_max + 1;
-            out = c;
-        }
-    } else {
-        atomicAdd(n_uncolored, 1);
-    }
-    colors_next[i] = out;
+        colors_next[i] = out;
+    }
+    if (__syncthreads_or(lost) && threadIdx.x == 0 && *left == 0) *left = 1;
 }
 
 void color_minmax_round(const int* ro, const int* ci, int n,
                         const int* colors_prev, int* colors_next, int iter,
-                        int seed, int mode, int* n_uncolored, hipStream_t s) {
+                        int seed, int mode, int* left, hipStream_t s) {
     hipLaunchKernelGGL(color_round_kernel, dim3(grid_1d(n)), dim3(AMGX_BLOCK),
                        0, s, ro, ci, n, colors_prev, colors_next, iter, seed,
-                       mode, n_uncolored);
+                       mode, left);
+}
+
+__global__ __launch_bounds__(AMGX_BLOCK) void int_max_kernel(
+    const int* __restrict__ v, int n, int* __restrict__ out) {
+    int m = INT_MIN;
+    for (long long i = (long long)blockIdx.x * blockDim.x + threadIdx.x; i < n;
+         i += (long long)gridDim.x * blockDim.x)
+        m = max(m, v[i]);
+    __shared__ int lds[AMGX_BLOCK];
+    lds[threadIdx.x] = m;
+    __syncthreads();
+    for (int w = AMGX_BLOCK / 2; w > 0; w >>= 1) {
+        if ((int)threadIdx.x < w)
+            lds[threadIdx.x] = max(lds[threadIdx.x], lds[threadIdx.x + w]);
+        __syncthreads();
+    }
+    if (threadIdx.x == 0) atomicMax(out, lds[0]);
+}
+
+void int_max(const int* v, int n, int* out, hipStream_t s) {
+    if (n <= 0) return;
+    hipLaunchKernelGGL(int_max_kernel, dim3(grid_1d(n, AMGX_BLOCK, 1024)),
+                       dim3(AMGX_BLOCK), 0, s, v, n, out);
 }
 
 template <typename T>
@@ -87,11 +114,25 @@
 }
 
 template <typename T>
+__global__ __launch_bounds__(AMGX_BLOCK) void agg_edge_weights_kernel(
+    const int* __restrict__ ro, const int* __restrict__ ci,
+    const T* __restrict__ va, const int* __restrict__ tidx,
+    const T* __restrict__ diag, int n, double* __restrict__ w) {
+    int i = blockIdx.x * blockDim.x + threadIdx.x;
+    if (i >= n) return;
+    for (int k = ro[i]; k < ro[i + 1]; ++k) {
+        int j = ci[k];
+        w[k] = (j == i || j >= n) ? 0.0 : edge_weight(va, tidx, diag, k, i, j);
+    }
+}
+
+template <typename T, bool PRE>
 __global__ __launch_bounds__(AMGX_BLOCK) void agg_propose_kernel(const int* __restrict__ ro,
                                    const int* __restrict__ ci,
                                    const T* __restrict__ va,
                                    const int* __restrict__ tidx,
-                                   const T* __restrict__ diag, int n,
+                                   const T* __restrict__ diag,
+                                   const double* __restrict__ wpre, int n,
                                    const int* __restrict__ agg,
                                    int* __restrict__ prop, int seed) {
     int i = blockIdx.x * blockDim.x + threadIdx.x;
@@ -103,7 +144,7 @@
     for (int k = ro[i]; k < ro[i + 1]; ++k) {
         int j = ci[k];
         if (j == i || j >= n || agg[j] >= 0) continue;
-        double w = edge_weight(va, tidx, diag, k, i, j);
+        double w = PRE ? wpre[k] : edge_weight(va, tidx, diag, k, i, j);
         unsigned int tj = hash_u32((unsigned)j, (unsigned)seed);
         if (w > bw ||
             (w == bw && best >= 0 &&
@@ -115,16 +156,19 @@
 }
 
 __global__ __launch_bounds__(AMGX_BLOCK) void agg_match_kernel(const int* __restrict__ prop, int n,
-                                 int* __restrict__ agg,
-                                 int* __restrict__ changed) {
-    int i = blockIdx.x * blockDim.x + threadIdx.x;
-    if (i >= n) return;
-    int j = prop[i];
-    if (j >= 0 && prop[j] == i && i < j) {
-        agg[i] = i;
-        agg[j] = i;
-        atomicAdd(changed, 1);
-    }
+                                 int* __restrict__ agg, int* changed) {
+    int i = blockIdx.x * blockDim.x + threadIdx.x;
+    int made = 0;
+    if (i < n) {
+        int j = prop[i];
+        if (j >= 0 && prop[j] == i && i < j) {
+            agg[i] = i;
+            agg[j] = i;
+            made = 1;
+        }
+    }
+    if (__syncthreads_or(made) && threadIdx.x == 0 && *changed == 0)
+        *changed = 1;
 }
 
 template <typename T>
@@ -153,12 +197,22 @@
 }
 
 template <typename T>
+void agg_edge_weights(const int* ro, const int* ci, const T* va,
+                      const int* tidx, const T* diag, int n, double* w,
+                      hipStream_t s) {
+    if (n <= 0) return;
+    hipLaunchKernelGGL((agg_edge_weights_kernel<T>), dim3(grid_1d(n)),
+                       dim3(AMGX_BLOCK), 0, s, ro, ci, va, tidx, diag, n, w);
+}
+
+template <typename T>
 void agg_propose(const int* ro, const int* ci, const T* va, const int* tidx,
-                 const T* diag, int n, const int* agg, int* prop, int seed,
-                 hipStream_t s) {
-    hipLaunchKernelGGL((agg_propose_kernel<T>), dim3(grid_1d(n)),
-                       dim3(AMGX_BLOCK), 0, s, ro, ci, va, tidx, diag, n, agg,
-                       prop, seed);
+                 const T* diag, const double* wpre, int n, const int* agg,
+                 int* prop, int seed, hipStream_t s) {
+    auto kern = wpre ? agg_propose_kernel<T, true>
+                     : agg_propose_kernel<T, false>;
+    hipLaunchKernelGGL(kern, dim3(grid_1d(n)), dim3(AMGX_BLOCK), 0, s, ro, ci,
+                       va, tidx, diag, wpre, n, agg, prop, seed);
 }
 
 void agg_match(const int* prop, int n, int* agg, int* changed, hipStream_t s) {
@@ -964,6 +1018,7 @@
 
 #define INSTANTIATE_SETUP(T)                                                   \
     AMGX_INSTANTIATE(agg_propose, T)                                           \
+    AMGX_INSTANTIATE(agg_edge_weights, T)                                      \
     AMGX_INSTANTIATE(agg_merge_singletons, T)                                  \
     AMGX_INSTANTIATE(pairwise_weights, T)                                      \
     AMGX_INSTANTIATE(galerkin_agg, T)                                         \
diff --git a/amgx_amd/ops/__init__.py b/amgx_amd/ops/__init__.py
--- a/amgx_amd/ops/__init__.py
+++ b/amgx_amd/ops/__init__.py
@@ -139,9 +139,10 @@
 
 
 def galerkin_aggregation(A, aggregates, num_aggregates, agg_col=None,
-                         ncols_mod=None, generator=None):
+                         ncols_mod=None, generator=None, structure=None):
     return _backend(A).galerkin_aggregation(A, aggregates, num_aggregates,
-                                            agg_col, ncols_mod, generator)
+                                            agg_col, ncols_mod, generator,
+                                            structure)
 
 
 def restrict_agg(r, aggregates, num_aggregates, block_dim: int = 1,
diff --git a/amgx_amd/ops/cpu.py b/amgx_amd/ops/cpu.py
--- a/amgx_amd/ops/cpu.py
+++ b/amgx_amd/ops/cpu.py
@@ -492,7 +492,7 @@
 
 
 def galerkin_aggregation(A, aggregates, num_aggregates, agg_col=None,
-                         ncols_mod=None, generator=None):
+                         ncols_mod=None, generator=None, structure=None):
     from ..matrix import CSRMatrix
     agg = _np(aggregates).astype(np.int64)
     n = A.n_rows
diff --git a/amgx_amd/ops/gpu.py b/amgx_amd/ops/gpu.py
--- a/amgx_amd/ops/gpu.py
+++ b/amgx_amd/ops/gpu.py
@@ -174,7 +174,8 @@
     _check_block_dim(A, "gs_sweep")
     if A.block_dim == 1:
         st = _slabs(A, coloring)
-        va_s = _slab_copy(st, "gs_va", A.values, lambda v: v[st.nzmap])
+        va_s = _slab_copy(st, "gs_va", A.values,
+                          lambda v: _gather_nz(v, st.nzmap))
         dinv_s = _slab_copy(st, "gs_dinv", dinv,
                             lambda d: d.reshape(-1)[st.perm])
         _core.gs_sweep_sorted(st.ro_s, st.ci_s, va_s, dinv_s, b.reshape(-1),
@@ -188,11 +189,26 @@
     return x
 
 
+ROUND_BATCH = 0
+
+
 def color_matrix(A, max_uncolored_frac: float = 0.0, seed: int = 0,
-                 multihash_rounds: int = 0):
+                 multihash_rounds: int = 0, batch: int = 0):
     colors, nc = _core.color_minmax(A.row_offsets, A.col_indices, A.n_rows,
-                                    4096, int(seed), int(multihash_rounds))
+                                    4096, int(seed), int(multihash_rounds),
+                                    int(batch or ROUND_BATCH))
     return colors, int(nc)
+
+
+def color_order(colors, num_colors):
+    return _core.key_order(colors.to(torch.int32).contiguous(),
+                           int(num_colors))
+
+
+def aggregate_csr(aggregates, num_aggregates):
+    fids, off = _core.key_order(aggregates.to(torch.int32).contiguous(),
+                                int(num_aggregates))
+    return off, fids
 
 
 class _Slabs:
@@ -207,25 +223,18 @@
         st.coloring = coloring
         st.copies = {}
         st.upper = st.lower = None
-        n = A.n_rows
-        perm = coloring.rows_sorted.to(torch.int64)
-        ro64 = A.row_offsets.to(torch.int64)
-        deg = ro64[1:] - ro64[:-1]
-        counts = deg[perm]
-        total = int(A.nnz)
-        st.ro_s = torch.zeros(n + 1, dtype=torch.int32, device=A.device)
-        csum = torch.cumsum(counts, 0)
-        st.ro_s[1:] = csum.to(torch.int32)
-        st.nzmap = (torch.repeat_interleave(ro64[perm], counts)
-                    + torch.arange(total, device=A.device, dtype=torch.int64)
-                    - torch.repeat_interleave(csum - counts, counts))
-        st.ci_s = A.col_indices[st.nzmap].contiguous()
-        st.perm = perm
-        st.slot_of_row = torch.empty(n, dtype=torch.int32, device=A.device)
-        st.slot_of_row[perm] = torch.arange(n, dtype=torch.int32,
-                                            device=A.device)
+        st.ro_s, st.ci_s, st.nzmap, st.slot_of_row = _core.slab_structure(
+            A.row_offsets, A.col_indices, coloring.rows_sorted)
+        st.perm = coloring.rows_sorted.to(torch.int64)
         A._cache["slabs"] = st
     return st
+
+
+def _gather_nz(values, nzmap, b: int = 1):
+    src = values.reshape(-1)
+    out = torch.empty(nzmap.numel() * b, dtype=src.dtype, device=src.device)
+    _core.gather(src.contiguous(), nzmap, b, out)
+    return out
 
 
 def _slab_copy(st, name, src, gather):
@@ -293,7 +302,7 @@
                             coloring.rows_sorted, coloring.bounds)
     st = _slabs(A, coloring)
     bb = A.block_dim * A.block_dim
-    va_s = A.values.reshape(A.nnz, -1)[st.nzmap].reshape(-1).contiguous()
+    va_s = _gather_nz(A.values, st.nzmap, bb)
     einv_s = einv.reshape(A.n_rows, bb)[st.perm].reshape(-1).contiguous() \
         if A.block_dim > 1 else einv[st.perm].contiguous()
     va_u = _gather_part(va_s, _slab_part(st, True)) if A.block_dim == 1 \
@@ -380,8 +389,8 @@
     return x
 
 
-def size2_matching(A, max_iterations: int = 15, deterministic: bool = True,
-                   seed: int = 0):
+def size2_roots(A, max_iterations: int = 15, seed: int = 0, batch: int = 0,
+                weights: bool = False):
     if A.block_dim > 1 and A.values.is_complex():
         raise NotImplementedError(
             "aggregation of a block matrix is not available in the complex "
@@ -391,15 +400,20 @@
         diag = torch.linalg.vector_norm(diag.reshape(A.n_rows, -1), dim=1)
         va = torch.linalg.vector_norm(
             A.values.reshape(A.nnz, -1).to(torch.float64), dim=1).to(A.dtype)
-        roots = _core.size2_match(A.row_offsets, A.col_indices, va, _tidx(A),
-                                  diag.to(A.dtype), A.n_rows, max_iterations,
-                                  int(seed) + 0x9E3779B1)
+        diag = diag.to(A.dtype)
     else:
-        roots = _core.size2_match(A.row_offsets, A.col_indices, A.values,
-                                  _tidx(A), diag, A.n_rows, max_iterations,
-                                  int(seed) + 0x9E3779B1)
-    uniq, agg = torch.unique(roots, sorted=True, return_inverse=True)
-    return agg.to(torch.int32), int(uniq.numel())
+        va = A.values
+    return _core.size2_match(A.row_offsets, A.col_indices, va, _tidx(A), diag,
+                             A.n_rows, max_iterations,
+                             int(seed) + 0x9E3779B1,
+                             int(batch or ROUND_BATCH), bool(weights))
+
+
+def size2_matching(A, max_iterations: int = 15, deterministic: bool = True,
+                   seed: int = 0, batch: int = 0):
+    agg, num = _core.size2_renumber(
+        size2_roots(A, max_iterations, seed, batch))
+    return agg, int(num)
 
 
 def pairwise_weights(A, formula: int = 0):
@@ -433,7 +447,7 @@
 
 
 def galerkin_aggregation(A, aggregates, num_aggregates, agg_col=None,
-                         ncols_mod=None, generator=None):
+                         ncols_mod=None, generator=None, structure=None):
     from ..matrix import CSRMatrix
     if agg_col is None:
         agg_col = aggregates
@@ -444,14 +458,10 @@
             "the Galerkin product of a block matrix is not available in the "
             "complex modes (dZZI / dCCI / dZCI)")
     if A.block_dim == 1 and generator != "THRUST":
-        agg64 = aggregates.to(torch.int64)
-        counts = torch.bincount(agg64, minlength=num_aggregates)
-        m_ro = torch.zeros(num_aggregates + 1, dtype=torch.int64,
-                           device=A.device)
-        m_ro[1:] = torch.cumsum(counts, 0)
-        fids = torch.argsort(agg64, stable=True).to(torch.int32)
+        m_ro, fids = structure if structure is not None \
+            else aggregate_csr(aggregates, num_aggregates)
         ro, ci, va, big = _core.spgemm_hash(
-            m_ro.to(torch.int32), fids, A.values,
+            m_ro, fids, A.values,
             A.row_offsets, A.col_indices, A.values,
             agg_col, 1, max(A.nnz, 1),
             64 if A.nnz <= 48 * max(num_aggregates, 1) else 512)
@@ -658,7 +668,7 @@
         return x
     lu_s, diag_s = _slab_copy(
         st, "ilu", factors, lambda f: (
-            f.reshape(-1)[st.nzmap],
+            _gather_nz(f, st.nzmap),
             f.reshape(-1)[_didx(A).to(torch.int64)][st.perm]))
     _core.ilu0_apply_sorted(st.ro_s, st.ci_s, lu_s, diag_s, st.slot_of_row,
                             coloring.rows_sorted, coloring.bounds,
diff --git a/profiles/setup_kernel_rows.py b/profiles/setup_kernel_rows.py
--- /dev/null
+++ b/profiles/setup_kernel_rows.py
@@ -0,0 +1,48 @@
+#!/usr/bin/env python3
+import collections
+import csv
+import re
+import sys
+
+ROWS = [
+    ("color_round_kernel", r"color_round_kernel"),
+    ("agg_match_kernel", r"agg_match_kernel"),
+    ("agg_propose_kernel", r"agg_propose_kernel"),
+    ("agg_singleton_kernel", r"agg_singleton_kernel"),
+    ("native orderings (key offsets, root flag / map, slab, int_max)",
+     r"keys_to_offsets|root_flag|root_map|slab_lengths|slab_fill_kernel|"
+     r"int_max_kernel|fill_int_kernel"),
+    ("gather_kernel", r"amgx_hip::gather_kernel"),
+    ("torch int64 chains and rocPRIM sorts / scans",
+     r"rocprim|compute_cuda_kernel<long>|kernelHistogram1D|"
+     r"index_elementwise_kernel|_scatter_gather_elementwise_kernel|"
+     r"CUDAFunctor_add<long>|write_indices|arange_cuda_out|"
+     r"FillFunctor<int>|FillFunctor<long>|radixSortKVInPlace|"
+     r"bitonicSortKVInPlace|fill_reverse_indices|sort_postprocess"),
+]
+
+
+def table(path):
+    out = collections.OrderedDict((name, [0, 0.0, 0.0]) for name, _ in ROWS)
+    for r in csv.DictReader(open(path)):
+        for name, pat in ROWS:
+            if re.search(pat, r["kernel"]):
+                e = out[name]
+                e[0] += int(r["calls"])
+                e[1] += float(r["total_ms"])
+                e[2] = max(e[2], float(r["max_ms"]))
+                break
+    return out
+
+
+def main():
+    a, b = table(sys.argv[1]), table(sys.argv[2])
+    print("| item | parent calls | ms | max call | branch calls | ms | max call |")
+    print("|---|---|---|---|---|---|---|")
+    for name in a:
+        print("| %s | %d | %.1f | %.2f | %d | %.1f | %.2f |"
+              % (name, *a[name], *b[name]))
+
+
+if __name__ == "__main__":
+    main()
diff --git a/setup.py b/setup.py
--- a/setup.py
+++ b/setup.py
@@ -16,6 +16,7 @@
         os.path.join(csrc, "bindings.cpp"),
         os.path.join(csrc, "kernels_solve.hip"),
         os.path.join(csrc, "kernels_setup.hip"),
+        os.path.join(csrc, "kernels_order.hip"),
         os.path.join(csrc, "kernels_classical.hip"),
         os.path.join(csrc, "kernels_mfma.hip"),
         os.path.join(csrc, "kernels_spgemm.hip"),
```
